# IGNF/StrataNet2-Vegetation-Coverage-Maps

Hardware: AMD Instinct MI355X
Metric: plots/s fwd+bwd, 32k-pt synthetic plots, batch 16/GPU (higher is better)
Workload: dtype f32; 1 GPU; C2 ref-arch: 16 plots/GPU x 32768 pts, SA npoint 1024/256 + global, r 1/2 m, train step fwd+P2+loss+bwd+Adam, inputs resident in HBM; plots_per_gpu=16, points_per_plot=32768, batches_per_geometry_pass=8, exchange=none (single GPU), parallelism=single GPU, ranks_seen=1, exchange_in_graph=False

## Files before the change

### include/strata_hip.h

```cpp
#ifndef STRATA_HIP_H
#define STRATA_HIP_H

#include <stddef.h>

#ifdef __cplusplus
extern "C" {
#endif

#define SN2_VERSION 102
#define SN2_EINVAL (-1)
#define SN2_ELIMIT (-2)

#define SN2_MAX_NEIGHBORS 2000
#define SN2_STAT_SLOTS 1024

int sn2_version(void);
int sn2_debug_mfma_chain(const float *a, const float *b, float *d, int mode, void *stream);
int sn2_debug_spin(int blocks, long long clocks, int *out, void *stream);

int sn2_debug_fp1_backward_parts(int mask);
int sn2_debug_fp_rows_form(int form);
int sn2_debug_fp_table_form(int form);
#define SN2_PROBE_SINK_WORDS 4096
int sn2_debug_stream_probe(const float *src, float *dst, size_t n_floats, int mode, float *sink, void *stream);
int sn2_debug_mfma_probe(int mode, int iters, float *sink, double *flops, void *stream);

typedef struct sn2_block {
    int cin, cout;
    const float *W, *b;
    const float *gamma, *beta;
    float *running_mean, *running_var;
    float *a, *c;
    float *mean, *invstd;
    float *stat_slots;
    float *dW, *db, *dgamma, *dbeta;
    int grad_replicas, grad_replica_stride;
    int mma_bf16;
    long long *num_batches_tracked;
    int frozen_stats;
} sn2_block;
#define SN2_BN_FROZEN_KEEP 2
int sn2_grad_reduce(float *flat, int n, int replicas, int stride, void *stream);


int sn2_pack_rows(const float *cloud, const float *xyz, int B, int C, int N, float *rows0, void *stream);

#define SN2_FPS_WS_WORDS(B, N) (6L * (B) * (N) + (4104L + 4096L) * (B) + 32L)
int sn2_fps(const float *pos_soa, int B, int N, int M, const int *start, int *idx, float *cpos_soa,
            float *cpos_aos, int *order_ws, void *stream);
int sn2_fps_waves(const float *pos_soa, int B, int N, int M, const int *start, int *idx, float *cpos_soa,
                  float *cpos_aos, int *order_ws, int waves, void *stream);
int sn2_fps_status(const float *pos_soa, int B, int N, int M, const int *start, int *idx, float *cpos_soa,
                   float *cpos_aos, int *order_ws, int waves, unsigned *status, void *stream);
int sn2_debug_fps_spin_limit(unsigned sweeps);

int sn2_ball_query(const float *src_soa, int B, int N, const float *cpos_soa, int M, float r2, int cap,
                   int *nbr, int *cnt, unsigned long long *total, const int *fps_ws, void *stream);

int sn2_count_sum(const int *cnt, int n, unsigned long long *total, void *stream);
int sn2_count_sum_group(const int *cnt, int G, int n, unsigned long long *total, size_t total_stride, void *stream);

#define SN2_THREE_NN_WS_WORDS(B, S) ((size_t)(B) * (4 * (size_t)(S) + 1032))
int sn2_three_nn(const float *src_soa, int B, int S, const float *dst_soa, int T, int k, int *idx, float *w,
                 void *ws, const int *dst_fps_ws, void *stream);
#define SN2_THREE_NN_XY_WS_WORDS(B, S, T) ((size_t)(B) * (4 * (size_t)(S) + 5 * (size_t)(T) + 1032))
int sn2_three_nn_xy(const float *src_soa, int B, int S, const float *dst_soa, int T, int k, int *idx, float *w,
                    void *ws, void *stream);

int sn2_prepare_plots(const float *raw, long T, const int *offsets, const float *centers, const float *fake_xy, int n_fake,
                      const int *idx, int B, int N, int train, const double *rot, const int *flips, const float *noise,
                      const long *noise_offsets, long noise_T, float z_max, float *cloud, float *xyz, void *stream);

#define SN2_SUBSAMPLE_LDS 1
#define SN2_SUBSAMPLE_GLOBAL 2
#define SN2_SUBSAMPLE_COARSE 4
#define SN2_SUBSAMPLE_LDS_MAX 16384
int sn2_subsample_form(int n_max, int N);
size_t sn2_subsample_ws_words(int B, int n_max, int N, int form);
int sn2_subsample(const int *offsets, int extra, int n_max, int B, int N, unsigned long long seed, const long long *plot_keys,
                  int form, int *ws, size_t ws_words, int *idx, void *stream);

#define SN2_ZNORM_WS_WORDS(n, cells) ((size_t)5 * (n) + 3 * (size_t)(cells) + 8)
int sn2_znorm(const float *x, const float *y, const float *z, int n, float radius, float x_min, float y_min, float x_max,
              float y_max, int *ws, float *zmin, float *z_out, void *stream);

size_t sn2_parcel_count_ws_words(int P, int rows);
size_t sn2_parcel_znorm_ws_words(long T, float radius, float x_min, float y_min, float x_max, float y_max);
int sn2_parcel_count(const float *cloud, long T, int L, int rows, const float *centers, int P, const int *cell_start,
                     const int *cell_items, int GX, int GY, double gx0, double gy0, double cell_inv, float radius, int *ws,
                     size_t ws_words, int *prefix, long long *total, void *stream);
int sn2_parcel_fill(const float *cloud, long T, int L, int rows, const float *centers, int P, const int *cell_start,
                    const int *cell_items, int GX, int GY, double gx0, double gy0, double cell_inv, float radius, int *prefix,
                    const int *plot_base, long sum_n, float *raw, int *point_index, void *stream);
int sn2_parcel_znorm(const float *cloud, long T, float x_min, float y_min, float x_max, float y_max, float radius,
                     float disc_radius, const int *offsets, const float *centers, int P, const int *point_index, long sum_n,
                     int *ws, size_t ws_words, float *raw, void *stream);

typedef struct sn2_sa {
    int B, Nsrc, M, cap;
    int cf;
    int nl;
    const float *feat; int feat_stride;
    const float *spos; int spos_stride;
    const float *cpos;
    const int *nbr, *cnt;
    const unsigned long long *total;
    const int *order;
    sn2_block blk[2];
    float *ext; int *arg;
    float *out;
    const float *dout;
    float *dfeat;
    float *bwd_ws;
} sn2_sa;
#define SN2_SA_BWD_WS_REPLICAS 32
#define SN2_SA_BWD_WS_WORDS (SN2_SA_BWD_WS_REPLICAS * 2 * 16 * 12)
#define SN2_SA_SOLO_MIN 64
#define SN2_SA_QUAD_MIN 8
#define SN2_SA_OCT_MIN 4
#define SN2_SA_SOLO_FLAG 0x40000000
#define SN2_SA_OCT_FLAG 0x20000000
#define SN2_SA_PACKED_ITEMS(M) ((M) / 8 + 2)
#define SN2_SA_ORDER_WORDS(B, M) ((size_t)4 * (B) * (M) + (size_t)16 * (B) * SN2_SA_PACKED_ITEMS(M) + 8)
int sn2_sa_order(const int *cnt, int B, int M, int *order, void *stream);
int sn2_sa_order_group(const int *cnt, int G, int B, int M, int *order, size_t stride_words, void *stream);
int sn2_sa_forward(const sn2_sa *p, int training, void *stream);
int sn2_sa_backward(const sn2_sa *p, void *stream);

typedef struct sn2_fp {
    int B, R_per_plot, S_per_plot;
    int ca, cb;
    const float *src; int src_stride; const float *src_a, *src_c;
    const int *knn_idx; const float *knn_w;
    const float *skip; int skip_stride;
    sn2_block blk;
    float *h; int h_stride;
    const float *dy;
    float *dsrc; int dsrc_stride;
    float *dskip; int dskip_stride;
    float *du_scratch;
    float *scatter_ws;
    int scatter_ready;
    const int *bn_sums_done;
    float *src_ws;
    int act_bf16;
    const int *row_perm;
} sn2_fp;
#define SN2_INTERP_CHUNKS(R, S) ((3 * (size_t)(R) + 62) / 63 + (size_t)(S))
#define SN2_FP_SRC_WS_WORDS(B, R, S, cout) ((size_t)(B) * SN2_INTERP_CHUNKS(R, S) * ((((cout) + 3) / 4) * 4))
#define SN2_INTERP_WS_WORDS(B, R, S) \
    ((size_t)(B) * (S) * (((R) + 2047) / 2048 + 6) + 6 * (size_t)(B) * (R) + 64 + 4 * (size_t)(B) * SN2_INTERP_CHUNKS(R, S))
int sn2_interp_index(const int *knn_idx, const float *knn_w, const float *src_pos, int B, int R_per_plot,
                     int S_per_plot, float *ws, void *stream);
int sn2_interp_index_perm(const int *knn_idx, const float *knn_w, const float *src_pos, const int *row_perm, int B,
                          int R_per_plot, int S_per_plot, float *ws, void *stream);
int sn2_interp_index_group(const int *knn_idx, const float *knn_w, const float *src_pos, const int *row_perm, int G, int B,
                           int R_per_plot, int S_per_plot, float *ws, size_t ws_stride_words, void *stream);
int sn2_fp_forward(const sn2_fp *p, int training, void *stream);
int sn2_fp_backward(const sn2_fp *p, void *stream);

int sn2_plot_max_forward(const float *h, const float *a, const float *c, int B, int R_per_plot, int C, float *out,
                         int *arg, void *stream);
int sn2_plot_max_backward(const float *dout, const int *arg, int B, int R_per_plot, int C, float *dy, void *stream);

int sn2_global_pool_backward(const float *du, int du_stride, const int *arg, const float *h, const float *mean,
                             const float *invstd, int B, int R_per_plot, int C, float *dx, float *dy, float *dgamma,
                             float *dbeta, void *stream);

#define SN2_GLOBAL_XCHG_WORDS(B) ((size_t)2 * (size_t)(B) * 4 * 128)
#define SN2_GLOBAL_CTL_WORDS 8
int sn2_global_level_forward(const sn2_fp *sa3, const sn2_fp *fp3, float *x3, int *arg3, unsigned long long *xchg,
                             unsigned *ctl, void *stream);
int sn2_debug_global_spin_limit(unsigned sweeps);

typedef struct sn2_head {
    int R, cin, f_stride;
    const float *f, *fa, *fc;
    const float *W1, *b1, *W2, *b2;
    float *coverages, *proba;
    const float *dcoverages, *dproba;
    float *dy;
    float *dW1, *db1, *dW2, *db2;
    int grad_replicas, grad_replica_stride;
    const int *drop_mask;
    float drop_scale;
    int act_bf16;
    float *zero_fill; long zero_fill_words;
} sn2_head;
int sn2_head_forward(const sn2_head *p, void *stream);
int sn2_fp_head_eval(const sn2_fp *p, const sn2_head *hd, void *stream);
int sn2_head_backward(const sn2_head *p, void *stream);
int sn2_head_bn_sums(const sn2_head *p, const float *gamma, const float *beta, const float *mean, const float *invstd,
                     float *dgamma, float *dbeta, int *ok, void *stream);
int sn2_fp_bn_sums(const sn2_fp *p, const float *gamma, const float *beta, const float *mean, const float *invstd,
                   float *dgamma, float *dbeta, int *ok, void *stream);


int sn2_plot_project_forward(const float *pred_pointwise, const float *cloud_xy, long plot_stride, int B, int N,
                             int D, unsigned long long *keys, int *pix, int *arg, int *nocc, float *pred,
                             void *stream);
#define SN2_P2_KEY_PARTS(N) (((N) + 4095) / 4096 < 1 ? 1 : (((N) + 4095) / 4096 > 64 ? 64 : ((N) + 4095) / 4096))
int sn2_plot_pixels(const float *cloud_xy, long plot_stride, int B, int N, int D, float *mm, int *pix, void *stream);
int sn2_plot_project_forward_pix(const float *pred_pointwise, const int *pix, int B, int N, int D,
                                 unsigned long long *keys, int *arg, int *nocc, float *pred, void *stream);
int sn2_plot_project_backward(const float *dpred, const int *arg, const int *nocc, const int *pix, int B, int N,
                              int D, float *dpointwise, void *stream);

int sn2_raster_project(const float *coverages, const float *cloud_xy, long plot_stride, int B, int N, int D,
                       int diam_meters, unsigned long long *keys, int *pix, float *rasters, void *stream);

int sn2_mosaic_merge(const float *rasters, const float *weights, const int *offsets, int B, int D, int H, int W,
                     float *mean, float *wsum, int win_y0, int win_x0, int win_h, int win_w, void *stream);

#define SN2_MOSAIC_HIST_WORDS 10004
int sn2_mosaic_finalize(const float *mean, const float *wsum, int H, int W, int *hist_ws, double *sum_ws, float *thr_out,
                        float *out, void *stream);

int sn2_kde_lookup(const float *cloud, int B, int C, int N, int z_channel, float z_max, const double *X, const double *Y,
                   int K, double *pdf, void *stream);
#define SN2_KDE_FIT_MAX_K 65536
#define SN2_KDE_FIT_ABS_SLOTS 256
#define SN2_KDE_FIT_SLICES 8
#define SN2_KDE_FIT_WS_WORDS(K) \
    (2 * ((4 + 3 * SN2_KDE_FIT_SLICES) * (size_t)(K) + 3 * (((size_t)(K) + 255) / 256)) + SN2_KDE_FIT_ABS_SLOTS)
int sn2_kde_fit(const float *z, long n, double bw, int K, void *ws, double *X, double *Y, void *stream);
#define SN2_LOSS_BLOCKS 1024
int sn2_loss_forward(const float *pred, const double *gt, int B, const float *proba, const double *pdf, int R, double m,
                     double e, double *partials, double *out, void *stream);
int sn2_loss_backward(const float *pred, const double *gt, int B, const float *proba, const double *pdf, int R, double m,
                      double e, const double *grad_total, float *dpred, float *dproba, void *stream);

#define SN2_PROJECTED_LOSS_WS (2 * 512 + 2)
int sn2_projected_loss_forward(const float *coverages, const int *pix, const float *proba, const double *pdf, const double *gt,
                               int B, int N, int D, double m, double e, unsigned long long *keys, int *arg, int *nocc,
                               float *pred, double *partials, double *out, void *stream);
int sn2_projected_loss_backward(const float *pred, const double *gt, int B, const float *proba, const double *pdf, int N, int D,
                                double m, double e, const double *grad_total, const int *arg, const int *nocc, const int *pix,
                                float *dcoverages, float *dproba, void *stream);

#define SN2_PLOT_LOSSES_SLICE_ROWS 2048
#define SN2_PLOT_LOSSES_SLICES(N) \
    (((N) + SN2_PLOT_LOSSES_SLICE_ROWS - 1) / SN2_PLOT_LOSSES_SLICE_ROWS < 1 ? 1 : \
     (((N) + SN2_PLOT_LOSSES_SLICE_ROWS - 1) / SN2_PLOT_LOSSES_SLICE_ROWS > 64 ? 64 : ((N) + SN2_PLOT_LOSSES_SLICE_ROWS - 1) / SN2_PLOT_LOSSES_SLICE_ROWS))
size_t sn2_plot_losses_ws_words(int B, int N, int D);
int sn2_plot_losses(const float *coverages, const int *pix, const float *proba, const double *pdf, const double *gt, int B, int N,
                    int D, double m, double e, void *ws, float *pred, double *out, void *stream);

int sn2_adam_step(float *param, const float *grad, float *exp_avg, float *exp_avg_sq, int n, float lr, float beta1,
                  float beta2, float eps, float weight_decay, int *step_dev ,
                  float grad_scale, void *stream);


typedef struct sn2_net_layer {
    int cin, cout;
    const float *W, *b, *gamma, *beta;
    float *running_mean, *running_var;
    long long *num_batches_tracked;
    int gW, gb, ggamma, gbeta;
    int mma_bf16;
} sn2_net_layer;

typedef struct sn2_net_model {
    sn2_net_layer sa1[2], sa2, sa3, fp3, fp2, fp1;
    const float *lin1_W, *lin1_b, *lin2_W, *lin2_b;
    int g_lin1_W, g_lin1_b, g_lin2_W, g_lin2_b;
    int n_flat;
    float r1_sq, r2_sq;
    int max_neighbors;
    float drop_p;
    int fuse_global_level;
    int fuse_eval_head;
    int source_side;
    int fps_waves_shared, fps_waves_many;
} sn2_net_model;

typedef struct sn2_net_dims {
    int B, N, M1, M2;
    int cap1, cap2;
    int act_bf16;
    int p2_diam_pix;
} sn2_net_dims;

typedef struct sn2_net_geo {
    const float *xyz;
    int *idx1; float *pos1_soa, *pos1_aos; int *ws1;
    int *nbr1, *cnt1; unsigned long long *tot1; int *ord1;
    int *idx2; float *pos2_soa, *pos2_aos; int *ws2;
    int *nbr2, *cnt2; unsigned long long *tot2; int *ord2;
    const float *pos3;
    int *knn3_idx; float *knn3_w;
    int *knn2_idx; float *knn2_w;
    int *knn1_idx; float *knn1_w;
    float *inv3, *inv2, *inv1;
    int *nn_ws2, *nn_ws1;
    const int *rank1;
    float *rows0;
    int *p2_pix; float *p2_mm;
} sn2_net_geo;

typedef struct sn2_net_act {
    float *aux;
    float *stats;
    float *ext1; int *arg1; float *x1;
    float *ext2; int *arg2; float *x2;
    float *h_sa3, *h3;
    float *x3; int *arg3;
    float *h2;
    void *h1;
    float *src_ws1, *src_ws2;
    float *cov, *proba;
    const int *drop_mask;
    float *bwd_arena; long bwd_arena_words;
} sn2_net_act;

typedef struct sn2_net_bwd {
    const float *dcov, *dproba;
    float *arena; long arena_words;
    int images, image_stride;
    float *dy2, *dy3, *dx1, *dx2, *dx3, *dy_sa3;
    float *sa1_ws;
    void *dy1, *du1;
    float *du2, *du3;
    int *bn_ok;
    float *src_ws1, *src_ws2;
    int defer_grad_reduce;
    int arena_is_zero;
    int frozen_stats;
} sn2_net_bwd;

#define SN2_NET_FORK 1
#define SN2_NET_SHARED 2
#define SN2_NET_INVERTED 4
#define SN2_NET_DEFER_JOIN 8
#define SN2_NET_INPUT_ONLY 16
#define SN2_NET_HAS_ROWS0 32
#define SN2_NET_JOIN_PENDING 64
#define SN2_NET_WITH_GEOMETRY 128
#define SN2_NET_HAS_INVERTED 256

typedef struct sn2_net_io {
    const float *cloud;
    const int *fps_start;
    unsigned *fps_status;
    unsigned long long *gl_xchg; unsigned *gl_ctl;
    void *stream_b, *stream_c, *stream_pack;
    void *ctx;
    int flags;
    int training;
} sn2_net_io;

int sn2_net_ctx_create(void **ctx);
int sn2_net_ctx_destroy(void *ctx);
int sn2_net_geo_carve(const sn2_net_model *m, const sn2_net_dims *d, void *base, sn2_net_geo *out, size_t *bytes);
int sn2_net_act_carve(const sn2_net_model *m, const sn2_net_dims *d, int training, void *base, sn2_net_act *out, size_t *bytes);
int sn2_net_bwd_carve(const sn2_net_model *m, const sn2_net_dims *d, void *arena_base, void *scratch_base, sn2_net_bwd *out,
                      size_t *arena_bytes, size_t *scratch_bytes);
int sn2_net_geometry(const sn2_net_model *m, const sn2_net_dims *d, const sn2_net_geo *g, const sn2_net_io *io, void *stream);
int sn2_net_forward(const sn2_net_model *m, const sn2_net_dims *d, const sn2_net_geo *g, const sn2_net_act *a,
                    const sn2_net_io *io, void *stream);
int sn2_net_backward(const sn2_net_model *m, const sn2_net_dims *d, const sn2_net_geo *g, const sn2_net_act *a,
                     const sn2_net_bwd *b, void *stream);

int sn2_adam_step_images(float *param, float *grad_images, int replicas, int stride, float *exp_avg, float *exp_avg_sq, int n,
                         float lr, float beta1, float beta2, float eps, float weight_decay, int *step_dev, float grad_scale,
                         void *stream);

#ifdef __cplusplus
}
#endif
#endif
```

### stratanet2_vegetation_coverage_maps_amd/_build.py

```python
import os
import subprocess
import sys
from concurrent.futures import ThreadPoolExecutor

HERE = os.path.dirname(os.path.abspath(__file__))
CSRC = os.path.join(HERE, "csrc")
LIB = os.path.join(CSRC, "libstrata_hip.so")
VARIANT_DIR = os.path.join(os.path.dirname(HERE), "build", "variants")
SOURCES = ["geometry.hip", "sa.hip", "sa_mfma.hip", "fp.hip", "interp_index.hip", "global_level.hip", "head.hip", "project.hip",
           "loss.hip", "misc.hip", "net.hip", "parcel.hip", "sample.hip", "kde.hip"]
HEADERS = ["common.h", "mlp.h", "fp_rows.h", os.path.join("..", "..", "include", "strata_hip.h")]
FLAGS = ["--offload-arch=gfx950", "-O3", "-fPIC", "-std=c++17", "-Wno-unused-result"] + os.environ.get("SN2_EXTRA_HIPCC_FLAGS", "").split()


def _stale(target, deps):
    if not os.path.exists(target):
        return True
    t = os.path.getmtime(target)
    return any(os.path.getmtime(d) > t for d in deps)


def _compile(lib, objdir, flags, force, verbose):
    hipcc = os.environ.get("HIPCC", "/opt/rocm/bin/hipcc")
    if not os.path.exists(hipcc):
        hipcc = "hipcc"
    hdrs = [os.path.join(CSRC, h) for h in HEADERS]
    objs, jobs = [], []
    for s in SOURCES:
        src = os.path.join(CSRC, s)
        obj = os.path.join(objdir, s.replace(".hip", ".o"))
        objs.append(obj)
        if force or _stale(obj, [src] + hdrs):
            jobs.append([hipcc] + flags + ["-c", src, "-o", obj])

    def run(cmd):
        if verbose:
            print(" ".join(cmd), flush=True)
        r = subprocess.run(cmd, stdout=subprocess.PIPE, stderr=subprocess.STDOUT, text=True)
        if r.returncode != 0:
            raise RuntimeError(f"hipcc failed ({r.returncode}):\n{r.stdout}")
        return r.stdout

    with ThreadPoolExecutor(max_workers=min(4, max(1, len(jobs)))) as ex:
        list(ex.map(run, jobs))
    if force or jobs or _stale(lib, objs):
        run([hipcc, "--offload-arch=gfx950", "-shared", "-fPIC"] + objs + ["-o", lib])
    return lib


def build(force: bool = False, verbose: bool = True) -> str:
    return _compile(LIB, CSRC, FLAGS, force, verbose)


def build_variant(name: str, extra_flags=(), verbose: bool = False) -> str:
    out = os.path.abspath(os.path.join(VARIANT_DIR, name))
    if os.path.commonpath([out, CSRC]) == CSRC:
        raise ValueError(f"{out}: a variant build must not go into {CSRC}")
    objdir = out + ".objs"
    os.makedirs(objdir, exist_ok=True)
    return _compile(out, objdir, FLAGS + list(extra_flags), True, verbose)


if __name__ == "__main__":
    print(build(force="--force" in sys.argv))
```

### stratanet2_vegetation_coverage_maps_amd/_lib.py

```python
import ctypes
import os
from ctypes import POINTER, Structure, c_double, c_float, c_int, c_long, c_longlong, c_void_p

HERE = os.path.dirname(os.path.abspath(__file__))
LIB_PATH = os.path.join(HERE, "csrc", "libstrata_hip.so")

SN2_VERSION = 102
MAX_NEIGHBORS = 2000
STAT_SLOTS = 1024


class Block(Structure):
    _fields_ = [("cin", c_int), ("cout", c_int), ("W", c_void_p), ("b", c_void_p), ("gamma", c_void_p),
                ("beta", c_void_p), ("running_mean", c_void_p), ("running_var", c_void_p), ("a", c_void_p),
                ("c", c_void_p), ("mean", c_void_p), ("invstd", c_void_p), ("stat_slots", c_void_p),
                ("dW", c_void_p), ("db", c_void_p), ("dgamma", c_void_p), ("dbeta", c_void_p),
                ("grad_replicas", c_int), ("grad_replica_stride", c_int), ("mma_bf16", c_int),
                ("num_batches_tracked", c_void_p), ("frozen_stats", c_int)]


BN_FROZEN_KEEP = 2


class SA(Structure):
    _fields_ = [("B", c_int), ("Nsrc", c_int), ("M", c_int), ("cap", c_int), ("cf", c_int), ("nl", c_int),
                ("feat", c_void_p), ("feat_stride", c_int), ("spos", c_void_p), ("spos_stride", c_int),
                ("cpos", c_void_p), ("nbr", c_void_p), ("cnt", c_void_p), ("total", c_void_p), ("order", c_void_p),
                ("blk", Block * 2),
                ("ext", c_void_p), ("arg", c_void_p), ("out", c_void_p), ("dout", c_void_p), ("dfeat", c_void_p),
                ("bwd_ws", c_void_p)]


class FP(Structure):
    _fields_ = [("B", c_int), ("R_per_plot", c_int), ("S_per_plot", c_int), ("ca", c_int), ("cb", c_int),
                ("src", c_void_p), ("src_stride", c_int), ("src_a", c_void_p), ("src_c", c_void_p),
                ("knn_idx", c_void_p), ("knn_w", c_void_p), ("skip", c_void_p), ("skip_stride", c_int),
                ("blk", Block), ("h", c_void_p), ("h_stride", c_int), ("dy", c_void_p), ("dsrc", c_void_p),
                ("dsrc_stride", c_int), ("dskip", c_void_p), ("dskip_stride", c_int), ("du_scratch", c_void_p),
                ("scatter_ws", c_void_p), ("scatter_ready", c_int), ("bn_sums_done", c_void_p), ("src_ws", c_void_p),
                ("act_bf16", c_int), ("row_perm", c_void_p)]


class Head(Structure):
    _fields_ = [("R", c_int), ("cin", c_int), ("f_stride", c_int), ("f", c_void_p), ("fa", c_void_p),
                ("fc", c_void_p), ("W1", c_void_p), ("b1", c_void_p), ("W2", c_void_p), ("b2", c_void_p),
                ("coverages", c_void_p), ("proba", c_void_p), ("dcoverages", c_void_p), ("dproba", c_void_p),
                ("dy", c_void_p), ("dW1", c_void_p), ("db1", c_void_p), ("dW2", c_void_p), ("db2", c_void_p),
                ("grad_replicas", c_int), ("grad_replica_stride", c_int), ("drop_mask", c_void_p), ("drop_scale", c_float),
                ("act_bf16", c_int), ("zero_fill", c_void_p), ("zero_fill_words", c_long)]


class NetLayer(Structure):
    _fields_ = [("cin", c_int), ("cout", c_int), ("W", c_void_p), ("b", c_void_p), ("gamma", c_void_p), ("beta", c_void_p),
                ("running_mean", c_void_p), ("running_var", c_void_p), ("num_batches_tracked", c_void_p),
                ("gW", c_int), ("gb", c_int), ("ggamma", c_int), ("gbeta", c_int), ("mma_bf16", c_int)]


class NetModel(Structure):
    _fields_ = [("sa1", NetLayer * 2), ("sa2", NetLayer), ("sa3", NetLayer), ("fp3", NetLayer), ("fp2", NetLayer), ("fp1", NetLayer),
                ("lin1_W", c_void_p), ("lin1_b", c_void_p), ("lin2_W", c_void_p), ("lin2_b", c_void_p),
                ("g_lin1_W", c_int), ("g_lin1_b", c_int), ("g_lin2_W", c_int), ("g_lin2_b", c_int), ("n_flat", c_int),
                ("r1_sq", c_float), ("r2_sq", c_float), ("max_neighbors", c_int), ("drop_p", c_float),
                ("fuse_global_level", c_int), ("fuse_eval_head", c_int), ("source_side", c_int),
                ("fps_waves_shared", c_int), ("fps_waves_many", c_int)]


class NetDims(Structure):
    _fields_ = [("B", c_int), ("N", c_int), ("M1", c_int), ("M2", c_int), ("cap1", c_int), ("cap2", c_int), ("act_bf16", c_int),
                ("p2_diam_pix", c_int)]


class NetGeo(Structure):
    _fields_ = [(n, c_void_p) for n in (
        "xyz", "idx1", "pos1_soa", "pos1_aos", "ws1", "nbr1", "cnt1", "tot1", "ord1",
        "idx2", "pos2_soa", "pos2_aos", "ws2", "nbr2", "cnt2", "tot2", "ord2", "pos3",
        "knn3_idx", "knn3_w", "knn2_idx", "knn2_w", "knn1_idx", "knn1_w", "inv3", "inv2", "inv1", "nn_ws2", "nn_ws1",
        "rank1", "rows0", "p2_pix", "p2_mm")]


class NetAct(Structure):
    _fields_ = [(n, c_void_p) for n in (
        "aux", "stats", "ext1", "arg1", "x1", "ext2", "arg2", "x2", "h_sa3", "h3", "x3", "arg3", "h2", "h1", "src_ws1", "src_ws2",
        "cov", "proba", "drop_mask", "bwd_arena")] + [("bwd_arena_words", c_long)]


class NetBwd(Structure):
    _fields_ = [("dcov", c_void_p), ("dproba", c_void_p), ("arena", c_void_p), ("arena_words", c_long), ("images", c_int),
                ("image_stride", c_int)] + [(n, c_void_p) for n in (
                    "dy2", "dy3", "dx1", "dx2", "dx3", "dy_sa3", "sa1_ws", "dy1", "du1", "du2", "du3", "bn_ok", "src_ws1", "src_ws2")] + [
                        ("defer_grad_reduce", c_int), ("arena_is_zero", c_int), ("frozen_stats", c_int)]


class NetIO(Structure):
    _fields_ = [("cloud", c_void_p), ("fps_start", c_void_p), ("fps_status", c_void_p), ("gl_xchg", c_void_p), ("gl_ctl", c_void_p),
                ("stream_b", c_void_p), ("stream_c", c_void_p), ("stream_pack", c_void_p), ("ctx", c_void_p), ("flags", c_int),
                ("training", c_int)]


NET_FORK, NET_SHARED, NET_INVERTED, NET_DEFER_JOIN, NET_INPUT_ONLY = 1, 2, 4, 8, 16
NET_HAS_ROWS0, NET_JOIN_PENDING, NET_WITH_GEOMETRY, NET_HAS_INVERTED = 32, 64, 128, 256


SIGNATURES = {
    "sn2_version": [],
    "sn2_debug_mfma_chain": [c_void_p, c_void_p, c_void_p, c_int, c_void_p],
    "sn2_debug_spin": [c_int, c_longlong, c_void_p, c_void_p],
    "sn2_debug_fp1_backward_parts": [c_int],
    "sn2_debug_fp_rows_form": [c_int],
    "sn2_debug_fp_table_form": [c_int],
    "sn2_debug_stream_probe": [c_void_p, c_void_p, ctypes.c_size_t, c_int, c_void_p, c_void_p],
    "sn2_debug_mfma_probe": [c_int, c_int, c_void_p, POINTER(c_double), c_void_p],
    "sn2_pack_rows": [c_void_p, c_void_p, c_int, c_int, c_int, c_void_p, c_void_p],
    "sn2_fps": [c_void_p, c_int, c_int, c_int, c_void_p, c_void_p, c_void_p, c_void_p, c_void_p, c_void_p],
    "sn2_fps_waves": [c_void_p, c_int, c_int, c_int, c_void_p, c_void_p, c_void_p, c_void_p, c_void_p, c_int, c_void_p],
    "sn2_fps_status": [c_void_p, c_int, c_int, c_int, c_void_p, c_void_p, c_void_p, c_void_p, c_void_p, c_int, c_void_p, c_void_p],
    "sn2_debug_fps_spin_limit": [ctypes.c_uint],
    "sn2_ball_query": [c_void_p, c_int, c_int, c_void_p, c_int, c_float, c_int, c_void_p, c_void_p, c_void_p, c_void_p,
                       c_void_p],
    "sn2_three_nn": [c_void_p, c_int, c_int, c_void_p, c_int, c_int, c_void_p, c_void_p, c_void_p, c_void_p, c_void_p],
    "sn2_count_sum": [c_void_p, c_int, c_void_p, c_void_p],
    "sn2_count_sum_group": [c_void_p, c_int, c_int, c_void_p, ctypes.c_size_t, c_void_p],
    "sn2_three_nn_xy": [c_void_p, c_int, c_int, c_void_p, c_int, c_int, c_void_p, c_void_p, c_void_p, c_void_p],
    "sn2_prepare_plots": [c_void_p, c_long, c_void_p, c_void_p, c_void_p, c_int, c_void_p, c_int, c_int, c_int, c_void_p,
                          c_void_p, c_void_p, c_void_p, c_long, c_float, c_void_p, c_void_p, c_void_p],
    "sn2_znorm": [c_void_p, c_void_p, c_void_p, c_int, c_float, c_float, c_float, c_float, c_float, c_void_p, c_void_p,
                  c_void_p, c_void_p],
    "sn2_parcel_count": [c_void_p, c_long, c_int, c_int, c_void_p, c_int, c_void_p, c_void_p, c_int, c_int, c_double, c_double,
                         c_double, c_float, c_void_p, ctypes.c_size_t, c_void_p, c_void_p, c_void_p],
    "sn2_parcel_fill": [c_void_p, c_long, c_int, c_int, c_void_p, c_int, c_void_p, c_void_p, c_int, c_int, c_double, c_double,
                        c_double, c_float, c_void_p, c_void_p, c_long, c_void_p, c_void_p, c_void_p],
    "sn2_parcel_znorm": [c_void_p, c_long, c_float, c_float, c_float, c_float, c_float, c_float, c_void_p, c_void_p, c_int,
                         c_void_p, c_long, c_void_p, ctypes.c_size_t, c_void_p, c_void_p],
    "sn2_subsample_form": [c_int, c_int],
    "sn2_subsample": [c_void_p, c_int, c_int, c_int, c_int, ctypes.c_ulonglong, c_void_p, c_int, c_void_p, ctypes.c_size_t,
                      c_void_p, c_void_p],
    "sn2_sa_order": [c_void_p, c_int, c_int, c_void_p, c_void_p],
    "sn2_sa_order_group": [c_void_p, c_int, c_int, c_int, c_void_p, ctypes.c_size_t, c_void_p],
    "sn2_sa_forward": [POINTER(SA), c_int, c_void_p],
    "sn2_sa_backward": [POINTER(SA), c_void_p],
    "sn2_grad_reduce": [c_void_p, c_int, c_int, c_int, c_void_p],
    "sn2_interp_index": [c_void_p, c_void_p, c_void_p, c_int, c_int, c_int, c_void_p, c_void_p],
    "sn2_interp_index_perm": [c_void_p, c_void_p, c_void_p, c_void_p, c_int, c_int, c_int, c_void_p, c_void_p],
    "sn2_interp_index_group": [c_void_p, c_void_p, c_void_p, c_void_p, c_int, c_int, c_int, c_int, c_void_p, ctypes.c_size_t, c_void_p],
    "sn2_fp_forward": [POINTER(FP), c_int, c_void_p],
    "sn2_fp_backward": [POINTER(FP), c_void_p],
    "sn2_plot_max_forward": [c_void_p, c_void_p, c_void_p, c_int, c_int, c_int, c_void_p, c_void_p, c_void_p],
    "sn2_plot_max_backward": [c_void_p, c_void_p, c_int, c_int, c_int, c_void_p, c_void_p],
    "sn2_global_pool_backward": [c_void_p, c_int, c_void_p, c_void_p, c_void_p, c_void_p, c_int, c_int, c_int, c_void_p, c_void_p,
                                 c_void_p, c_void_p, c_void_p],
    "sn2_global_level_forward": [POINTER(FP), POINTER(FP), c_void_p, c_void_p, c_void_p, c_void_p, c_void_p],
    "sn2_debug_global_spin_limit": [ctypes.c_uint],
    "sn2_head_forward": [POINTER(Head), c_void_p],
    "sn2_fp_head_eval": [POINTER(FP), POINTER(Head), c_void_p],
    "sn2_fp_bn_sums": [POINTER(FP), c_void_p, c_void_p, c_void_p, c_void_p, c_void_p, c_void_p, c_void_p, c_void_p],
    "sn2_head_bn_sums": [POINTER(Head), c_void_p, c_void_p, c_void_p, c_void_p, c_void_p, c_void_p, c_void_p, c_void_p],
    "sn2_head_backward": [POINTER(Head), c_void_p],
    "sn2_plot_project_forward": [c_void_p, c_void_p, c_long, c_int, c_int, c_int, c_void_p, c_void_p, c_void_p,
                                 c_void_p, c_void_p, c_void_p],
    "sn2_plot_pixels": [c_void_p, c_long, c_int, c_int, c_int, c_void_p, c_void_p, c_void_p],
    "sn2_plot_project_forward_pix": [c_void_p, c_void_p, c_int, c_int, c_int, c_void_p, c_void_p, c_void_p, c_void_p, c_void_p],
    "sn2_plot_project_backward": [c_void_p, c_void_p, c_void_p, c_void_p, c_int, c_int, c_int, c_void_p, c_void_p],
    "sn2_raster_project": [c_void_p, c_void_p, c_long, c_int, c_int, c_int, c_int, c_void_p, c_void_p, c_void_p,
                           c_void_p],
    "sn2_mosaic_merge": [c_void_p, c_void_p, c_void_p, c_int, c_int, c_int, c_int, c_void_p, c_void_p,
                         c_int, c_int, c_int, c_int, c_void_p],
    "sn2_mosaic_finalize": [c_void_p, c_void_p, c_int, c_int, c_void_p, c_void_p, c_void_p, c_void_p, c_void_p],
    "sn2_kde_lookup": [c_void_p, c_int, c_int, c_int, c_int, c_float, c_void_p, c_void_p, c_int, c_void_p, c_void_p],
    "sn2_kde_fit": [c_void_p, c_long, c_double, c_int, c_void_p, c_void_p, c_void_p, c_void_p],
    "sn2_loss_forward": [c_void_p, c_void_p, c_int, c_void_p, c_void_p, c_int, c_double, c_double, c_void_p, c_void_p,
                         c_void_p],
    "sn2_loss_backward": [c_void_p, c_void_p, c_int, c_void_p, c_void_p, c_int, c_double, c_double, c_void_p, c_void_p,
                          c_void_p, c_void_p],
    "sn2_adam_step": [c_void_p, c_void_p, c_void_p, c_void_p, c_int, c_float, c_float, c_float, c_float, c_float,
                      c_void_p, c_float, c_void_p],
    "sn2_projected_loss_forward": [c_void_p, c_void_p, c_void_p, c_void_p, c_void_p, c_int, c_int, c_int, c_double, c_double, c_void_p,
                                   c_void_p, c_void_p, c_void_p, c_void_p, c_void_p, c_void_p],
    "sn2_projected_loss_backward": [c_void_p, c_void_p, c_int, c_void_p, c_void_p, c_int, c_int, c_double, c_double, c_void_p, c_void_p,
                                    c_void_p, c_void_p, c_void_p, c_void_p, c_void_p],
    "sn2_plot_losses": [c_void_p, c_void_p, c_void_p, c_void_p, c_void_p, c_int, c_int, c_int, c_double, c_double, c_void_p, c_void_p,
                        c_void_p, c_void_p],
    "sn2_adam_step_images": [c_void_p, c_void_p, c_int, c_int, c_void_p, c_void_p, c_int, c_float, c_float, c_float, c_float, c_float,
                             c_void_p, c_float, c_void_p],
    "sn2_net_ctx_create": [POINTER(c_void_p)],
    "sn2_net_ctx_destroy": [c_void_p],
    "sn2_net_geo_carve": [POINTER(NetModel), POINTER(NetDims), c_void_p, POINTER(NetGeo), POINTER(ctypes.c_size_t)],
    "sn2_net_act_carve": [POINTER(NetModel), POINTER(NetDims), c_int, c_void_p, POINTER(NetAct), POINTER(ctypes.c_size_t)],
    "sn2_net_bwd_carve": [POINTER(NetModel), POINTER(NetDims), c_void_p, c_void_p, POINTER(NetBwd), POINTER(ctypes.c_size_t),
                          POINTER(ctypes.c_size_t)],
    "sn2_net_geometry": [POINTER(NetModel), POINTER(NetDims), POINTER(NetGeo), POINTER(NetIO), c_void_p],
    "sn2_net_forward": [POINTER(NetModel), POINTER(NetDims), POINTER(NetGeo), POINTER(NetAct), POINTER(NetIO), c_void_p],
    "sn2_net_backward": [POINTER(NetModel), POINTER(NetDims), POINTER(NetGeo), POINTER(NetAct), POINTER(NetBwd), c_void_p],
}

SIZE_HELPERS = {
    "sn2_parcel_count_ws_words": [c_int, c_int],
    "sn2_parcel_znorm_ws_words": [c_long, c_float, c_float, c_float, c_float, c_float],
    "sn2_subsample_ws_words": [c_int, c_int, c_int, c_int],
    "sn2_plot_losses_ws_words": [c_int, c_int, c_int],
}

_lib = None


class StrataHipError(RuntimeError):
    pass


def load():
    global _lib
    if _lib is not None:
        return _lib
    if not os.path.exists(LIB_PATH):
        raise StrataHipError(
            f"{LIB_PATH} not found: build it with `python -m stratanet2_vegetation_coverage_maps_amd._build` "
            "(or __graft_entry__.build()); the HIP library is mandatory, there is no fallback path")
    lib = ctypes.CDLL(LIB_PATH)
    for name, argtypes in SIGNATURES.items():
        fn = getattr(lib, name)
        fn.argtypes = argtypes
        fn.restype = c_int
    for name, argtypes in SIZE_HELPERS.items():
        fn = getattr(lib, name)
        fn.argtypes = argtypes
        fn.restype = ctypes.c_size_t
    if lib.sn2_version() != SN2_VERSION:
        raise StrataHipError(f"libstrata_hip.so version {lib.sn2_version()} != binding {SN2_VERSION}: rebuild")
    _lib = lib
    return lib


def check(rc: int, what: str):
    if rc != 0:
        kind = "hipError_t" if rc > 0 else {-1: "SN2_EINVAL", -2: "SN2_ELIMIT"}.get(rc, "error")
        raise StrataHipError(f"{what} failed: {kind} {rc}")
```

### stratanet2_vegetation_coverage_maps_amd/csrc/common.h

```cpp
#pragma once
#include <hip/hip_runtime.h>
#include <stdint.h>

#include "../../include/strata_hip.h"

#define SN2_WAVE 64

#define SN2_RETURN_LAUNCH()                                   \
    do {                                                      \
        hipError_t e__ = hipGetLastError();                   \
        return e__ == hipSuccess ? 0 : (int)e__;              \
    } while (0)

#define SN2_TRY(expr)                \
    do {                             \
        int r__ = (expr);            \
        if (r__ != 0) return r__;    \
    } while (0)

#ifdef SN2_NO_FLUSH
#define SN2_FLUSH_ADD(ptr, v) do { if ((v) == 12345.678f) atomicAdd((ptr), (v)); } while (0)
#else
#define SN2_FLUSH_ADD(ptr, v) atomicAdd((ptr), (v))
#endif

#ifdef __HIPCC__
__device__ __forceinline__ int sn2_grad_image(int replicas, int stride) {
    return replicas > 1 ? (int)(blockIdx.x % (unsigned)replicas) * stride : 0;
}
#endif

static inline int sn2_cdiv(long a, long b) { return (int)((a + b - 1) / b); }

constexpr int GL_MAX_PLOTS = 28;

#ifdef __HIPCC__
static __global__ __launch_bounds__(256) void sn2_fill_words_kernel(uint32_t* __restrict__ p, uint32_t v, size_t n) {
    for (size_t i = (size_t)blockIdx.x * 256 + threadIdx.x; i < n; i += (size_t)gridDim.x * 256) p[i] = v;
}
static inline void sn2_fill_words(void* p, uint32_t v, size_t nwords, hipStream_t st) {
    if (nwords == 0) return;
    int grid = sn2_cdiv((long)nwords, 256 * 4);
    grid = grid < 1 ? 1 : (grid > 2048 ? 2048 : grid);
    hipLaunchKernelGGL(sn2_fill_words_kernel, dim3(grid), dim3(256), 0, st, (uint32_t*)p, v, nwords);
}
#endif

static inline bool sn2_small_sort_wg(int B) { return B > 32; }

static inline int sn2_cu_count() {
    static int n = 0;
    if (n == 0) {
        int dev = 0, v = 0;
        if (hipGetDevice(&dev) == hipSuccess &&
            hipDeviceGetAttribute(&v, hipDeviceAttributeMultiprocessorCount, dev) == hipSuccess && v > 0)
            n = v;
        else
            n = 256;
    }
    return n;
}

typedef const float __attribute__((address_space(4)))* cfp;
__device__ __forceinline__ cfp as_const(const float* p) { return (cfp)(uintptr_t)p; }
__device__ __forceinline__ cfp opaque(cfp p) {
    uint64_t v = (uint64_t)p;
    asm volatile("" : "+s"(v));
    return (cfp)v;
}

__device__ __forceinline__ float sn2_d2(float ax, float ay, float az, float bx, float by, float bz) {
#pragma clang fp contract(off)
    float dx = ax - bx;
    float dy = ay - by;
    float dz = az - bz;
    float xx = dx * dx;
    float yy = dy * dy;
    float zz = dz * dz;
    float s = xx + yy;
    return s + zz;
}

__device__ __forceinline__ unsigned long long wave_max_u64(unsigned long long v) {
#pragma unroll
    for (int o = 32; o > 0; o >>= 1) {
        unsigned long long t = __shfl_xor(v, o);
        v = t > v ? t : v;
    }
    return v;
}

#define SN2_DPP(x, ctrl, rmask) __builtin_amdgcn_update_dpp((x), (x), (ctrl), (rmask), 0xF, false)
__device__ __forceinline__ float wave_max_dpp(float v) {
    v = fmaxf(v, __int_as_float(SN2_DPP(__float_as_int(v), 0xB1, 0xF)));
    v = fmaxf(v, __int_as_float(SN2_DPP(__float_as_int(v), 0x4E, 0xF)));
    v = fmaxf(v, __int_as_float(SN2_DPP(__float_as_int(v), 0x141, 0xF)));
    v = fmaxf(v, __int_as_float(SN2_DPP(__float_as_int(v), 0x140, 0xF)));
    v = fmaxf(v, __int_as_float(SN2_DPP(__float_as_int(v), 0x142, 0xA)));
    v = fmaxf(v, __int_as_float(SN2_DPP(__float_as_int(v), 0x143, 0xC)));
    return __int_as_float(__builtin_amdgcn_readlane(__float_as_int(v), 63));
}
__device__ __forceinline__ float wave_min_dpp(float v) { return -wave_max_dpp(-v); }
__device__ __forceinline__ float wave_sum_dpp(float v) {
    v += __int_as_float(SN2_DPP(__float_as_int(v), 0xB1, 0xF));
    v += __int_as_float(SN2_DPP(__float_as_int(v), 0x4E, 0xF));
    v += __int_as_float(SN2_DPP(__float_as_int(v), 0x141, 0xF));
    v += __int_as_float(SN2_DPP(__float_as_int(v), 0x140, 0xF));
    v += __int_as_float(SN2_DPP(__float_as_int(v), 0x142, 0xA));
    v += __int_as_float(SN2_DPP(__float_as_int(v), 0x143, 0xC));
    return __int_as_float(__builtin_amdgcn_readlane(__float_as_int(v), 63));
}
__device__ __forceinline__ float wave_sum(float v) { return wave_sum_dpp(v); }
__device__ __forceinline__ float wave_max(float v) { return wave_max_dpp(v); }
__device__ __forceinline__ float wave_min(float v) { return wave_min_dpp(v); }
__device__ __forceinline__ unsigned wave_min_u32_dpp(unsigned v) {
    v = min(v, (unsigned)SN2_DPP((int)v, 0xB1, 0xF));
    v = min(v, (unsigned)SN2_DPP((int)v, 0x4E, 0xF));
    v = min(v, (unsigned)SN2_DPP((int)v, 0x141, 0xF));
    v = min(v, (unsigned)SN2_DPP((int)v, 0x140, 0xF));
    v = min(v, (unsigned)SN2_DPP((int)v, 0x142, 0xA));
    v = min(v, (unsigned)SN2_DPP((int)v, 0x143, 0xC));
    return (unsigned)__builtin_amdgcn_readlane((int)v, 63);
}

__device__ __forceinline__ int lane_id() { return threadIdx.x & 63; }

__device__ __forceinline__ uint32_t f2ord(float f) {
    uint32_t u = __float_as_uint(f);
    return (u & 0x80000000u) ? ~u : (u | 0x80000000u);
}
__device__ __forceinline__ float ord2f(uint32_t o) {
    uint32_t u = (o & 0x80000000u) ? (o & 0x7FFFFFFFu) : ~o;
    return __uint_as_float(u);
}
```

### stratanet2_vegetation_coverage_maps_amd/csrc/global_level.hip

```cpp
#include "fp_rows.h"

namespace {

#ifdef SN2_GL_STAMPS
__device__ unsigned long long g_gl_dbg[16];
extern "C" int sn2_debug_gl_stamps(unsigned long long* out) {
    return (int)hipMemcpyFromSymbol(out, HIP_SYMBOL(g_gl_dbg), sizeof(g_gl_dbg));
}
#define GSTAMP(i)                                                                                   \
    if (blockIdx.x == 0 && threadIdx.x == 0) {                                                      \
        unsigned long long t_;                                                                      \
        asm volatile("s_memtime %0\n\ts_waitcnt lgkmcnt(0)" : "=s"(t_)::"memory");                   \
        g_gl_dbg[i] = t_;                                                                           \
    }
#else
#define GSTAMP(i)
#endif
typedef unsigned long long gl_u64;
constexpr int GL_GROUPS = 4, GL_QS = OuterAcc<16, 36>::QS;
constexpr int GL_W3 = 64 * 35 + 64, GL_WF = 64 * 96 + 64;
constexpr int GL_FIXED_FLOATS = GL_GROUPS * 64 * GL_QS + GL_GROUPS * 128 + 128 + 64 + 2 * 1024 + 2 * 8 * 128 + GL_W3 + GL_WF;
static_assert((GL_FIXED_FLOATS + GL_MAX_PLOTS * GL_GROUPS * 128) * 4 <= 160 * 1024, "LDS");

template <int KB>
__device__ __forceinline__ void gl_block_tiles(const float* s_q, int QS, int lane, int g, long row0, long R_lim,
                                               const float (&Wb)[KB], float init, float* __restrict__ h, int h_stride,
                                               float& ssum, float& ssq, f32x4 (&V)[4]) {
    const int qq = lane >> 4, cc = lane & 15, o = 16 * g + cc;
#pragma unroll
    for (int t = 0; t < 4; ++t) V[t] = f32x4{init, init, init, init};
#pragma unroll
    for (int kb = 0; kb < KB; ++kb) {
#pragma unroll
        for (int t = 0; t < 4; ++t)
            V[t] = __builtin_amdgcn_mfma_f32_16x16x4f32(s_q[(16 * t + cc) * QS + 4 * kb + qq], Wb[kb], V[t], 0, 0, 0);
    }
#pragma unroll
    for (int t = 0; t < 4; ++t)
#pragma unroll
        for (int j = 0; j < 4; ++j) {
            const long row = row0 + 16 * t + 4 * qq + j;
            const float v = row < R_lim ? fmaxf(V[t][j], 0.f) : 0.f;
            V[t][j] = v;
            ssum += v;
            ssq = fmaf(v, v, ssq);
            if (row < R_lim) h[(size_t)row * h_stride + o] = v;
        }
}

struct GlLayer {
    const float *W, *bias, *gamma, *beta;
    float *running_mean, *running_var, *a, *c, *mean, *invstd;
    long long* nbt;
    float* h;
};
struct GlArgs {
    int B, M2;
    const float* x2;
    const float* pos2;
    const int* knn_idx;
    const float* knn_w;
    float* x3;
    int* arg3;
    GlLayer sa3, fp3;
    gl_u64* xchg;
    unsigned* ctl;
    unsigned spin_limit;
};

constexpr unsigned GL_POISON = 0x80000000u;
__device__ __forceinline__ bool gl_collect(const gl_u64* gx, int n, unsigned tag, float* s_x, unsigned spin_limit) {
    bool ok = true;
    for (int i0 = threadIdx.x; i0 < n; i0 += 8 * 1024) {
        gl_u64 v[8];
        unsigned spins = 0;
        bool all, poisoned;
        do {
#pragma unroll
            for (int u = 0; u < 8; ++u) {
                const int i = i0 + u * 1024;
                v[u] = __hip_atomic_load(gx + (i < n ? i : i0), __ATOMIC_RELAXED, __HIP_MEMORY_SCOPE_AGENT);
            }
            all = true, poisoned = false;
#pragma unroll
            for (int u = 0; u < 8; ++u) {
                all = all && (unsigned)(v[u] >> 32) == tag;
                poisoned = poisoned || (unsigned)(v[u] >> 32) == (tag ^ GL_POISON);
            }
            if (!all && !poisoned) __builtin_amdgcn_s_sleep(2);
        } while (!all && !poisoned && ++spins < spin_limit);
        if (!all) ok = false;
#pragma unroll
        for (int u = 0; u < 8; ++u)
            if (i0 + u * 1024 < n) s_x[i0 + u * 1024] = __uint_as_float((unsigned)v[u]);
    }
    return ok;
}

template <bool REPAIR>
__device__ __forceinline__ void gl_level_body(const GlArgs& A, float* gl_smem) {
    const int tid = threadIdx.x, lane = tid & 63;
    const int grp = __builtin_amdgcn_readfirstlane(tid >> 8), g = __builtin_amdgcn_readfirstlane((tid >> 6) & 3);
    float* s_q = gl_smem + grp * 64 * GL_QS;

    float* s_red = gl_smem + GL_GROUPS * 64 * GL_QS;
    float* s_ac = s_red + GL_GROUPS * 128;
    float* s_x3 = s_ac + 128;
    float* s_mv = s_x3 + 64;
    int* s_mi = reinterpret_cast<int*>(s_mv + 1024);
    double* s_d = reinterpret_cast<double*>(s_mi + 1024);
    float* s_w3 = reinterpret_cast<float*>(s_d + 8 * 128);
    float* s_wf = s_w3 + GL_W3;
    float* s_x = s_wf + GL_WF;
    __shared__ unsigned s_epoch;
    __shared__ int s_fail;
    const int B = A.B, M2 = A.M2;
    const int b_lo = REPAIR ? 0 : (int)blockIdx.x, b_hi = REPAIR ? B : b_lo + 1;
    const bool lead = REPAIR || blockIdx.x == 0;
    float w3r[3], b3r, bfr;
    f32x4 wfr[2];
#pragma unroll
    for (int j = 0; j < 3; ++j) w3r[j] = A.sa3.W[min(tid + 1024 * j, 64 * 35 - 1)];
#pragma unroll
    for (int j = 0; j < 2; ++j) wfr[j] = reinterpret_cast<const f32x4*>(A.fp3.W)[min(tid + 1024 * j, 64 * 96 / 4 - 1)];
    b3r = A.sa3.bias[tid & 63], bfr = A.fp3.bias[tid & 63];
    unsigned epoch_now = 0;
    if (tid == 0) epoch_now = __hip_atomic_load(&A.ctl[0], __ATOMIC_RELAXED, __HIP_MEMORY_SCOPE_AGENT);
#pragma unroll
    for (int j = 0; j < 3; ++j)
        if (tid + 1024 * j < 64 * 35) s_w3[tid + 1024 * j] = w3r[j];
#pragma unroll
    for (int j = 0; j < 2; ++j)
        if (tid + 1024 * j < 64 * 96 / 4) reinterpret_cast<f32x4*>(s_wf)[tid + 1024 * j] = wfr[j];
    if (tid < 64) s_w3[64 * 35 + tid] = b3r, s_wf[64 * 96 + tid] = bfr;
    if (tid == 0) {
        s_epoch = epoch_now + 1u;
        s_fail = 0;
    }
    const int nblk = (M2 + 63) >> 6, trips = (nblk + GL_GROUPS - 1) / GL_GROUPS;
    const int qq = lane >> 4, cc = lane & 15, o = 16 * g + cc;
    const int n_gran = B * GL_GROUPS * 128;
    const double n_rows = (double)B * (double)M2;
    __syncthreads();
    const unsigned epoch = s_epoch;
    unsigned applied = 0;
    if constexpr (REPAIR) applied = __hip_atomic_load(&A.ctl[3], __ATOMIC_RELAXED, __HIP_MEMORY_SCOPE_AGENT);
    f32x4 V3[4];
#pragma unroll
    for (int t = 0; t < 4; ++t) V3[t] = f32x4{0.f, 0.f, 0.f, 0.f};
    GSTAMP(0)
    for (int b = b_lo; b < b_hi; ++b) {
        constexpr int CA = 32, CB = 3, CI = CA + CB, CK = CI + 1, KB = (CK + 3) / 4, QS = OuterAcc<16, CK>::QS;
        const long row_lo = (long)b * M2, R_lim = row_lo + M2;
        float Wb[KB];
        float ssum = 0.f, ssq = 0.f;
        for (int it = 0; it < trips; ++it) {
            const int blk = it * GL_GROUPS + grp;
            const long r0 = row_lo + (long)blk * 64;
            if (blk < nblk) {
                stage_inputs<CA, CB, false>(s_q, QS, g, lane, r0, (int)R_lim, M2, M2, A.x2, 32, nullptr, nullptr, nullptr, nullptr,
                                            A.pos2, 4);
                if (g == 2) {
#pragma unroll
                    for (int k = CK; k < 4 * KB; ++k) s_q[lane * QS + k] = 0.f;
                }
            }
            __syncthreads();
            if (it == 0) {
#pragma unroll
                for (int kb = 0; kb < KB; ++kb) {
                    const int k = 4 * kb + qq;
                    Wb[kb] = k < CI ? s_w3[o * CI + k] : (k == CI ? s_w3[64 * CI + o] : 0.f);
                }
            }
            if (blk < nblk) gl_block_tiles<KB>(s_q, QS, lane, g, r0, R_lim, Wb, 0.f, A.sa3.h, 64, ssum, ssq, V3);
            __syncthreads();
        }
        ssum += __shfl_xor(ssum, 16);
        ssq += __shfl_xor(ssq, 16);
        ssum += __shfl_xor(ssum, 32);
        ssq += __shfl_xor(ssq, 32);
        if (qq == 0) {
            s_red[grp * 128 + o] = ssum;
            s_red[grp * 128 + 64 + o] = ssq;
        }
        __syncthreads();
        if (b == b_lo) { GSTAMP(1) }
        if (tid < GL_GROUPS * 128)
            __hip_atomic_store(A.xchg + (size_t)b * GL_GROUPS * 128 + tid,
                               ((gl_u64)(epoch * 2u + 0u) << 32) | (gl_u64)__float_as_uint(s_red[tid]), __ATOMIC_RELAXED,
                               __HIP_MEMORY_SCOPE_AGENT);
        if constexpr (REPAIR) __syncthreads();
    }
    {
        const unsigned tag = epoch * 2u + 0u;
        if (!gl_collect(A.xchg, n_gran, tag, s_x, A.spin_limit)) s_fail = 1;
        __syncthreads();
        GSTAMP(2)
        if (s_fail) {
            if constexpr (!REPAIR) {
                if (tid < GL_GROUPS * 128)
                    __hip_atomic_store(A.xchg + n_gran + (size_t)b_lo * GL_GROUPS * 128 + tid, (gl_u64)((epoch * 2u + 1u) ^ GL_POISON) << 32,
                                       __ATOMIC_RELAXED, __HIP_MEMORY_SCOPE_AGENT);
                if (tid == 0) {
                    atomicAdd(&A.ctl[1], 1u);
                    if (lead) {
                        __hip_atomic_store(&A.ctl[3], 0u, __ATOMIC_RELAXED, __HIP_MEMORY_SCOPE_AGENT);
                        __hip_atomic_store(&A.ctl[0], epoch, __ATOMIC_RELAXED, __HIP_MEMORY_SCOPE_AGENT);
                    }
                }
                return;
            }
        }
        {
            const int col = tid & 127, part = tid >> 7;
            double acc = 0.0;
            for (int w = part; w < B * GL_GROUPS; w += 8) acc += (double)s_x[w * 128 + col];
            s_d[part * 128 + col] = acc;
        }
        __syncthreads();
        if (tid < 64) {
            double s1 = 0.0, s2 = 0.0;
#pragma unroll
            for (int part = 0; part < 8; ++part) s1 += s_d[part * 128 + tid], s2 += s_d[part * 128 + 64 + tid];
            float aa, cc2, mean, invstd;
            const bool upd = lead && !(applied & 1u);
            sn2_bn_from_sums(s1, s2, n_rows, A.sa3.gamma[tid], A.sa3.beta[tid], upd ? &A.sa3.running_mean[tid] : nullptr,
                             upd ? &A.sa3.running_var[tid] : nullptr, aa, cc2, mean, invstd);
            s_ac[tid] = aa;
            s_ac[64 + tid] = cc2;
            if (lead) {
                A.sa3.a[tid] = aa, A.sa3.c[tid] = cc2, A.sa3.mean[tid] = mean, A.sa3.invstd[tid] = invstd;
                if (tid == 0 && upd && A.sa3.nbt) *A.sa3.nbt += 1;
            }
        }
        __syncthreads();
    }
    GSTAMP(3)
    for (int b = b_lo; b < b_hi; ++b) {
    const long row_lo = (long)b * M2, R_lim = row_lo + M2;
    if (!REPAIR && trips == 1) {
        const float aa = s_ac[o], cc2 = s_ac[64 + o];
        float best = -INFINITY;
        int bi = 0x7FFFFFFF;
#pragma unroll
        for (int t = 0; t < 4; ++t)
#pragma unroll
            for (int j = 0; j < 4; ++j) {
                const int r = grp * 64 + 16 * t + 4 * qq + j;
                const float y = fmaf(aa, V3[t][j], cc2);
                if (r < M2 && y > best) best = y, bi = r;
            }
#pragma unroll
        for (int m = 16; m <= 32; m <<= 1) {
            const float v = __shfl_xor(best, m);
            const int i = __shfl_xor(bi, m);
            if (v > best || (v == best && i < bi)) best = v, bi = i;
        }
        if (qq == 0) s_mv[grp * 64 + o] = best, s_mi[grp * 64 + o] = bi;
        __syncthreads();
        if (tid < 64) {
            best = s_mv[tid], bi = s_mi[tid];
            for (int k2 = 1; k2 < GL_GROUPS; ++k2) {
                const float v = s_mv[k2 * 64 + tid];
                const int i = s_mi[k2 * 64 + tid];
                if (v > best || (v == best && i < bi)) best = v, bi = i;
            }
            A.x3[(size_t)b * 64 + tid] = best;
            A.arg3[(size_t)b * 64 + tid] = bi;
            s_x3[tid] = best;
        }
        __syncthreads();
    } else {
        const int ch = tid & 63, rg = tid >> 6;
        const float aa = s_ac[ch], cc2 = s_ac[64 + ch];
        float best = -INFINITY;
        int bi = 0x7FFFFFFF;
        const float* hb = A.sa3.h + (size_t)row_lo * 64 + ch;
        int r = rg;
        for (; r + 7 * 16 < M2; r += 8 * 16) {
            float v[8];
#pragma unroll
            for (int u = 0; u < 8; ++u) v[u] = hb[(size_t)(r + u * 16) * 64];
#pragma unroll
            for (int u = 0; u < 8; ++u) {
                const float y = fmaf(aa, v[u], cc2);
                if (y > best) best = y, bi = r + u * 16;
            }
        }
        for (; r < M2; r += 16) {
            const float y = fmaf(aa, hb[(size_t)r * 64], cc2);
            if (y > best) best = y, bi = r;
        }
        s_mv[tid] = best;
        s_mi[tid] = bi;
        __syncthreads();
        if (tid < 64) {
            for (int k2 = 1; k2 < 16; ++k2) {
                const float v = s_mv[k2 * 64 + ch];
                const int i = s_mi[k2 * 64 + ch];
                if (v > best || (v == best && i < bi)) best = v, bi = i;
            }
            A.x3[(size_t)b * 64 + ch] = best;
            A.arg3[(size_t)b * 64 + ch] = bi;
            s_x3[ch] = best;
        }
        __syncthreads();
    }
    if (b == b_lo) { GSTAMP(4) }
    {
        constexpr int CA = 64, CB = 32, CI = CA + CB, KB = CB / 4, QS = OuterAcc<16, 36>::QS;
        float* s_pv = s_mv;
        {
            const int oo = tid >> 4, part = tid & 15;
            const float4 w4 = *reinterpret_cast<const float4*>(s_wf + oo * CI + 4 * part);
            const float4 u4 = *reinterpret_cast<const float4*>(s_x3 + 4 * part);
            float acc = ((w4.x * u4.x + w4.y * u4.y) + w4.z * u4.z) + w4.w * u4.w;
#pragma unroll
            for (int m = 8; m > 0; m >>= 1) acc += __shfl_xor(acc, m);
            if (part == 0) s_pv[oo] = acc + s_wf[64 * CI + oo];
        }
        float Wb[KB];
#pragma unroll
        for (int kb = 0; kb < KB; ++kb) Wb[kb] = s_wf[o * CI + CA + 4 * kb + qq];
        float ssum = 0.f, ssq = 0.f;
        f32x4 Vf[4];
        for (int it = 0; it < trips; ++it) {
            const int blk = it * GL_GROUPS + grp;
            const long r0 = row_lo + (long)blk * 64;
            if (blk < nblk && (REPAIR || trips > 1)) {
                const int t256 = tid & 255;
#pragma unroll
                for (int pass = 0; pass < 2; ++pass) {
                    const int row = pass * 32 + (t256 >> 3), q8 = t256 & 7;
                    const long r = r0 + row;
                    const size_t rr = r < R_lim ? (size_t)r : (size_t)(R_lim - 1);
                    *reinterpret_cast<float4*>(&s_q[row * QS + 4 * q8]) = reinterpret_cast<const float4*>(A.x2 + rr * 32)[q8];
                }
            }
            __syncthreads();
            if (blk < nblk) gl_block_tiles<KB>(s_q, QS, lane, g, r0, R_lim, Wb, s_pv[o], A.fp3.h, 64, ssum, ssq, Vf);
            __syncthreads();
        }
        ssum += __shfl_xor(ssum, 16);
        ssq += __shfl_xor(ssq, 16);
        ssum += __shfl_xor(ssum, 32);
        ssq += __shfl_xor(ssq, 32);
        if (qq == 0) {
            s_red[grp * 128 + o] = ssum;
            s_red[grp * 128 + 64 + o] = ssq;
        }
    }
    __syncthreads();
    if (b == b_lo) { GSTAMP(5) }
    if (tid < GL_GROUPS * 128)
        __hip_atomic_store(A.xchg + n_gran + (size_t)b * GL_GROUPS * 128 + tid,
                           ((gl_u64)(epoch * 2u + 1u) << 32) | (gl_u64)__float_as_uint(s_red[tid]), __ATOMIC_RELAXED,
                           __HIP_MEMORY_SCOPE_AGENT);
    if constexpr (REPAIR) __syncthreads();
    }
    {
        gl_u64* gx = A.xchg + n_gran;
        const unsigned tag = epoch * 2u + 1u;
        if (!lead) return;
        if (!gl_collect(gx, n_gran, tag, s_x, A.spin_limit)) s_fail = 1;
        __syncthreads();
        GSTAMP(6)
        if (s_fail) {
            if (tid == 0) {
                atomicAdd(&A.ctl[1], 1u);
                __hip_atomic_store(&A.ctl[3], 1u, __ATOMIC_RELAXED, __HIP_MEMORY_SCOPE_AGENT);
                __hip_atomic_store(&A.ctl[0], epoch, __ATOMIC_RELAXED, __HIP_MEMORY_SCOPE_AGENT);
            }
            return;
        }
        {
            const int col = tid & 127, part = tid >> 7;
            double acc = 0.0;
            for (int w = part; w < B * GL_GROUPS; w += 8) acc += (double)s_x[w * 128 + col];
            s_d[part * 128 + col] = acc;
        }
        __syncthreads();
        if (tid < 64) {
            double s1 = 0.0, s2 = 0.0;
#pragma unroll
            for (int part = 0; part < 8; ++part) s1 += s_d[part * 128 + tid], s2 += s_d[part * 128 + 64 + tid];
            float aa, cc2, mean, invstd;
            const bool upd = !(applied & 2u);
            sn2_bn_from_sums(s1, s2, n_rows, A.fp3.gamma[tid], A.fp3.beta[tid], upd ? &A.fp3.running_mean[tid] : nullptr,
                             upd ? &A.fp3.running_var[tid] : nullptr, aa, cc2, mean, invstd);
            A.fp3.a[tid] = aa, A.fp3.c[tid] = cc2, A.fp3.mean[tid] = mean, A.fp3.invstd[tid] = invstd;
            if (tid == 0 && upd && A.fp3.nbt) *A.fp3.nbt += 1;
        }
        __syncthreads();
        GSTAMP(7)
        if (tid == 0) {
            if constexpr (REPAIR) {
                __hip_atomic_store(&A.ctl[2], __hip_atomic_load(&A.ctl[1], __ATOMIC_RELAXED, __HIP_MEMORY_SCOPE_AGENT), __ATOMIC_RELAXED,
                                   __HIP_MEMORY_SCOPE_AGENT);
                __hip_atomic_store(&A.ctl[0], epoch + 2u, __ATOMIC_RELAXED, __HIP_MEMORY_SCOPE_AGENT);
            } else {
                __hip_atomic_store(&A.ctl[3], 3u, __ATOMIC_RELAXED, __HIP_MEMORY_SCOPE_AGENT);
                __hip_atomic_store(&A.ctl[0], epoch, __ATOMIC_RELAXED, __HIP_MEMORY_SCOPE_AGENT);
            }
        }
    }
}

__global__ __launch_bounds__(1024) void global_level_fwd_kernel(GlArgs A) {
    extern __shared__ __attribute__((aligned(16))) float gl_smem[];
    __shared__ int s_repair;
    gl_level_body<false>(A, gl_smem);
    __syncthreads();
    if (threadIdx.x == 0) {
        const unsigned t = atomicAdd(&A.ctl[4], 1u);
        int repair = 0;
        if (t == gridDim.x - 1) {
            __hip_atomic_store(&A.ctl[4], 0u, __ATOMIC_RELAXED, __HIP_MEMORY_SCOPE_AGENT);
            repair = __hip_atomic_load(&A.ctl[1], __ATOMIC_RELAXED, __HIP_MEMORY_SCOPE_AGENT) !=
                     __hip_atomic_load(&A.ctl[2], __ATOMIC_RELAXED, __HIP_MEMORY_SCOPE_AGENT);
        }
        s_repair = repair;
    }
    __syncthreads();
    if (!s_repair) return;
    gl_level_body<true>(A, gl_smem);
}

}

static unsigned g_gl_spin_limit = 1u << 18;
extern "C" int sn2_debug_global_spin_limit(unsigned sweeps) {
    g_gl_spin_limit = sweeps ? sweeps : (1u << 18);
    return 0;
}

extern "C" int sn2_global_level_forward(const sn2_fp* sa3, const sn2_fp* fp3, float* x3, int* arg3, unsigned long long* xchg,
                                        unsigned* ctl, void* stream) {
    if (!sa3 || !fp3 || !x3 || !arg3 || !xchg || !ctl) return SN2_EINVAL;
    const int B = sa3->B, M2 = sa3->R_per_plot;
    if (!(B > 0 && M2 > 0 && fp3->B == B && fp3->R_per_plot == M2 && sa3->S_per_plot == M2 && fp3->S_per_plot == 1)) return SN2_EINVAL;
    if (!(sa3->ca == 32 && sa3->cb == 3 && sa3->blk.cin == 35 && sa3->blk.cout == 64 && fp3->ca == 64 && fp3->cb == 32 &&
          fp3->blk.cin == 96 && fp3->blk.cout == 64))
        return SN2_ELIMIT;
    if (sa3->blk.mma_bf16 || fp3->blk.mma_bf16 || sa3->act_bf16 || fp3->act_bf16) return SN2_ELIMIT;
    if (sa3->knn_idx || sa3->src_a || !fp3->knn_idx || !fp3->knn_w || fp3->src_a) return SN2_EINVAL;
    if (!sa3->src || sa3->src_stride != 32 || !sa3->skip || sa3->skip_stride != 4 || !sa3->h || sa3->h_stride != 64) return SN2_EINVAL;
    if (fp3->src != x3 || fp3->src_stride != 64 || fp3->skip != sa3->src || fp3->skip_stride != 32 || !fp3->h || fp3->h_stride != 64)
        return SN2_EINVAL;
    if (B > GL_MAX_PLOTS || (long)B * M2 >= (1L << 31) / 64) return SN2_ELIMIT;
    for (const sn2_block* k : {&sa3->blk, &fp3->blk})
        if (!k->W || !k->b || !k->gamma || !k->beta || !k->running_mean || !k->running_var || !k->a || !k->c || !k->mean || !k->invstd)
            return SN2_EINVAL;
    GlArgs A;
    A.B = B, A.M2 = M2;
    A.x2 = sa3->src, A.pos2 = sa3->skip, A.knn_idx = fp3->knn_idx, A.knn_w = fp3->knn_w, A.x3 = x3, A.arg3 = arg3;
    auto layer = [](const sn2_fp* p) {
        GlLayer l;
        l.W = p->blk.W, l.bias = p->blk.b, l.gamma = p->blk.gamma, l.beta = p->blk.beta;
        l.running_mean = p->blk.running_mean, l.running_var = p->blk.running_var;
        l.a = p->blk.a, l.c = p->blk.c, l.mean = p->blk.mean, l.invstd = p->blk.invstd;
        l.nbt = p->blk.num_batches_tracked, l.h = p->h;
        return l;
    };
    A.sa3 = layer(sa3), A.fp3 = layer(fp3);
    A.xchg = xchg, A.ctl = ctl;
    A.spin_limit = g_gl_spin_limit;
    const size_t lds = ((size_t)GL_FIXED_FLOATS + (size_t)B * GL_GROUPS * 128) * 4;
    (void)hipFuncSetAttribute(reinterpret_cast<const void*>(&global_level_fwd_kernel), hipFuncAttributeMaxDynamicSharedMemorySize, (int)lds);
    hipLaunchKernelGGL(global_level_fwd_kernel, dim3(B), dim3(1024), lds, (hipStream_t)stream, A);
    SN2_RETURN_LAUNCH();
}
```

### stratanet2_vegetation_coverage_maps_amd/csrc/net.hip

```cpp
#include "common.h"

#include <cstring>
#include <new>

namespace {

constexpr int WIDTHS[7] = {16, 16, 32, 64, 64, 34, 34};
constexpr int WIDTH_SUM = 260;
constexpr int GRAD_IMAGES = 32;

struct NetCtx {
    hipEvent_t fork, b_tables, b_nn, b_done, c_nn, c_done, pack_fork, packed;
};

inline long rows_stat_limit() { return 64L * SN2_STAT_SLOTS; }

inline bool fps_fills_ws(int B, int N, int m) {
    const bool many_small = N <= 4096 && B > 32;
    return N > 2048 && !many_small && m > 16 && ((long)B * N) % 4 == 0 && N <= 131072;
}
inline bool three_nn_uses_grid(int S, int T) { return S >= 128 && S <= 8192 && T > 2048; }
inline bool fp_src_ws_wanted(const sn2_net_model* m, long R, int cb, bool force) {
    return m->source_side && cb > 0 && cb <= 16 && cb % 4 == 0 && (R > rows_stat_limit() || force);
}
// ... 227 lines not shown
    if (fork) {
        sb = (hipStream_t)io->stream_b, sc = (hipStream_t)io->stream_c;
        NET_HIP(hipEventRecord(ctx->fork, cur));
        NET_HIP(hipStreamWaitEvent(sb, ctx->fork, 0));
        NET_HIP(hipStreamWaitEvent(sc, ctx->fork, 0));
    }
    SN2_TRY(sn2_fps_status(g->pos1_soa, B, M1, M2, start1, g->idx2, g->pos2_soa, g->pos2_aos, ws2, 0, io->fps_status, sb));
    SN2_TRY(sn2_ball_query(g->pos1_soa, B, M1, g->pos2_soa, M2, m->r2_sq, d->cap2, g->nbr2, g->cnt2, inverted ? g->tot2 : nullptr, ws2, sb));
    SN2_TRY(sn2_sa_order(g->cnt2, B, M2, g->ord2, sb));
    if (fork) NET_HIP(hipEventRecord(ctx->b_tables, sb));
    SN2_TRY(sn2_three_nn(g->pos3, B, 1, g->pos2_soa, M2, 1, g->knn3_idx, g->knn3_w, nullptr, nullptr, sb));
    SN2_TRY(three_nn_any(g->pos2_soa, B, M2, g->pos1_soa, M1, 3, g->knn2_idx, g->knn2_w, g->nn_ws2, sb));
    if (fork) NET_HIP(hipEventRecord(ctx->b_nn, sb));
    if (inverted) SN2_TRY(inverted_tables(d, g, 1, sb));
    SN2_TRY(three_nn_any(g->pos1_soa, B, M1, g->xyz, N, 3, g->knn1_idx, g->knn1_w, g->nn_ws1, sc));
    if (fork) NET_HIP(hipEventRecord(ctx->c_nn, sc));
    if (inverted) SN2_TRY(inverted_tables(d, g, 2, sc));
    if (flags & SN2_NET_INPUT_ONLY) {
        if (!io->cloud) return SN2_EINVAL;
        SN2_TRY(sn2_pack_rows(io->cloud, g->xyz, B, 10, N, g->rows0, cur));
        if (d->p2_diam_pix > 0 && g->p2_pix && g->p2_mm)
            SN2_TRY(sn2_plot_pixels(io->cloud, 10L * N, B, N, d->p2_diam_pix, g->p2_mm, g->p2_pix, cur));
    }
    SN2_TRY(sn2_ball_query(g->xyz, B, N, g->pos1_soa, M1, m->r1_sq, d->cap1, g->nbr1, g->cnt1, inverted ? g->tot1 : nullptr, ws1, cur));
    SN2_TRY(sn2_sa_order(g->cnt1, B, M1, g->ord1, cur));
    if (fork) {
        NET_HIP(hipEventRecord(ctx->b_done, sb));
        NET_HIP(hipEventRecord(ctx->c_done, sc));
        if (!(flags & SN2_NET_DEFER_JOIN)) {
            NET_HIP(hipStreamWaitEvent(cur, ctx->b_done, 0));
            NET_HIP(hipStreamWaitEvent(cur, ctx->c_done, 0));
        }
    }
    return 0;
}

}

extern "C" int sn2_net_ctx_create(void** out) {
    if (!out) return SN2_EINVAL;
    NetCtx* c = new (std::nothrow) NetCtx();
    if (!c) return SN2_EINVAL;
    hipEvent_t* ev[8] = {&c->fork, &c->b_tables, &c->b_nn, &c->b_done, &c->c_nn, &c->c_done, &c->pack_fork, &c->packed};
    for (int i = 0; i < 8; ++i) {
        hipError_t e = hipEventCreateWithFlags(ev[i], hipEventDisableTiming);
        if (e != hipSuccess) {
            for (int j = 0; j < i; ++j) (void)hipEventDestroy(*ev[j]);
            delete c;
            return (int)e;
        }
    }
    *out = c;
    return 0;
}

extern "C" int sn2_net_ctx_destroy(void* ctx) {
    if (!ctx) return SN2_EINVAL;
    NetCtx* c = static_cast<NetCtx*>(ctx);
    (void)hipEventDestroy(c->fork);
    (void)hipEventDestroy(c->b_tables);
    (void)hipEventDestroy(c->b_nn);
    (void)hipEventDestroy(c->b_done);
    (void)hipEventDestroy(c->c_nn);
    (void)hipEventDestroy(c->c_done);
    (void)hipEventDestroy(c->pack_fork);
    (void)hipEventDestroy(c->packed);
    delete c;
    return 0;
}

extern "C" int sn2_net_geo_carve(const sn2_net_model* m, const sn2_net_dims* d, void* base, sn2_net_geo* g, size_t* bytes) {
    SN2_TRY(check_dims(m, d));
    if (!g || !bytes) return SN2_EINVAL;
    const size_t B = d->B, N = d->N, M1 = d->M1, M2 = d->M2;
    memset(g, 0, sizeof(*g));
    Carver c(base);
    g->idx1 = c.take<int>(B * M1), g->pos1_soa = c.take<float>(B * 3 * M1), g->pos1_aos = c.take<float>(B * M1 * 4);
    g->ws1 = fps_fills_ws(d->B, d->N, d->M1) ? c.take<int>((size_t)SN2_FPS_WS_WORDS(B, N)) : nullptr;
    g->nbr1 = c.take<int>(B * M1 * (size_t)d->cap1), g->cnt1 = c.take<int>(B * M1);
    g->tot1 = c.take<unsigned long long>(1), g->ord1 = c.take<int>(SN2_SA_ORDER_WORDS(B, M1));
    g->idx2 = c.take<int>(B * M2), g->pos2_soa = c.take<float>(B * 3 * M2), g->pos2_aos = c.take<float>(B * M2 * 4);
    g->ws2 = fps_fills_ws(d->B, d->M1, d->M2) ? c.take<int>((size_t)SN2_FPS_WS_WORDS(B, M1)) : nullptr;
    g->nbr2 = c.take<int>(B * M2 * (size_t)d->cap2), g->cnt2 = c.take<int>(B * M2);
    g->tot2 = c.take<unsigned long long>(1), g->ord2 = c.take<int>(SN2_SA_ORDER_WORDS(B, M2));
    g->knn3_idx = c.take<int>(B * M2 * 3), g->knn3_w = c.take<float>(B * M2 * 3);
    g->knn2_idx = c.take<int>(B * M1 * 3), g->knn2_w = c.take<float>(B * M1 * 3);
    g->knn1_idx = c.take<int>(B * N * 3), g->knn1_w = c.take<float>(B * N * 3);
    g->inv3 = c.take<float>(SN2_INTERP_WS_WORDS(B, M2, 1));
    g->inv2 = c.take<float>(SN2_INTERP_WS_WORDS(B, M1, M2));
    g->inv1 = c.take<float>(SN2_INTERP_WS_WORDS(B, N, M1));
    g->nn_ws2 = three_nn_uses_grid(d->M2, d->M1) ? c.take<int>(SN2_THREE_NN_XY_WS_WORDS(B, M2, M1)) : nullptr;
    g->nn_ws1 = three_nn_uses_grid(d->M1, d->N) ? c.take<int>(SN2_THREE_NN_XY_WS_WORDS(B, M1, N)) : nullptr;
    g->rows0 = c.take<float>(B * N * 12);
    if (d->p2_diam_pix > 0) g->p2_pix = c.take<int>(B * N), g->p2_mm = c.take<float>(B * 4);
    *bytes = c.bytes();
    return 0;
}

extern "C" int sn2_net_act_carve(const sn2_net_model* m, const sn2_net_dims* d, int training, void* base, sn2_net_act* a,
                                 size_t* bytes) {
    SN2_TRY(check_dims(m, d));
    if (!a || !bytes) return SN2_EINVAL;
    const size_t B = d->B, N = d->N, M1 = d->M1, M2 = d->M2;
    memset(a, 0, sizeof(*a));
    Carver c(base);
    a->aux = c.take<float>(4 * WIDTH_SUM), a->stats = c.take<float>((size_t)SN2_STAT_SLOTS * 2 * WIDTH_SUM);
    a->ext1 = c.take<float>(B * M1 * 16), a->arg1 = c.take<int>(B * M1 * 16), a->x1 = c.take<float>(B * M1 * 16);
    a->ext2 = c.take<float>(B * M2 * 32), a->arg2 = c.take<int>(B * M2 * 32), a->x2 = c.take<float>(B * M2 * 32);
    a->h_sa3 = c.take<float>(B * M2 * 64), a->h3 = c.take<float>(B * M2 * 64);
    a->x3 = c.take<float>(B * 64), a->arg3 = c.take<int>(B * 64);
    a->h2 = c.take<float>(B * M1 * 36);
    const bool fused_eval = !training && m->fuse_eval_head && !d->act_bf16 && m->source_side;
    if (!fused_eval) a->h1 = d->act_bf16 ? (void*)c.take<unsigned short>(B * N * 36) : (void*)c.take<float>(B * N * 36);
    if (fp_src_ws_wanted(m, (long)B * N, 8, fused_eval)) a->src_ws1 = c.take<float>(SN2_FP_SRC_WS_WORDS(B, N, M1, 34));
    if (fp_src_ws_wanted(m, (long)B * M1, 16, false)) a->src_ws2 = c.take<float>(SN2_FP_SRC_WS_WORDS(B, M1, M2, 34));
    *bytes = c.bytes();
    return 0;
}

extern "C" int sn2_net_bwd_carve(const sn2_net_model* m, const sn2_net_dims* d, void* arena_base, void* scratch_base,
                                 sn2_net_bwd* b, size_t* arena_bytes, size_t* scratch_bytes) {
    SN2_TRY(check_dims(m, d));
    if (!b || !arena_bytes || !scratch_bytes || m->n_flat <= 0) return SN2_EINVAL;
    const size_t B = d->B, N = d->N, M1 = d->M1, M2 = d->M2;
    memset(b, 0, sizeof(*b));
    const size_t stride = ((size_t)m->n_flat + 63) / 64 * 64;
    float* ar = static_cast<float*>(arena_base);
    size_t o = GRAD_IMAGES * stride;
    auto take = [&](size_t n) {
        float* p = ar + o;
        o += (n + 3) / 4 * 4;
        return p;
    };
    b->arena = ar, b->images = GRAD_IMAGES, b->image_stride = (int)stride;
    b->dy2 = take(B * M1 * 36), b->dy3 = take(B * M2 * 64), b->dx1 = take(B * M1 * 16), b->dx2 = take(B * M2 * 32);
    b->dx3 = take(B * 64), b->dy_sa3 = take(B * M2 * 64);
    b->sa1_ws = take(SN2_SA_BWD_WS_WORDS);
    b->arena_words = (long)o;
    *arena_bytes = o * sizeof(float);
    Carver c(scratch_base);
    if (d->act_bf16) {
        b->dy1 = c.take<unsigned short>(B * N * 36), b->du1 = c.take<unsigned short>(B * N * 36);
    } else {
        b->dy1 = c.take<float>(B * N * 36), b->du1 = c.take<float>(B * N * 36);
    }
    b->du2 = c.take<float>(B * M1 * 64), b->du3 = c.take<float>(B * M2 * 64);
    b->bn_ok = c.take<int>(4);
    if (fp_src_ws_wanted(m, (long)B * N, 8, false)) b->src_ws1 = c.take<float>(SN2_FP_SRC_WS_WORDS(B, N, M1, 34));
    if (fp_src_ws_wanted(m, (long)B * M1, 16, false)) b->src_ws2 = c.take<float>(SN2_FP_SRC_WS_WORDS(B, M1, M2, 34));
    *scratch_bytes = c.bytes();
    return 0;
}

extern "C" int sn2_net_geometry(const sn2_net_model* m, const sn2_net_dims* d, const sn2_net_geo* g, const sn2_net_io* io,
                                void* stream) {
    SN2_TRY(check_dims(m, d));
    if (!io) return SN2_EINVAL;
    SN2_TRY(check_geo(d, g));
    SN2_TRY(check_geo_workspaces(d, g));
    if ((io->flags & SN2_NET_INVERTED) && (!g->inv1 || !g->inv2 || !g->inv3)) return SN2_EINVAL;
    return geometry_impl(m, d, g, io, io->flags, (hipStream_t)stream);
}

extern "C" int sn2_net_forward(const sn2_net_model* m, const sn2_net_dims* d, const sn2_net_geo* g, const sn2_net_act* a,
                               const sn2_net_io* io, void* stream) {
    SN2_TRY(check_dims(m, d));
    SN2_TRY(check_model_ptrs(m));
    if (!io || !a) return SN2_EINVAL;
    SN2_TRY(check_geo(d, g));
    if (!a->aux || !a->stats || !a->ext1 || !a->arg1 || !a->x1 || !a->ext2 || !a->arg2 || !a->x2 || !a->h_sa3 || !a->h3 || !a->x3 ||
        !a->arg3 || !a->h2 || !a->cov || !a->proba)
        return SN2_EINVAL;
    if (io->training < 0 || io->training > SN2_BN_FROZEN_KEEP) return SN2_EINVAL;
    const int mode = io->training, training = mode != 0 ? 1 : 0, batch_stats = mode == 1 ? 1 : 0, flags = io->flags;
    const int B = d->B, N = d->N, M2 = d->M2;
    hipStream_t cur = (hipStream_t)stream;
    NetCtx* ctx = static_cast<NetCtx*>(io->ctx);
    const bool fused_eval = !training && m->fuse_eval_head && !d->act_bf16 && m->source_side;
    if (!fused_eval && !a->h1) return SN2_EINVAL;
    if (training && !(g->inv1 && g->inv2 && g->inv3)) return SN2_EINVAL;
    const GradDst nograd{nullptr, 0, 0};
    bool join_b = false, join_c = false, wait_pack = false;
    bool have_rows0 = flags & SN2_NET_HAS_ROWS0;
    if (flags & SN2_NET_WITH_GEOMETRY) {
        if (!io->cloud) return SN2_EINVAL;
        SN2_TRY(check_geo_workspaces(d, g));
        int gflags = (flags & (SN2_NET_FORK | SN2_NET_SHARED)) | (training ? SN2_NET_INVERTED : 0);
        const bool fork = (flags & SN2_NET_FORK) && ctx && io->stream_b && io->stream_c;
        if (fork) {
            gflags |= SN2_NET_DEFER_JOIN;
            if (io->stream_pack && !have_rows0) {
                hipStream_t sp = (hipStream_t)io->stream_pack;
                NET_HIP(hipEventRecord(ctx->pack_fork, cur));
                NET_HIP(hipStreamWaitEvent(sp, ctx->pack_fork, 0));
                SN2_TRY(sn2_pack_rows(io->cloud, g->xyz, B, 10, N, g->rows0, sp));
                NET_HIP(hipEventRecord(ctx->packed, sp));
                wait_pack = have_rows0 = true;
            }
        } else {
            gflags &= ~SN2_NET_FORK;
        }
        SN2_TRY(geometry_impl(m, d, g, io, gflags, cur));
        join_b = join_c = fork;
    } else {
        if (flags & SN2_NET_JOIN_PENDING) {
            if (!ctx) return SN2_EINVAL;
            join_b = join_c = true;
        }
        if (training && !(flags & SN2_NET_HAS_INVERTED)) {
            if (join_b) NET_HIP(hipStreamWaitEvent(cur, ctx->b_done, 0));
            if (join_c) NET_HIP(hipStreamWaitEvent(cur, ctx->c_done, 0));
            join_b = join_c = false;
            SN2_TRY(inverted_tables(d, g, 3, cur));
        }
    }
    if (wait_pack) NET_HIP(hipStreamWaitEvent(cur, ctx->packed, 0));
    if (!have_rows0) {
        if (!io->cloud) return SN2_EINVAL;
        SN2_TRY(sn2_pack_rows(io->cloud, g->xyz, B, 10, N, g->rows0, cur));
    }
    sn2_sa sa;
    sa1_desc(&sa, m, d, g, a, nograd, nullptr);
    SN2_TRY(sn2_sa_forward(&sa, mode, cur));
    if (join_b) NET_HIP(hipStreamWaitEvent(cur, ctx->b_tables, 0));
    sa2_desc(&sa, m, d, g, a, nograd, nullptr, nullptr);
    SN2_TRY(sn2_sa_forward(&sa, mode, cur));
    if (join_b) NET_HIP(hipStreamWaitEvent(cur, ctx->b_nn, 0));
    sn2_fp p3, pf3;
    fp_desc(&p3, d, a, sa3_in(m, d, g, a), nograd);
    fp_desc(&pf3, d, a, fp3_in(m, d, g, a), nograd);
    if (batch_stats && m->fuse_global_level && io->gl_xchg && io->gl_ctl && B <= GL_MAX_PLOTS && !m->sa3.mma_bf16 &&
        !m->fp3.mma_bf16) {
        SN2_TRY(sn2_global_level_forward(&p3, &pf3, a->x3, a->arg3, io->gl_xchg, io->gl_ctl, cur));
    } else {
        SN2_TRY(sn2_fp_forward(&p3, mode, cur));
        SN2_TRY(sn2_plot_max_forward(a->h_sa3, p3.blk.a, p3.blk.c, B, M2, 64, a->x3, a->arg3, cur));
        SN2_TRY(sn2_fp_forward(&pf3, mode, cur));
    }
    sn2_fp p2;
    fp_desc(&p2, d, a, fp2_in(m, d, g, a, a->src_ws2), nograd);
    SN2_TRY(sn2_fp_forward(&p2, mode, cur));
    if (join_c) NET_HIP(hipStreamWaitEvent(cur, ctx->c_nn, 0));
    sn2_fp p1;
    sn2_head hd;
    if (fused_eval) {
        if (!a->src_ws1) return SN2_EINVAL;
        sn2_net_act a2 = *a;
        a2.h1 = nullptr;
        fp_desc(&p1, d, &a2, fp1_in(m, d, g, &a2, a->src_ws1), nograd);
        head_desc(&hd, m, d, &a2, 0);
        SN2_TRY(sn2_fp_head_eval(&p1, &hd, cur));
    } else {
        fp_desc(&p1, d, a, fp1_in(m, d, g, a, a->src_ws1), nograd);
        SN2_TRY(sn2_fp_forward(&p1, mode, cur));
        head_desc(&hd, m, d, a, batch_stats);
        if (training && a->bwd_arena && a->bwd_arena_words > 0) hd.zero_fill = a->bwd_arena, hd.zero_fill_words = a->bwd_arena_words;
        SN2_TRY(sn2_head_forward(&hd, cur));
    }
    if (join_b) NET_HIP(hipStreamWaitEvent(cur, ctx->b_done, 0));
    if (join_c) NET_HIP(hipStreamWaitEvent(cur, ctx->c_done, 0));
    return 0;
}

extern "C" int sn2_net_backward(const sn2_net_model* m, const sn2_net_dims* d, const sn2_net_geo* g, const sn2_net_act* a,
                                const sn2_net_bwd* b, void* stream) {
    SN2_TRY(check_dims(m, d));
    SN2_TRY(check_model_ptrs(m));
    if (!a || !b) return SN2_EINVAL;
    SN2_TRY(check_geo(d, g));
    if (!g->inv1 || !g->inv2 || !g->inv3) return SN2_EINVAL;
    if (!a->aux || !a->stats || !a->h1 || !a->h2 || !a->h3 || !a->h_sa3 || !a->x3 || !a->arg3) return SN2_EINVAL;
    if (!b->arena || b->images != GRAD_IMAGES || b->image_stride < m->n_flat || !b->dy1 || !b->du1 || !b->du2 || !b->du3 || !b->bn_ok ||
        !b->dy2 || !b->dy3 || !b->dx1 || !b->dx2 || !b->dx3 || !b->dy_sa3 || b->arena_words <= 0)
        return SN2_EINVAL;
    const int B = d->B, M2 = d->M2;
    hipStream_t cur = (hipStream_t)stream;
    if (!b->arena_is_zero) {
        sn2_fill_words(b->arena, 0u, (size_t)b->arena_words, cur);
        NET_HIP(hipGetLastError());
    }
    const GradDst gd{b->arena, b->image_stride, b->frozen_stats ? 1 : 0};
    sn2_head hd;
    head_desc(&hd, m, d, a, b->frozen_stats ? 0 : 1);
    hd.coverages = hd.proba = nullptr;
    hd.dcoverages = b->dcov, hd.dproba = b->dproba, hd.dy = static_cast<float*>(b->dy1);
    hd.dW1 = b->arena + m->g_lin1_W, hd.db1 = b->arena + m->g_lin1_b, hd.dW2 = b->arena + m->g_lin2_W, hd.db2 = b->arena + m->g_lin2_b;
    hd.grad_replicas = GRAD_IMAGES, hd.grad_replica_stride = b->image_stride;
    SN2_TRY(sn2_head_backward(&hd, cur));
    SN2_TRY(sn2_head_bn_sums(&hd, m->fp1.gamma, m->fp1.beta, aux_row(a, 6, 2), aux_row(a, 6, 3), b->arena + m->fp1.ggamma,
                             b->arena + m->fp1.gbeta, b->bn_ok + 0, cur));
    sn2_fp p1;
    fp_desc(&p1, d, a, fp1_in(m, d, g, a, b->src_ws1), gd);
    p1.dy = static_cast<const float*>(b->dy1), p1.dsrc = b->dy2, p1.dsrc_stride = 36, p1.dskip = nullptr, p1.dskip_stride = 0;
    p1.du_scratch = static_cast<float*>(b->du1), p1.scatter_ws = g->inv1, p1.scatter_ready = 1, p1.bn_sums_done = b->bn_ok + 0;
    p1.row_perm = (g->rank1 && p1.src_ws) ? g->rank1 : nullptr;
    SN2_TRY(sn2_fp_backward(&p1, cur));
    SN2_TRY(sn2_fp_bn_sums(&p1, m->fp2.gamma, m->fp2.beta, aux_row(a, 5, 2), aux_row(a, 5, 3), b->arena + m->fp2.ggamma,
                           b->arena + m->fp2.gbeta, b->bn_ok + 1, cur));
    sn2_fp p2;
    fp_desc(&p2, d, a, fp2_in(m, d, g, a, b->src_ws2), gd);
    p2.dy = b->dy2, p2.dsrc = b->dy3, p2.dsrc_stride = 64, p2.dskip = b->dx1, p2.dskip_stride = 16;
    p2.du_scratch = b->du2, p2.scatter_ws = g->inv2, p2.scatter_ready = 1, p2.bn_sums_done = b->bn_ok + 1;
    SN2_TRY(sn2_fp_backward(&p2, cur));
    SN2_TRY(sn2_fp_bn_sums(&p2, m->fp3.gamma, m->fp3.beta, aux_row(a, 4, 2), aux_row(a, 4, 3), b->arena + m->fp3.ggamma,
                           b->arena + m->fp3.gbeta, b->bn_ok + 2, cur));
    sn2_fp pf3;
    fp_desc(&pf3, d, a, fp3_in(m, d, g, a), gd);
    pf3.dy = b->dy3, pf3.dsrc = b->dx3, pf3.dsrc_stride = 64, pf3.dskip = b->dx2, pf3.dskip_stride = 32;
    pf3.du_scratch = b->du3, pf3.scatter_ws = g->inv3, pf3.scatter_ready = -1, pf3.bn_sums_done = b->bn_ok + 2;
    SN2_TRY(sn2_fp_backward(&pf3, cur));
    SN2_TRY(sn2_global_pool_backward(b->du3, 64, a->arg3, a->h_sa3, aux_row(a, 3, 2), aux_row(a, 3, 3), B, M2, 64, b->dx3, b->dy_sa3,
                                     b->arena + m->sa3.ggamma, b->arena + m->sa3.gbeta, cur));
    sn2_fp p3;
    fp_desc(&p3, d, a, sa3_in(m, d, g, a), gd);
    p3.dy = b->dy_sa3, p3.dsrc = b->dx2, p3.dsrc_stride = 32, p3.bn_sums_done = b->bn_ok + 3;
    SN2_TRY(sn2_fp_backward(&p3, cur));
    sn2_sa sa;
    sa2_desc(&sa, m, d, g, a, gd, b->dx2, b->dx1);
    SN2_TRY(sn2_sa_backward(&sa, cur));
    sa1_desc(&sa, m, d, g, a, gd, b->dx1, b->sa1_ws);
    SN2_TRY(sn2_sa_backward(&sa, cur));
    if (b->defer_grad_reduce) return 0;
    return sn2_grad_reduce(b->arena, m->n_flat, GRAD_IMAGES, b->image_stride, cur);
}
```

### stratanet2_vegetation_coverage_maps_amd/executor.py

```python
import ctypes
import weakref
from ctypes import byref

import torch

from . import _lib
from . import hip_ops as ops
from ._lib import NetAct, NetBwd, NetDims, NetGeo, NetIO, NetModel, StrataHipError

F32, I32, I64, BF16, U8 = torch.float32, torch.int32, torch.int64, torch.bfloat16, torch.uint8
_FAKE_BASE = 1 << 40
_ITEM = {F32: 4, I32: 4, I64: 8, BF16: 2, U8: 1}


def _geo_shapes(B, N, M1, M2, cap1, cap2):
    return {
        "idx1": (I32, (B, M1)), "pos1_soa": (F32, (B, 3, M1)), "pos1_aos": (F32, (B * M1, 4)), "ws1": (I32, (ops.fps_ws_words(B, N),)),
        "nbr1": (I32, (B * M1, cap1)), "cnt1": (I32, (B * M1,)), "tot1": (I64, (1,)), "ord1": (I32, (ops.sa_order_len(B, M1),)),
        "idx2": (I32, (B, M2)), "pos2_soa": (F32, (B, 3, M2)), "pos2_aos": (F32, (B * M2, 4)), "ws2": (I32, (ops.fps_ws_words(B, M1),)),
        "nbr2": (I32, (B * M2, cap2)), "cnt2": (I32, (B * M2,)), "tot2": (I64, (1,)), "ord2": (I32, (ops.sa_order_len(B, M2),)),
        "knn3_idx": (I32, (B * M2, 3)), "knn3_w": (F32, (B * M2, 3)), "knn2_idx": (I32, (B * M1, 3)), "knn2_w": (F32, (B * M1, 3)),
        "knn1_idx": (I32, (B * N, 3)), "knn1_w": (F32, (B * N, 3)),
        "inv3": (F32, (ops.interp_ws_words(B, M2, 1),)), "inv2": (F32, (ops.interp_ws_words(B, M1, M2),)),
        "inv1": (F32, (ops.interp_ws_words(B, N, M1),)),
# ... 94 lines not shown

    _PAIRS = {"knn3": ("knn3_idx", "knn3_w"), "knn2": ("knn2_idx", "knn2_w"), "knn1": ("knn1_idx", "knn1_w")}

    def __getattr__(self, name):
        d = self.__dict__
        plan = d.get("plan")
        if plan is None:
            raise AttributeError(name)
        spec = plan.geo_offsets.get(name)
        if spec is not None:
            v = _view(d["arena"], *spec)
        elif name in self._PAIRS:
            v = tuple(getattr(self, n) for n in self._PAIRS[name])
        elif name == "nn_ws":
            v = tuple(getattr(self, n) if n in plan.geo_offsets else None for n in ("nn_ws2", "nn_ws1"))
        elif name == "rank1":
            v = ops.fps_ws_rank(self.ws1, self.B, self.N) if d.get("_want_rank1") else None
        elif name in ("ws1", "ws2", "nn_ws1", "nn_ws2", "p2_pix", "p2_mm"):
            v = None
        else:
            raise AttributeError(name)
        d[name] = v
        return v


def geo_struct(g):
    cg = getattr(g, "cgeo", None)
    if cg is not None:
        return cg
    cg = NetGeo()
    p = lambda t: None if t is None else t.data_ptr()
    for n in ("idx1", "pos1_soa", "pos1_aos", "nbr1", "cnt1", "tot1", "ord1", "idx2", "pos2_soa", "pos2_aos", "nbr2", "cnt2", "tot2",
              "ord2", "inv3", "inv2", "inv1", "rows0"):
        setattr(cg, n, p(getattr(g, n)))
    for n in ("ws1", "ws2", "rank1", "p2_pix", "p2_mm"):
        setattr(cg, n, p(getattr(g, n, None)))
    nn_ws = getattr(g, "nn_ws", None) or (None, None)
    cg.nn_ws2, cg.nn_ws1 = p(nn_ws[0]), p(nn_ws[1])
    for k in ("knn3", "knn2", "knn1"):
        idx, w = getattr(g, k)
        setattr(cg, k + "_idx", idx.data_ptr())
        setattr(cg, k + "_w", w.data_ptr())
    pos3 = getattr(g, "pos3", None)
    if pos3 is None:
        pos3 = g.pos3 = _pos3(g.idx1.device, g.B)
    cg.pos3 = pos3.data_ptr()
    g.cgeo = cg
    return cg


def _check_handle(g, plan, what):
    d = plan.dims
    ok = (g.B, g.N, g.M1, g.M2) == (d.B, d.N, d.M1, d.M2)
    if ok:
        gp = getattr(g, "plan", None)
        if gp is not None:
            ok = gp is plan or (gp.dims.cap1, gp.dims.cap2, gp.geo_bytes) == (d.cap1, d.cap2, plan.geo_bytes) or \
                (gp.dims.cap1, gp.dims.cap2) == (d.cap1, d.cap2) and gp.dims.p2_diam_pix >= d.p2_diam_pix
        else:
            ok = g.nbr1.shape[1] == d.cap1 and g.nbr2.shape[1] == d.cap2
    if not ok:
        raise ValueError(f"{what} do not match this batch")


class NetSaved:

    def __init__(self, plan, geo, arena, cact, training):
        self.plan, self.geo, self.arena, self.cact, self.training = plan, geo, arena, cact, training
        self.B, self.N, self.M1, self.M2 = plan.B, plan.N, plan.M1, plan.M2

    def __getattr__(self, name):
        d = self.__dict__
        plan = d.get("plan")
        if plan is None:
            raise AttributeError(name)
        spec = plan.act_offsets[1 if d["training"] else 0].get(name)
        if spec is not None:
            v = d[name] = _view(d["arena"], *spec)
            return v
        return getattr(d["geo"], name)


_BLOCKS = ("sa1_module.conv.local_nn.0", "sa1_module.conv.local_nn.1", "sa2_module.conv.local_nn.0", "sa3_module.nn.0",
           "fp3_module.nn.0", "fp2_module.nn.0", "fp1_module.nn.0")


class ModelStruct:

    def __init__(self, model, params, max_neighbors):
        offs, n_flat = ops.flat_layout(params)
        off_of = {id(p): o for p, o in zip(params, offs)}
        self.param_offsets, self.n_flat = offs, n_flat
        self.param_shapes = [tuple(p.shape) for p in params]
        self.param_numels = [p.numel() for p in params]
        m = NetModel()
        mods = dict(model.named_modules())
        layers = [m.sa1[0], m.sa1[1], m.sa2, m.sa3, m.fp3, m.fp2, m.fp1]
        self.tensors = []
        for L, name in zip(layers, _BLOCKS):
            blk = mods[name]
            lin, bn = blk[0], blk[2]
            prefix = name.rsplit(".", 1)[0]
            for t in (lin.weight, lin.bias, bn.weight, bn.bias, bn.running_mean, bn.running_var):
                ops._chk(t, F32, None, name)
            L.cin, L.cout = lin.in_features, lin.out_features
            L.W, L.b, L.gamma, L.beta = lin.weight.data_ptr(), lin.bias.data_ptr(), bn.weight.data_ptr(), bn.bias.data_ptr()
            L.running_mean, L.running_var = bn.running_mean.data_ptr(), bn.running_var.data_ptr()
            nbt = bn.num_batches_tracked
            if nbt is not None:
                ops._chk(nbt, I64, None, "num_batches_tracked")
            L.num_batches_tracked = None if nbt is None else nbt.data_ptr()
            L.gW, L.gb, L.ggamma, L.gbeta = (off_of[id(t)] for t in (lin.weight, lin.bias, bn.weight, bn.bias))
            L.mma_bf16 = int(model.mma_dtype == "bf16" and prefix in model.BF16_BLOCKS)
            self.tensors += [lin.weight, lin.bias, bn.weight, bn.bias, bn.running_mean, bn.running_var] + ([nbt] if nbt is not None else [])
        for t, shape in ((model.lin1.weight, (16, 34)), (model.lin1.bias, (16,)), (model.lin2.weight, (5, 16)), (model.lin2.bias, (5,))):
            ops._chk(t, F32, shape, "head parameter")
        m.lin1_W, m.lin1_b, m.lin2_W, m.lin2_b = (t.data_ptr() for t in (model.lin1.weight, model.lin1.bias, model.lin2.weight, model.lin2.bias))
        m.g_lin1_W, m.g_lin1_b, m.g_lin2_W, m.g_lin2_b = (off_of[id(t)] for t in (model.lin1.weight, model.lin1.bias, model.lin2.weight,
                                                                                model.lin2.bias))
        self.tensors += [model.lin1.weight, model.lin1.bias, model.lin2.weight, model.lin2.bias]
        m.n_flat = n_flat
        m.r1_sq, m.r2_sq = ops.r2_threshold(model.sa1_module.r), ops.r2_threshold(model.sa2_module.r)
        m.max_neighbors = int(max_neighbors)
        m.drop_p = float(model.drop)
        m.fuse_global_level, m.fuse_eval_head, m.source_side = int(bool(model.fuse_global_level)), int(bool(model.fuse_eval_head)), int(bool(ops.SOURCE_SIDE))
        m.fps_waves_shared, m.fps_waves_many = int(model.fps_waves_shared), int(model.fps_waves_many)
        self.c = m
        self.settings = settings_of(model, max_neighbors)
        self.key = tuple(t.data_ptr() for t in self.tensors)
        self.plans = {}
        dev = model.lin1.weight.device
        if any(t.device != dev for t in self.tensors):
            raise StrataHipError("PointNet2: parameters and buffers must live on one HIP device")

    def current(self, model, max_neighbors):
        return self.settings == settings_of(model, max_neighbors) and self.key == tuple(t.data_ptr() for t in self.tensors)

    def plan(self, model, B, N):
        k = (B, N)
        p = self.plans.get(k)
        if p is None:
            if len(self.plans) > 32:
                self.plans.clear()
            p = self.plans[k] = Plan(model, self.c, B, N, self.c.max_neighbors)
        return p


def settings_of(model, max_neighbors):
    return (model.mma_dtype, float(model.drop), bool(model.fuse_global_level), bool(model.fuse_eval_head), bool(ops.SOURCE_SIDE),
            int(model.fps_waves_shared), int(model.fps_waves_many), float(model.sa1_module.r), float(model.sa2_module.r),
            float(model.sa1_module.ratio), float(model.sa2_module.ratio), int(max_neighbors), model.p2_diam_pix,
            bool(model.fp1_morton_rows))


class NetCtx:

    def __init__(self):
        h = ctypes.c_void_p()
        _lib.check(_lib.load().sn2_net_ctx_create(byref(h)), "sn2_net_ctx_create")
        self.handle = h.value
        self._fin = weakref.finalize(self, _destroy_ctx, self.handle)


def _destroy_ctx(handle):
    try:
        _lib.load().sn2_net_ctx_destroy(handle)
    except Exception:
        pass


def _io(model, dev, training, flags, cloud=None, fps_start=None, fork=False):
    io = NetIO()
    io.cloud = None if cloud is None else cloud.data_ptr()
    io.fps_start = None if fps_start is None else fps_start.data_ptr()
    io.fps_status = ops.fps_status_word(dev).data_ptr()
    io.training = int(training) if training in (0, 1, 2) else int(bool(training))
    if fork:
        io.stream_b = ops.shared_stream(dev, "fork_b").cuda_stream
        io.stream_c = ops.shared_stream(dev, "fork_c").cuda_stream
        io.stream_pack = ops.shared_stream(dev, "pack").cuda_stream
        io.ctx = model._net_ctx().handle
    io.flags = flags
    return io


def geometry(model, ms, xyz, fps_start, out=None, fork=None, shared=False, defer_join=False, inverted=True, cloud=None):
    dev = xyz.device
    B, _, N = xyz.shape
    ops._chk(xyz, F32, (B, 3, N), "xyz")
    ops._chk(fps_start, I32, (2, B), "fps_start")
    plan = ms.plan(model, B, N)
    g = out if out is not None else ArenaGeometry(plan, dev, model)
    _check_handle(g, plan, "geometry buffers")
    cg = geo_struct(g)
    g.xyz = xyz
    cg.xyz = xyz.data_ptr()
    fork = model.geometry_fork if fork is None else fork
    flags = (_lib.NET_FORK if fork else 0) | (_lib.NET_SHARED if shared else 0) | (_lib.NET_INVERTED if inverted else 0)
    if fork and defer_join:
        flags |= _lib.NET_DEFER_JOIN
    if cloud is not None:
        ops._chk(cloud, F32, (B, 10, N), "cloud")
        flags |= _lib.NET_INPUT_ONLY
    io = _io(model, dev, model.training, flags, cloud=cloud, fps_start=fps_start, fork=fork)
    _lib.check(_lib.load().sn2_net_geometry(byref(ms.c), byref(plan.dims), byref(cg), byref(io), ops._stream()), "sn2_net_geometry")
    g.has_inverted = bool(inverted)
    g.has_rows0 = cloud is not None
    if cloud is not None and plan.dims.p2_diam_pix > 0 and getattr(g, "p2_pix", None) is not None:
        g.p2_diam_pix = int(plan.dims.p2_diam_pix)
    g._join = "ctx" if (fork and defer_join) else None
    return g


def forward(model, ms, xyz, cloud, fps_start, training, geo=None, drop_keep=None, need_grad=True):
    dev = xyz.device
    B, _, N = xyz.shape
    ops._chk(xyz, F32, (B, 3, N), "xyz")
    ops._chk(cloud, F32, (B, 10, N), "cloud")
    plan = ms.plan(model, B, N)
    lib = _lib.load()
    fork = False
    frozen = (not training) and bool(need_grad)
    keep = bool(training) or frozen
    mode = 1 if training else (_lib.BN_FROZEN_KEEP if frozen else 0)
    if geo is None:
        ops._chk(fps_start, I32, (2, B), "fps_start")
        geo = ArenaGeometry(plan, dev, model)
        fork = bool(model.geometry_fork)
        flags = _lib.NET_WITH_GEOMETRY | (_lib.NET_FORK if fork else 0)
        geo.has_inverted = keep
        fs = fps_start
    else:
        _check_handle(geo, plan, "prefetched geometry tables")
        flags, fs = 0, None
        if getattr(geo, "has_rows0", False):
            flags |= _lib.NET_HAS_ROWS0
        if getattr(geo, "_join", None) is not None:
            flags |= _lib.NET_JOIN_PENDING
            geo._join = None
            fork = True
        if getattr(geo, "has_inverted", True):
            flags |= _lib.NET_HAS_INVERTED
    cg = geo_struct(geo)
    geo.xyz = xyz
    cg.xyz = xyz.data_ptr()
    t = 1 if keep else 0
    arena = torch.empty(plan.act_bytes[t], dtype=U8, device=dev)
    ca = NetAct()
    base = arena.data_ptr()
    for name, (off, _, _) in plan.act_offsets[t].items():
        setattr(ca, name, base + off)
    cov = torch.empty(B * N, 4, dtype=F32, device=dev)
    proba = torch.empty(B * N, 4, dtype=F32, device=dev)
    ca.cov, ca.proba = cov.data_ptr(), proba.data_ptr()
    if drop_keep is not None:
        ops._chk(drop_keep, I32, (B * N,), "drop_mask")
        ca.drop_mask = drop_keep.data_ptr()
    bwd_arena = None
    if keep and need_grad:
        bwd_arena = torch.empty(plan.bwd_arena_words, dtype=F32, device=dev)
        ca.bwd_arena, ca.bwd_arena_words = bwd_arena.data_ptr(), plan.bwd_arena_words
    io = _io(model, dev, mode, flags, cloud=cloud, fps_start=fs, fork=fork)
    if training and model.fuse_global_level:
        ws = ops.global_level_ws(dev, owner=model)
        io.gl_xchg, io.gl_ctl = ws[0].data_ptr(), ws[1].data_ptr()
    _lib.check(lib.sn2_net_forward(byref(ms.c), byref(plan.dims), byref(cg), byref(ca), byref(io), ops._stream()), "sn2_net_forward")
    geo.has_rows0 = True
    if keep:
        geo.has_inverted = True
    s = NetSaved(plan, geo, arena, ca, keep)
    s.frozen = frozen
    s.drop_keep = drop_keep
    s.xyz = xyz
    s.ms = ms
    s.bwd_arena = bwd_arena
    return cov, proba, s


def backward(model, s, dcov, dproba):
    plan, ms = s.plan, s.ms
    dev = s.xyz.device
    R = plan.B * plan.N
    arena = s.__dict__.get("bwd_arena")
    s.bwd_arena = None
    pre_zeroed = arena is not None
    if arena is None:
        arena = torch.empty(plan.bwd_arena_words, dtype=F32, device=dev)
    scratch = torch.empty(plan.bwd_scratch_bytes, dtype=U8, device=dev)
    cb = NetBwd()
    sz, sz2 = ctypes.c_size_t(), ctypes.c_size_t()
    lib = _lib.load()
    _lib.check(lib.sn2_net_bwd_carve(byref(ms.c), byref(plan.dims), arena.data_ptr(), scratch.data_ptr(), byref(cb), byref(sz), byref(sz2)),
               "sn2_net_bwd_carve")
    if dcov is not None:
        dcov = ops._chk(dcov.contiguous(), F32, (R, 4), "dcoverages")
        cb.dcov = dcov.data_ptr()
    if dproba is not None:
        dproba = ops._chk(dproba.contiguous(), F32, (R, 4), "dproba")
        cb.dproba = dproba.data_ptr()
    defer = bool(getattr(model, "defer_grad_reduce", False))
    cb.defer_grad_reduce = int(defer)
    cb.arena_is_zero = int(pre_zeroed)
    cb.frozen_stats = int(bool(s.__dict__.get("frozen", False)))
    _lib.check(lib.sn2_net_backward(byref(ms.c), byref(plan.dims), byref(geo_struct(s.geo)), byref(s.cact), byref(cb), ops._stream()),
               "sn2_net_backward")
    flat = arena[:ms.n_flat]
    s.flat_grad = flat
    model._last_flat_grad = flat
    model._grad_images_pending = (arena, cb.images, cb.image_stride) if defer else None
    return [p if len(shape) == 1 else p.view(shape) for p, shape in zip(flat.split(ms.param_numels), ms.param_shapes)]
```

### stratanet2_vegetation_coverage_maps_amd/hip_ops.py

```python
import math
from typing import Optional

import numpy as np
import torch

from . import _lib
from ._lib import FP, SA, Block, Head, StrataHipError, check

I32, F32, F64, I64, BF16 = torch.int32, torch.float32, torch.float64, torch.int64, torch.bfloat16


_timing = None


class timing:

    def __init__(self, names=None):
        self.names = None if names is None else set(names)
        self.events = []

    def __enter__(self):
        global _timing
        self._prev, _timing = _timing, self
        return self
# ... 512 lines not shown
    return int(_lib.load().sn2_parcel_count_ws_words(int(P), int(rows)))


def parcel_znorm_ws_words(T: int, radius: float, x_min: float, y_min: float, x_max: float, y_max: float) -> int:
    return int(_lib.load().sn2_parcel_znorm_ws_words(int(T), float(radius), float(x_min), float(y_min), float(x_max),
                                                     float(y_max)))


def _chk_center_grid(grid, P: int):
    start, items, GX, GY, gx0, gy0, inv = grid
    _chk(start, I32, (GX * GY + 1,), "cell_start")
    _chk(items, I32, None, "cell_items")
    if items.dim() != 1 or items.numel() < 1 or items.numel() > P:
        raise ValueError("cell_items: expected 1..P centre ids")
    return start, items, int(GX), int(GY), float(gx0), float(gy0), float(inv)


def parcel_count(cloud: torch.Tensor, centers: torch.Tensor, grid, radius: float, L: int, rows: int):
    _, T = cloud.shape
    _chk(cloud, F32, (10, T), "cloud")
    P = centers.shape[0]
    _chk(centers, F32, (P, 2), "centers")
    start, items, GX, GY, gx0, gy0, inv = _chk_center_grid(grid, P)
    dev = cloud.device
    nw = parcel_count_ws_words(P, rows)
    ws = torch.empty(nw + 4, dtype=I32, device=dev)
    prefix = torch.empty(P * rows + 1, dtype=I32, device=dev)
    total = torch.empty(1, dtype=I64, device=dev)
    _call("sn2_parcel_count", _ptr(cloud), T, int(L), int(rows), _ptr(centers), P, _ptr(start), _ptr(items), GX, GY, gx0, gy0,
          inv, float(radius), _ptr(ws), nw, _ptr(prefix), _ptr(total), _stream())
    return prefix, total


def parcel_fill(cloud: torch.Tensor, centers: torch.Tensor, grid, radius: float, L: int, rows: int, prefix: torch.Tensor,
                plot_base: torch.Tensor, sum_n: int):
    _, T = cloud.shape
    _chk(cloud, F32, (10, T), "cloud")
    P = centers.shape[0]
    _chk(centers, F32, (P, 2), "centers")
    start, items, GX, GY, gx0, gy0, inv = _chk_center_grid(grid, P)
    _chk(prefix, I32, (P * rows + 1,), "prefix")
    _chk(plot_base, I32, (P,), "plot_base")
    dev = cloud.device
    raw = torch.empty(10, sum_n, dtype=F32, device=dev)
    pidx = torch.empty(sum_n, dtype=I32, device=dev)
    _call("sn2_parcel_fill", _ptr(cloud), T, int(L), int(rows), _ptr(centers), P, _ptr(start), _ptr(items), GX, GY, gx0, gy0,
          inv, float(radius), _ptr(prefix), _ptr(plot_base), int(sum_n), _ptr(raw), _ptr(pidx), _stream())
    return raw, pidx


def parcel_znorm(cloud: torch.Tensor, bbox, radius: float, disc_radius: float, offsets: torch.Tensor, centers: torch.Tensor,
                 point_index: torch.Tensor, raw: torch.Tensor):
    _, T = cloud.shape
    _chk(cloud, F32, (10, T), "cloud")
    P = centers.shape[0]
    _chk(centers, F32, (P, 2), "centers")
    _chk(offsets, I32, (P + 1,), "offsets")
    sum_n = point_index.shape[0]
    _chk(point_index, I32, (sum_n,), "point_index")
    _chk(raw, F32, (10, sum_n), "raw")
    nw = parcel_znorm_ws_words(T, radius, *bbox)
    if nw == 0:
        raise ValueError("parcel_znorm: the parcel's extent needs more than 2^26 cells of the z-norm radius")
    ws = torch.empty(nw + 4, dtype=I32, device=cloud.device)
    _call("sn2_parcel_znorm", _ptr(cloud), T, *[float(v) for v in bbox], float(radius), float(disc_radius), _ptr(offsets),
          _ptr(centers), P, _ptr(point_index), sum_n, _ptr(ws), nw, _ptr(raw), _stream())
    return raw


def sa_order_len(B: int, M: int) -> int:
    return 4 * B * M + 16 * B * (M // 8 + 2) + 8


def sa_order(cnt: torch.Tensor, B: int, M: int, out: Optional[torch.Tensor] = None) -> torch.Tensor:
    _chk(cnt, I32, (B * M,), "cnt")
    n = sa_order_len(B, M)
    if out is None:
        out = torch.empty(n, dtype=I32, device=cnt.device)
    else:
        _chk(out, I32, (n,), "out order")
    _call("sn2_sa_order", _ptr(cnt), B, M, _ptr(out), _stream())
    return out


def sa_order_group(cnt: torch.Tensor, G: int, B: int, M: int, out_all: torch.Tensor, stride: int):
    _chk(cnt, I32, (G * B * M,), "cnt")
    if stride < sa_order_len(B, M):
        raise ValueError("sa_order_group: stride smaller than a table")
    _chk(out_all, I32, (G * stride,), "out order tables")
    _call("sn2_sa_order_group", _ptr(cnt), G, B, M, _ptr(out_all), stride, _stream(), key="sn2_sa_order")


SA_BWD_WS_WORDS = 32 * 2 * 16 * 12


def sa_desc(blocks, feat, cf, spos, cpos_aos, nbr, cnt, total, B, Nsrc, M, ext, arg, out, dout=None, dfeat=None,
            with_grads=False, order=None, bwd_ws=None) -> SA:
    cap = nbr.shape[1]
    cl = blocks[-1].cout
    feat_stride = _chk_rows(feat, F32, B * Nsrc, cf, "feat")
    spos_stride = _chk_rows(spos, F32, B * Nsrc, 4, "spos")
    _chk(cpos_aos, F32, (B * M, 4), "cpos_aos")
    _chk(nbr, I32, (B * M, cap), "nbr")
    _chk(cnt, I32, (B * M,), "cnt")
    _chk(total, I64, (1,), "total")
    _chk(ext, F32, (B * M, cl), "ext")
    _chk(arg, I32, (B * M, cl), "arg")
    _chk(out, F32, (B * M, cl), "out")
    d = SA()
    d.B, d.Nsrc, d.M, d.cap, d.cf, d.nl = B, Nsrc, M, cap, cf, len(blocks)
    d.feat, d.feat_stride, d.spos, d.spos_stride = _ptr(feat), feat_stride, _ptr(spos), spos_stride
    d.cpos, d.nbr, d.cnt, d.total = _ptr(cpos_aos), _ptr(nbr), _ptr(cnt), _ptr(total)
    if order is not None:
        _chk(order, I32, (sa_order_len(B, M),), "order")
    d.order = _ptr(order)
    for i, bb in enumerate(blocks):
        bb.fill(d.blk[i], with_grads)
    d.ext, d.arg, d.out = _ptr(ext), _ptr(arg), _ptr(out)
    if dout is not None:
        _chk(dout, F32, (B * M, cl), "dout")
    if dfeat is not None:
        _chk(dfeat, F32, (B * Nsrc, cf), "dfeat")
    if bwd_ws is not None:
        _chk(bwd_ws, F32, (SA_BWD_WS_WORDS,), "bwd_ws")
    d.dout, d.dfeat, d.bwd_ws = _ptr(dout), _ptr(dfeat), _ptr(bwd_ws)
    return d


def sa_forward(d: SA, training: bool):
    _call("sn2_sa_forward", d, int(training), _stream(), tag=f"cf={d.cf}")


def sa_backward(d: SA):
    _call("sn2_sa_backward", d, _stream(), tag=f"cf={d.cf}")


def interp_ws_words(B: int, R_per_plot: int, S_per_plot: int) -> int:
    return (B * S_per_plot * ((R_per_plot + 2047) // 2048 + 6) + 6 * B * R_per_plot + 64
            + 4 * B * interp_chunks(R_per_plot, S_per_plot))


def interp_chunks(R_per_plot: int, S_per_plot: int) -> int:
    return (3 * R_per_plot + 62) // 63 + S_per_plot


def interp_index(knn, B: int, R_per_plot: int, S_per_plot: int, out: Optional[torch.Tensor] = None,
                 src_pos: Optional[torch.Tensor] = None, row_perm: Optional[torch.Tensor] = None) -> torch.Tensor:
    if src_pos is not None:
        _chk(src_pos, F32, (B * S_per_plot, 4), "src_pos")
    if row_perm is not None:
        _chk(row_perm, I32, (B * R_per_plot,), "row_perm")
    R = B * R_per_plot
    _chk(knn[0], I32, (R, 3), "knn_idx")
    _chk(knn[1], F32, (R, 3), "knn_w")
    n = interp_ws_words(B, R_per_plot, S_per_plot)
    if out is None:
        out = torch.empty(n, dtype=F32, device=knn[0].device)
    else:
        _chk(out, F32, (n,), "out index")
    _call("sn2_interp_index_perm", _ptr(knn[0]), _ptr(knn[1]), _ptr(src_pos), _ptr(row_perm), B, R_per_plot, S_per_plot, _ptr(out),
          _stream(), key="sn2_interp_index")
    return out


def interp_index_group(knn, G: int, B: int, R_per_plot: int, S_per_plot: int, out_all: torch.Tensor, stride: int,
                       src_pos: Optional[torch.Tensor] = None, row_perm: Optional[torch.Tensor] = None):
    R = G * B * R_per_plot
    _chk(knn[0], I32, (R, 3), "knn_idx")
    _chk(knn[1], F32, (R, 3), "knn_w")
    if src_pos is not None:
        _chk(src_pos, F32, (G * B * S_per_plot, 4), "src_pos")
    if row_perm is not None:
        _chk(row_perm, I32, (R,), "row_perm")
    if stride % 4 or stride < interp_ws_words(B, R_per_plot, S_per_plot):
        raise ValueError("interp_index_group: stride must be a multiple of 4 words and hold one index")
    _chk(out_all, F32, (G * stride,), "out indices")
    _call("sn2_interp_index_group", _ptr(knn[0]), _ptr(knn[1]), _ptr(src_pos), _ptr(row_perm), G, B, R_per_plot, S_per_plot, _ptr(out_all),
          stride, _stream(), key="sn2_interp_index")


SOURCE_SIDE = True


def fp_desc(block: BlockBuffers, B, R_per_plot, S_per_plot, ca, cb, src, h, src_affine=None, knn=None, skip=None,
            dy=None, dsrc=None, dskip=None, du_scratch=None, with_grads=False, interp_index=None,
            bn_sums_done=None, row_perm=None, force_src_ws=False, gather=True) -> FP:
    R = B * R_per_plot
    hs = (block.cout + 3) // 4 * 4
    AT = BF16 if (h is not None and h.dtype == BF16) else F32
    n_src_rows = R if knn is None else B * S_per_plot
    src_stride = _chk_rows(src, F32, n_src_rows, ca, "src")
    if src.shape[1] < (ca + 3) // 4 * 4 and src_stride < (ca + 3) // 4 * 4:
        raise ValueError("fp: src rows must be padded to a multiple of 4 floats")
    if h is not None or not force_src_ws:
        _chk(h, AT, (R, hs), "h")
    d = FP()
    d.B, d.R_per_plot, d.S_per_plot, d.ca, d.cb = B, R_per_plot, S_per_plot, ca, cb
    d.src, d.src_stride = _ptr(src), src_stride
    if src_affine is not None:
        _chk(src_affine[0], F32, (ca,), "src_a")
        _chk(src_affine[1], F32, (ca,), "src_c")
        d.src_a, d.src_c = _ptr(src_affine[0]), _ptr(src_affine[1])
    else:
        d.src_a = d.src_c = None
    if knn is not None:
        _chk(knn[0], I32, (R, 3), "knn_idx")
        _chk(knn[1], F32, (R, 3), "knn_w")
        d.knn_idx, d.knn_w = _ptr(knn[0]), _ptr(knn[1])
    else:
        d.knn_idx = d.knn_w = None
    if cb > 0:
        d.skip_stride = _chk_rows(skip, F32, R, cb, "skip", align=4 if cb % 4 == 0 else 1)
        d.skip = _ptr(skip)
    else:
        d.skip, d.skip_stride = None, 0
    block.fill(d.blk, with_grads)
    if R > 64 * _lib.STAT_SLOTS:
        d.blk.mma_bf16 = 0
    d.h, d.h_stride = _ptr(h), hs
    if dy is not None:
        _chk(dy, AT, (R, hs), "dy")
    d.dsrc_stride = d.dskip_stride = 0
    if dsrc is not None:
        d.dsrc_stride = _chk_rows(dsrc, F32, n_src_rows, ca, "dsrc", align=1)
    if dskip is not None:
        d.dskip_stride = _chk_rows(dskip, F32, R, cb, "dskip", align=1)
    d.scatter_ws, d.scatter_ready = None, 0
    if bn_sums_done is not None:
        _chk(bn_sums_done, I32, (1,), "bn_sums_done")
    d.bn_sums_done = _ptr(bn_sums_done)
    d._src_ws = None
    if SOURCE_SIDE and knn is not None and 0 < cb <= 16 and cb % 4 == 0 and (R > 64 * _lib.STAT_SLOTS or force_src_ws):
        d._src_ws = torch.empty(B * interp_chunks(R_per_plot, S_per_plot) * hs, dtype=F32, device=src.device)
    d.src_ws = _ptr(d._src_ws)
    d.row_perm = None
    if row_perm is not None and d._src_ws is not None and du_scratch is not None:
        _chk(row_perm, I32, (R,), "row_perm")
        d.row_perm = _ptr(row_perm)
    d.act_bf16 = int(AT == BF16)
    if d.act_bf16 and d._src_ws is None:
        raise ValueError("fp: bfloat16 activation rows need the source-side form (a k-NN layer of more than 65 536 rows)")
    if du_scratch is not None:
        _chk(du_scratch, AT, (R, max(ca, hs)), "du_scratch")
        if knn is not None and dsrc is not None:
            words = interp_ws_words(B, R_per_plot, S_per_plot)
            if interp_index is not None:
                _chk(interp_index, F32, (words,), "interp_index")
                d._scatter_ws, d.scatter_ready = interp_index, 1
            else:
                d._scatter_ws = torch.empty(words, dtype=F32, device=src.device)
            d.scatter_ws = _ptr(d._scatter_ws)
            if not gather:
                d.scatter_ready = -1
    d.dy, d.dsrc, d.dskip, d.du_scratch = _ptr(dy), _ptr(dsrc), _ptr(dskip), _ptr(du_scratch)
    return d


def fp_bn_sums(d: FP, gamma, beta, mean, invstd, dgamma, dbeta, ok):
    for t, n in ((gamma, "gamma"), (beta, "beta"), (mean, "mean"), (invstd, "invstd"), (dgamma, "dgamma"), (dbeta, "dbeta")):
        _chk(t, F32, (d.ca,), n)
    _chk(ok, I32, (1,), "ok")
    _call("sn2_fp_bn_sums", d, _ptr(gamma), _ptr(beta), _ptr(mean), _ptr(invstd), _ptr(dgamma), _ptr(dbeta), _ptr(ok), _stream())


def fp_forward(d: FP, training: bool):
    _call("sn2_fp_forward", d, int(training), _stream(), tag=f"{d.ca}+{d.cb}->{d.blk.cout}")


def fp_backward(d: FP):
    _call("sn2_fp_backward", d, _stream(), tag=f"{d.ca}+{d.cb}->{d.blk.cout}")


def plot_max_forward(h, a, c, B, R_per_plot, C):
    hs = (C + 3) // 4 * 4
    _chk(h, F32, (B * R_per_plot, hs), "h")
    _chk(a, F32, (C,), "a")
    _chk(c, F32, (C,), "c")
    out = torch.empty(B, C, dtype=F32, device=h.device)
    arg = torch.empty(B, C, dtype=I32, device=h.device)
    _call("sn2_plot_max_forward", _ptr(h), _ptr(a), _ptr(c), B, R_per_plot, C, _ptr(out), _ptr(arg), _stream())
    return out, arg


GL_MAX_PLOTS = 28
_GLOBAL_WS = {}
_GLOBAL_WS_ALL = []


class _GlobalWs(list):
    __slots__ = ("__weakref__",)


def global_level_ws(dev, B: int = GL_MAX_PLOTS, owner=None):
    dev = torch.device(dev)
    if B > GL_MAX_PLOTS:
        raise ValueError(f"global_level_forward takes at most {GL_MAX_PLOTS} plots")
    key = dev.index if dev.index is not None else torch.cuda.current_device()
    store = _GLOBAL_WS if owner is None else owner.__dict__.setdefault("_gl_ws", {})
    ws = store.get(key)
    if ws is None:
        if torch.cuda.is_current_stream_capturing():
            raise StrataHipError("global_level_forward: its exchange area must exist before a stream capture starts -- run one "
                                 "eager training forward first (TrainPipeline.capture does) or call hip_ops.global_level_ws(dev, owner=model)")
        ws = _GlobalWs([torch.zeros(2 * GL_MAX_PLOTS * 4 * 128, dtype=I64, device=dev), torch.zeros(8, dtype=I32, device=dev), 0])
        store[key] = ws
        import weakref
        _GLOBAL_WS_ALL[:] = [r for r in _GLOBAL_WS_ALL if r() is not None]
        _GLOBAL_WS_ALL.append(weakref.ref(ws))
    return ws


def global_level_forward(d_sa3: FP, d_fp3: FP, x3: torch.Tensor, arg3: torch.Tensor, owner=None):
    B = d_sa3.B
    _chk(x3, F32, (B, 64), "x3")
    _chk(arg3, I32, (B, 64), "arg3")
    ws = global_level_ws(x3.device, B, owner=owner)
    _call("sn2_global_level_forward", d_sa3, d_fp3, _ptr(x3), _ptr(arg3), _ptr(ws[0]), _ptr(ws[1]), _stream())


def global_level_gave_up(dev, warn: bool = True) -> int:
    dev = torch.device(dev)
    key = dev.index if dev.index is not None else torch.cuda.current_device()
    total = 0
    for r in list(_GLOBAL_WS_ALL):
        ws = r()
        if ws is None or ws[1].device.index != key:
            continue
        n = int(ws[1][1].item())
        total += n
        if n > ws[2]:
            seen, ws[2] = ws[2], n
            if warn:
                import warnings
                warnings.warn(f"global_level_forward: {n - seen} exchange wait(s) gave up on {dev}; those launches were repeated "
                              "by the single-workgroup repair launch (results unaffected, the passes took longer); set "
                              "PointNet2.fuse_global_level = False where other kernels or processes share the device",
                              StrataHipWarning, stacklevel=2)
    return total


def plot_max_backward(dout, arg, B, R_per_plot, C, dy):
    hs = (C + 3) // 4 * 4
    _chk(dout, F32, (B, C), "dout")
    _chk(arg, I32, (B, C), "arg")
    _chk(dy, F32, (B * R_per_plot, hs), "dy")
    _call("sn2_plot_max_backward", _ptr(dout), _ptr(arg), B, R_per_plot, C, _ptr(dy), _stream())


def global_pool_backward(du, arg, h, mean, invstd, B, R_per_plot, dx, dy, dgamma, dbeta):
    _chk(du, F32, (B * R_per_plot, 64), "du")
    _chk(arg, I32, (B, 64), "arg")
    _chk(h, F32, (B * R_per_plot, 64), "h")
    for t, n in ((mean, "mean"), (invstd, "invstd"), (dgamma, "dgamma"), (dbeta, "dbeta")):
        _chk(t, F32, (64,), n)
    _chk(dx, F32, (B, 64), "dx")
    _chk(dy, F32, (B * R_per_plot, 64), "dy")
    _call("sn2_global_pool_backward", _ptr(du), 64, _ptr(arg), _ptr(h), _ptr(mean), _ptr(invstd), B, R_per_plot, 64, _ptr(dx), _ptr(dy),
          _ptr(dgamma), _ptr(dbeta), _stream())


def dropout_mask_words(keep: torch.Tensor) -> torch.Tensor:
    if keep.dim() != 2 or keep.shape[1] != 16:
        raise ValueError("dropout mask must be (rows, 16)")
    pow2 = (2 ** torch.arange(16, device=keep.device, dtype=torch.int32))
    return ((keep != 0).to(torch.int32) * pow2).sum(1, dtype=torch.int32).contiguous()


def head_desc(f, fa, fc, lin1, lin2, coverages=None, proba=None, dcov=None, dproba=None, dy=None, grads=None,
              grad_images=(1, 0), drop_mask=None, drop_p: float = 0.0, rows: Optional[int] = None) -> Head:
    if f is None:
        if rows is None or coverages is None:
            raise ValueError("head_desc: without f the row count and the outputs must be given")
        R, AT = int(rows), F32
    else:
        R = f.shape[0]
        AT = BF16 if f.dtype == BF16 else F32
        _chk(f, AT, (R, 36), "f")
    _chk(fa, F32, (34,), "fa")
    _chk(fc, F32, (34,), "fc")
    _chk(lin1.weight, F32, (16, 34), "lin1.weight")
    _chk(lin1.bias, F32, (16,), "lin1.bias")
    _chk(lin2.weight, F32, (5, 16), "lin2.weight")
    _chk(lin2.bias, F32, (5,), "lin2.bias")
    d = Head()
    d.R, d.cin, d.f_stride = R, 34, 36
    d.f, d.fa, d.fc = _ptr(f), _ptr(fa), _ptr(fc)
    d.W1, d.b1, d.W2, d.b2 = _ptr(lin1.weight), _ptr(lin1.bias), _ptr(lin2.weight), _ptr(lin2.bias)
    for t, n in ((coverages, "coverages"), (proba, "proba"), (dcov, "dcoverages"), (dproba, "dproba")):
        if t is not None:
            _chk(t, F32, (R, 4), n)
    d.coverages, d.proba, d.dcoverages, d.dproba = _ptr(coverages), _ptr(proba), _ptr(dcov), _ptr(dproba)
    if dy is not None:
        _chk(dy, AT, (R, 36), "dy")
    d.dy = _ptr(dy)
    d.act_bf16 = int(AT == BF16)
    if grads is not None:
        for t, ref in zip(grads, (lin1.weight, lin1.bias, lin2.weight, lin2.bias)):
            _chk(t, F32, ref.shape, "head grad view")
        d.dW1, d.db1, d.dW2, d.db2 = (_ptr(t) for t in grads)
        d.grad_replicas, d.grad_replica_stride = grad_images
    else:
        d.dW1 = d.db1 = d.dW2 = d.db2 = None
        d.grad_replicas, d.grad_replica_stride = 1, 0
    if drop_mask is not None:
        _chk(drop_mask, I32, (R,), "drop_mask")
        d.drop_mask, d.drop_scale = _ptr(drop_mask), (1.0 / (1.0 - drop_p) if drop_p < 1.0 else 0.0)
    else:
        d.drop_mask, d.drop_scale = None, 1.0
    return d


GRAD_IMAGES = 32


def flat_layout(params):
    offs, o = [], 0
    for p in params:
        offs.append(o)
        o += p.numel()
    return offs, o


def grad_images_alloc(n_flat: int, device, extra_words: int = 0):
    stride = (n_flat + 63) // 64 * 64
    arena = torch.zeros(GRAD_IMAGES * stride + extra_words, dtype=F32, device=device)
    return arena, arena[:n_flat], (GRAD_IMAGES, stride), arena[GRAD_IMAGES * stride:]


def grad_reduce(arena, n_flat: int, images):
    replicas, stride = images
    _chk(arena, F32, None, "arena")
    if arena.numel() < replicas * stride:
        raise ValueError("grad_reduce: arena smaller than its images")
    _call("sn2_grad_reduce", _ptr(arena), n_flat, replicas, stride, _stream())


def fp_head_eval(d: FP, hd: Head):
    _call("sn2_fp_head_eval", d, hd, _stream())


def head_forward(d: Head):
    _call("sn2_head_forward", d, _stream())


def head_backward(d: Head):
    _call("sn2_head_backward", d, _stream())


def head_bn_sums(d: Head, gamma, beta, mean, invstd, dgamma, dbeta, ok):
    for t, n in ((gamma, "gamma"), (beta, "beta"), (mean, "mean"), (invstd, "invstd"), (dgamma, "dgamma"), (dbeta, "dbeta")):
        _chk(t, F32, (d.cin,), n)
    _chk(ok, I32, (1,), "ok")
    _call("sn2_head_bn_sums", d, _ptr(gamma), _ptr(beta), _ptr(mean), _ptr(invstd), _ptr(dgamma), _ptr(dbeta), _ptr(ok), _stream())


def _xy_rows(clouds_dev: torch.Tensor):
    B, C, N = clouds_dev.shape
    _chk(clouds_dev, F32, (B, C, N), "clouds")
    if C < 2:
        raise ValueError("clouds needs at least the x and y rows")
    return clouds_dev, C * N


def plot_project_forward(pred_pointwise: torch.Tensor, clouds_dev: torch.Tensor, diam_pix: int):
    B, C, N = clouds_dev.shape
    _chk(pred_pointwise, F32, (B * N, 4), "pred_pointwise")
    t, stride = _xy_rows(clouds_dev)
    dev = pred_pointwise.device
    D = int(diam_pix)
    keys = torch.empty(B * D * D * 3, dtype=I64, device=dev)
    pix = torch.empty(B * N, dtype=I32, device=dev)
    arg = torch.empty(B * D * D * 3, dtype=I32, device=dev)
    nocc = torch.empty(B, dtype=I32, device=dev)
    pred = torch.empty(B, 4, dtype=F32, device=dev)
    _call("sn2_plot_project_forward", _ptr(pred_pointwise), _ptr(t), stride, B, N, D, _ptr(keys), _ptr(pix),
                                               _ptr(arg), _ptr(nocc), _ptr(pred), _stream())
    return pred, pix, arg, nocc


def p2_key_parts(N: int) -> int:
    return max(1, min(64, (N + 4095) // 4096))


def plot_pixels(clouds_dev: torch.Tensor, diam_pix: int, out=None):
    B, C, N = clouds_dev.shape
    t, stride = _xy_rows(clouds_dev)
    if out is None:
        mm = torch.empty(B, 4, dtype=F32, device=clouds_dev.device)
        pix = torch.empty(B * N, dtype=I32, device=clouds_dev.device)
    else:
        mm, pix = out
        _chk(mm, F32, (B, 4), "out mm")
        _chk(pix, I32, (B * N,), "out pix")
    _call("sn2_plot_pixels", _ptr(t), stride, B, N, int(diam_pix), _ptr(mm), _ptr(pix), _stream())
    return mm, pix


def plot_project_forward_pix(pred_pointwise: torch.Tensor, pix: torch.Tensor, B: int, N: int, diam_pix: int):
    _chk(pred_pointwise, F32, (B * N, 4), "pred_pointwise")
    _chk(pix, I32, (B * N,), "pix")
    dev = pred_pointwise.device
    D = int(diam_pix)
    keys = torch.empty(p2_key_parts(N) * B * D * D * 3, dtype=I64, device=dev)
    arg = torch.empty(B * D * D * 3, dtype=I32, device=dev)
    nocc = torch.empty(B, dtype=I32, device=dev)
    pred = torch.empty(B, 4, dtype=F32, device=dev)
    _call("sn2_plot_project_forward_pix", _ptr(pred_pointwise), _ptr(pix), B, N, D, _ptr(keys), _ptr(arg), _ptr(nocc), _ptr(pred),
          _stream(), key="sn2_plot_project_forward")
    return pred, pix, arg, nocc


def plot_project_backward(dpred, arg, nocc, pix, B, N, diam_pix):
    D = int(diam_pix)
    _chk(dpred, F32, (B, 4), "dpred")
    _chk(arg, I32, (B * D * D * 3,), "arg")
    _chk(nocc, I32, (B,), "nocc")
    _chk(pix, I32, (B * N,), "pix")
    dpw = torch.empty(B * N, 4, dtype=F32, device=dpred.device)
    _call("sn2_plot_project_backward", _ptr(dpred), _ptr(arg), _ptr(nocc), _ptr(pix), B, N, D, _ptr(dpw), _stream())
    return dpw


def raster_project(coverages: torch.Tensor, clouds_dev: torch.Tensor, diam_pix: int, diam_meters: int):
    B, C, N = clouds_dev.shape
    _chk(coverages, F32, (B * N, 4), "coverages")
    t, stride = _xy_rows(clouds_dev)
    dev = coverages.device
    D = int(diam_pix)
    keys = torch.empty(B * D * D * 3, dtype=I64, device=dev)
    pix = torch.empty(B * N, dtype=I32, device=dev)
    rasters = torch.empty(B, 3, D, D, dtype=F32, device=dev)
    _call("sn2_raster_project", _ptr(coverages), _ptr(t), stride, B, N, D, int(diam_meters), _ptr(keys),
                                         _ptr(pix), _ptr(rasters), _stream())
    return rasters, pix


def mosaic_merge(rasters, weights, offsets, mean, wsum, window=None):
    B, _, D, _ = rasters.shape
    _, H, W = mean.shape
    _chk(rasters, F32, (B, 3, D, D), "rasters")
    _chk(weights, F32, (D, D), "weights")
    _chk(offsets, I32, (B, 2), "offsets")
    _chk(mean, F32, (3, H, W), "mean")
    _chk(wsum, F32, (3, H, W), "wsum")
    y0, x0, wh, ww = (0, 0, H, W) if window is None else [int(v) for v in window]
    _call("sn2_mosaic_merge", _ptr(rasters), _ptr(weights), _ptr(offsets), B, D, H, W, _ptr(mean), _ptr(wsum),
          y0, x0, wh, ww, _stream())


def mosaic_finalize(mean: torch.Tensor, wsum: torch.Tensor):
    _, H, W = mean.shape
    _chk(mean, F32, (3, H, W), "mean")
    _chk(wsum, F32, (H, W), "wsum")
    dev = mean.device
    hist = torch.empty(10004, dtype=I32, device=dev)
    acc = torch.empty(1, dtype=F64, device=dev)
    thr = torch.empty(2, dtype=F32, device=dev)
    out = torch.empty(5, H, W, dtype=F32, device=dev)
    _call("sn2_mosaic_finalize", _ptr(mean), _ptr(wsum), H, W, _ptr(hist), _ptr(acc), _ptr(thr), _ptr(out), _stream())
    return out, thr


LOSS_BLOCKS = 1024


def kde_lookup(clouds_dev: torch.Tensor, z_max: float, X: torch.Tensor, Y: torch.Tensor, z_channel: int = 2) -> torch.Tensor:
    B, C, N = clouds_dev.shape
    _chk(clouds_dev, F32, (B, C, N), "clouds")
    K = X.shape[0]
    _chk(X, F64, (K,), "X")
    _chk(Y, F64, (3, K), "Y")
    if K < 2 or not (0 <= z_channel < C):
        raise ValueError("kde_lookup: need K >= 2 knots and a valid z channel")
    pdf = torch.empty(B * N, 3, dtype=F64, device=clouds_dev.device)
    _call("sn2_kde_lookup", _ptr(clouds_dev), B, C, N, int(z_channel), float(z_max), _ptr(X), _ptr(Y), K, _ptr(pdf), _stream())
    return pdf


KDE_FIT_MAX_K = 65536


def kde_fit_ws_words(K: int) -> int:
    K = max(int(K), 2)
    return 2 * ((4 + 3 * 8) * K + 3 * ((K + 255) // 256)) + 256


def kde_fit(z_dev: torch.Tensor, bw: float = 0.1, grid_points: int = 5000):
    _chk(z_dev, F32, None, "z")
    if z_dev.dim() != 1:
        raise ValueError(f"z: expected a 1-D tensor of heights, got {tuple(z_dev.shape)}")
    K = int(grid_points)
    dev = z_dev.device
    ws = torch.empty(kde_fit_ws_words(K) // 2 + 1, dtype=F64, device=dev)
    X = torch.empty(max(K, 2), dtype=F64, device=dev)
    Y = torch.empty(3, max(K, 2), dtype=F64, device=dev)
    _call("sn2_kde_fit", _ptr(z_dev) or None, z_dev.numel(), float(bw), K, _ptr(ws), _ptr(X), _ptr(Y), _stream())
    return X, Y


def loss_forward(pred, gt, proba, pdf, m: float, e: float):
    B, R = pred.shape[0], proba.shape[0]
    _chk(pred, F32, (B, 4), "pred")
    _chk(gt, F64, (B, 4), "gt")
    _chk(proba, F32, (R, 4), "proba")
    _chk(pdf, F64, (R, 3), "pdf")
    partials = torch.empty(2 * LOSS_BLOCKS, dtype=F64, device=pred.device)
    out = torch.empty(4, dtype=F64, device=pred.device)
    _call("sn2_loss_forward", _ptr(pred), _ptr(gt), B, _ptr(proba), _ptr(pdf), R, float(m), float(e), _ptr(partials),
          _ptr(out), _stream())
    return out


def loss_backward(pred, gt, proba, pdf, m: float, e: float, grad_total):
    B, R = pred.shape[0], proba.shape[0]
    _chk(grad_total, F64, None, "grad_total")
    dpred = torch.empty(B, 4, dtype=F32, device=pred.device)
    dproba = torch.empty(R, 4, dtype=F32, device=pred.device)
    _call("sn2_loss_backward", _ptr(pred), _ptr(gt), B, _ptr(proba), _ptr(pdf), R, float(m), float(e), _ptr(grad_total),
          _ptr(dpred), _ptr(dproba), _stream())
    return dpred, dproba


PROJECTED_LOSS_WS = 2 * 512 + 2


def projected_loss_forward(cov, pix, proba, pdf, gt, B: int, N: int, diam_pix: int, m: float, e: float):
    R, D = B * N, int(diam_pix)
    _chk(cov, F32, (R, 4), "coverages")
    _chk(pix, I32, (R,), "pix")
    _chk(proba, F32, (R, 4), "proba")
    _chk(pdf, F64, (R, 3), "pdf")
    _chk(gt, F64, (B, 4), "gt")
    dev = cov.device
    keys = torch.empty(p2_key_parts(N) * B * D * D * 3, dtype=I64, device=dev)
    arg = torch.empty(B * D * D * 3, dtype=I32, device=dev)
    nocc = torch.empty(B, dtype=I32, device=dev)
    pred = torch.empty(B, 4, dtype=F32, device=dev)
    partials = torch.empty(PROJECTED_LOSS_WS, dtype=F64, device=dev)
# ... 103 lines not shown
```

### stratanet2_vegetation_coverage_maps_amd/point_net2.py

```python
import os
from collections import OrderedDict

import torch
import torch.nn as nn
from torch.nn import BatchNorm1d as BN
from torch.nn import Linear as Lin
from torch.nn import ReLU
from torch.nn import Sequential as Seq

from . import executor as X
from . import hip_ops as ops
from ._lib import BN_FROZEN_KEEP, MAX_NEIGHBORS as _MAXN, STAT_SLOTS, StrataHipError

MAX_NEIGHBORS = _MAXN

F32, I32, I64, F64 = torch.float32, torch.int32, torch.int64, torch.float64


def MLP(channels):
    return Seq(*[Seq(Lin(channels[i - 1], channels[i]), ReLU(), BN(channels[i])) for i in range(1, len(channels))])


class PointConv(nn.Module):

# ... 320 lines not shown
            if inverted:
                ops.interp_index(g.knn3, B, M2, 1, out=g.inv3)
                ops.interp_index(g.knn2, B, M1, M2, out=g.inv2)
        with torch.cuda.stream(sc):
            ops.three_nn(g.pos1_soa, xyz, 3, out=g.knn1, ws=g.nn_ws[1])
            if inverted:
                ops.interp_index(g.knn1, B, N, M1, out=g.inv1, src_pos=g.pos1_aos, row_perm=g.rank1)
        g.has_inverted = bool(inverted)
        g.has_rows0 = False
        if cloud is not None:
            self._input_only(g, cloud, xyz)
        ops.ball_query(xyz, g.pos1_soa, self.sa1_module.r, MAX_NEIGHBORS, g.tot1 if inverted else False, fps_ws=g.ws1, out=(g.nbr1, g.cnt1))
        ops.sa_order(g.cnt1, B, M1, out=g.ord1)
        g._join = None
        if fork and defer_join:
            g._join = (sb, sc)
        elif fork:
            cur.wait_stream(sb)
            cur.wait_stream(sc)
        return g

    def alloc_geometry_pair(self, B, N, device=None, group=2):
        dev = torch.device(device if device is not None else self.lin1.weight.device)
        M1, M2 = self._sizes(N)
        gp = self.alloc_geometry(group * B, N, dev)
        e = lambda *shape, dt=F32: torch.empty(*shape, dtype=dt, device=dev)
        up4 = lambda n: (n + 3) // 4 * 4
        so1, so2 = ops.sa_order_len(B, M1), ops.sa_order_len(B, M2)
        si = [up4(ops.interp_ws_words(B, R, S)) for R, S in ((M2, 1), (M1, M2), (N, M1))]
        grp = _Saved()
        grp.G, grp.so1, grp.so2, grp.si = group, so1, so2, si
        grp.ord1, grp.ord2 = e(group * so1, dt=I32), e(group * so2, dt=I32)
        grp.inv = [e(group * w) for w in si]
        grp.totals = torch.zeros(group, 2, dtype=I64, device=dev)
        gp._grp = grp
        halves = []
        for h in range(group):
            g = _Saved()
            g.B, g.N, g.M1, g.M2 = B, N, M1, M2
            pl, r1, r2, rn = slice(h * B, (h + 1) * B), slice(h * B * M1, (h + 1) * B * M1), \
                slice(h * B * M2, (h + 1) * B * M2), slice(h * B * N, (h + 1) * B * N)
            g.idx1, g.pos1_soa, g.pos1_aos, g.nbr1, g.cnt1 = gp.idx1[pl], gp.pos1_soa[pl], gp.pos1_aos[r1], gp.nbr1[r1], gp.cnt1[r1]
            g.idx2, g.pos2_soa, g.pos2_aos, g.nbr2, g.cnt2 = gp.idx2[pl], gp.pos2_soa[pl], gp.pos2_aos[r2], gp.nbr2[r2], gp.cnt2[r2]
            g.knn3 = (gp.knn3[0][r2], gp.knn3[1][r2])
            g.knn2 = (gp.knn2[0][r1], gp.knn2[1][r1])
            g.knn1 = (gp.knn1[0][rn], gp.knn1[1][rn])
            g.totals = grp.totals[h]
            g.tot1, g.tot2 = grp.totals[h, 0:1], grp.totals[h, 1:2]
            g.ord1, g.ord2 = grp.ord1[h * so1:(h + 1) * so1], grp.ord2[h * so2:(h + 1) * so2]
            g.inv3, g.inv2, g.inv1 = (grp.inv[k][h * si[k]:h * si[k] + ops.interp_ws_words(B, R, S)]
                                      for k, (R, S) in enumerate(((M2, 1), (M1, M2), (N, M1))))
            g.ws1 = g.ws2 = g.nn_ws = None
            g.rank1 = gp.rank1[rn] if (gp.rank1 is not None and self._fp1_source_side(B * N)) else None
            g.rows0, g.has_rows0 = gp.rows0[rn], False
            g.p2_pix = gp.p2_pix[rn] if gp.p2_pix is not None else None
            g.p2_mm = gp.p2_mm[pl] if gp.p2_mm is not None else None
            g.p2_diam_pix = None
            g.ready = None
            halves.append(g)
        return gp, tuple(halves)

    def _geometry_pair(self, xyz2, fps_start2, gp, halves, clouds=None, cloud2=None):
        B2, _, N = xyz2.shape
        B = B2 // len(halves)
        M1, M2 = self._sizes(N)
        if (gp.B, gp.N) != (B2, N):
            raise ValueError("geometry buffers do not match this batch pair")
        ops.fps(xyz2, M1, fps_start2[0], out=(gp.idx1, gp.pos1_soa, gp.pos1_aos, gp.ws1), waves=self.fps_waves_shared)
        ops.ball_query(xyz2, gp.pos1_soa, self.sa1_module.r, MAX_NEIGHBORS, False, fps_ws=gp.ws1, out=(gp.nbr1, gp.cnt1))
        ops.fps(gp.pos1_soa, M2, fps_start2[1], out=(gp.idx2, gp.pos2_soa, gp.pos2_aos, gp.ws2))
        ops.ball_query(gp.pos1_soa, gp.pos2_soa, self.sa2_module.r, MAX_NEIGHBORS, False, fps_ws=gp.ws2,
                       out=(gp.nbr2, gp.cnt2))
        ops.three_nn(gp.pos3, gp.pos2_soa, 1, out=gp.knn3)
        ops.three_nn(gp.pos2_soa, gp.pos1_soa, 3, out=gp.knn2, ws=gp.nn_ws[0])
        ops.three_nn(gp.pos1_soa, xyz2, 3, out=gp.knn1, ws=gp.nn_ws[1])
        grp, G = gp._grp, len(halves)
        tot_flat = grp.totals.view(-1)
        ops.count_sum_group(gp.cnt1, G, B * M1, tot_flat, 2)
        ops.count_sum_group(gp.cnt2, G, B * M2, tot_flat[1:], 2)
        ops.sa_order_group(gp.cnt1, G, B, M1, grp.ord1, grp.so1)
        ops.sa_order_group(gp.cnt2, G, B, M2, grp.ord2, grp.so2)
        ops.interp_index_group(gp.knn3, G, B, M2, 1, grp.inv[0], grp.si[0])
        ops.interp_index_group(gp.knn2, G, B, M1, M2, grp.inv[1], grp.si[1])
        rank = gp.rank1 if halves[0].rank1 is not None else None
        ops.interp_index_group(gp.knn1, G, B, N, M1, grp.inv[2], grp.si[2], src_pos=gp.pos1_aos, row_perm=rank)
        if cloud2 is not None:
            self._input_only(gp, cloud2, xyz2)
        for h, g in enumerate(halves):
            g.xyz = xyz2[h * B:(h + 1) * B]
            g.has_rows0 = cloud2 is not None
            g.p2_diam_pix = gp.p2_diam_pix if cloud2 is not None else None
            g.has_inverted = True
            if clouds is not None and cloud2 is None:
                self._input_only(g, clouds[h], g.xyz)
        return halves

    def prefetch_geometry(self, cloud_data, lane: int = 0):
        dev = self.lin1.weight.device
        if dev.type != "cuda":
            raise StrataHipError("prefetch_geometry needs a HIP device")
        with torch.cuda.device(dev):
            xyz_d, fs = self._stage_positions(cloud_data, dev)
            side = ops.shared_stream(dev, f"side{lane}")
            side.wait_stream(torch.cuda.current_stream())
            xyz_d.record_stream(side)
            fs.record_stream(side)
            with torch.cuda.stream(side):
                cl = cloud_data.get("cloud", None) if isinstance(cloud_data, dict) else None
                cl = cl if (isinstance(cl, torch.Tensor) and cl.is_cuda and cl.dtype == F32 and cl.is_contiguous()) else None
                g = self._geometry(xyz_d, fs, shared=True, fork=False, inverted=self.training, cloud=cl)
                g.fps_start = fs
                g.ready = torch.cuda.Event()
                g.ready.record(side)
            g.stream = side
        return g

    def _stage_positions(self, cloud_data, dev, ring=None):
        xyz = cloud_data["xyz"]
        if ring is not None and not xyz.is_cuda:
            xyz_d = ring.upload(xyz, dtype=F32)
        else:
            xyz_d = xyz.to(device=dev, dtype=F32, non_blocking=True).contiguous()
        B, _, N = xyz_d.shape
        fs = cloud_data.get("fps_start", None) if isinstance(cloud_data, dict) else None
        if fs is None:
            m1 = ops.fps_num_samples(N, self.sa1_module.ratio)
            fs = torch.stack([torch.randint(0, N, (B,)), torch.randint(0, m1, (B,))])
        fs = torch.as_tensor(fs).to(device=dev, dtype=I32, non_blocking=True).contiguous()
        if fs.shape != (2, B):
            raise ValueError(f"fps_start must have shape (2,{B})")
        return xyz_d, fs

    def _forward_impl(self, xyz, cloud, fps_start, training, geo=None, drop_keep=None, need_grad=True):
        if self._use_executor():
            cov, proba, s = X.forward(self, self._net_model(), xyz, cloud, fps_start, training, geo, drop_keep, need_grad=need_grad)
            if self.log_embeddings:
                self.last_G_tensor = s.x3
            return cov, proba, s
        dev = xyz.device
        B, _, N = xyz.shape
        M1, M2 = self._sizes(N)
        cur_stream = torch.cuda.current_stream(dev)
        frozen = (not training) and bool(need_grad)
        keep = bool(training) or frozen
        mode = 1 if training else (BN_FROZEN_KEEP if frozen else 0)
        rows0, packed = None, None
        if geo is not None and getattr(geo, "has_rows0", False) and geo.rows0.shape[0] == B * N:
            rows0 = geo.rows0
        if geo is None:
            if self.geometry_fork:
                rows0 = torch.empty(B * N, 12, dtype=F32, device=dev)
                pack_stream = ops.shared_stream(dev, "pack")
                pack_stream.wait_stream(cur_stream)
                with torch.cuda.stream(pack_stream):
                    ops.pack_rows(cloud, xyz, out=rows0)
                    packed = torch.cuda.Event()
                    packed.record(pack_stream)
            geo = self._geometry(xyz, fps_start, defer_join=True, inverted=keep)
        elif (geo.B, geo.N, geo.M1, geo.M2) != (B, N, M1, M2):
            raise ValueError("prefetched geometry does not match this batch")
        join = getattr(geo, "_join", None)
        geo._join = None
        if join == "ctx":
            raise StrataHipError("a geometry pass launched by the executor with a deferred join must be consumed by the executor")
        if keep and not getattr(geo, "has_inverted", True):
            if join is not None:
                cur_stream.wait_stream(join[0])
                cur_stream.wait_stream(join[1])
                join = None
            ops.count_sum(geo.cnt1, geo.tot1)
            ops.count_sum(geo.cnt2, geo.tot2)
            ops.interp_index(geo.knn3, B, M2, 1, out=geo.inv3)
            ops.interp_index(geo.knn2, B, M1, M2, out=geo.inv2)
            ops.interp_index(geo.knn1, B, N, M1, out=geo.inv1, src_pos=geo.pos1_aos, row_perm=getattr(geo, "rank1", None))
            geo.has_inverted = True
        s = _Saved()
        s.__dict__.update({k: v for k, v in geo.__dict__.items()
                           if k not in ("ready", "stream", "ws1", "ws2", "totals", "nn_ws", "fps_start", "_join", "has_rows0")})
        s.xyz = xyz
        widths = [16, 16, 32, 64, 64, 34, 34]
        aux = torch.empty(4 * sum(widths), dtype=F32, device=dev)
        stats = torch.empty(STAT_SLOTS * 2 * sum(widths), dtype=F32, device=dev)
        cur = [0, 0]
        bf = lambda prefix: self.mma_dtype == "bf16" and prefix in self.BF16_BLOCKS
        s.b_sa1 = _blocks_of(self.sa1_module.conv.local_nn, aux, stats, cur, bf("sa1_module.conv.local_nn"))
        s.b_sa2 = _blocks_of(self.sa2_module.conv.local_nn, aux, stats, cur, bf("sa2_module.conv.local_nn"))
        s.b_sa3 = _blocks_of(self.sa3_module.nn, aux, stats, cur, bf("sa3_module.nn"))[0]
        s.b_fp3 = _blocks_of(self.fp3_module.nn, aux, stats, cur, bf("fp3_module.nn"))[0]
        s.b_fp2 = _blocks_of(self.fp2_module.nn, aux, stats, cur, bf("fp2_module.nn"))[0]
        s.b_fp1 = _blocks_of(self.fp1_module.nn, aux, stats, cur)[0]
        s.aux, s.stats = aux, stats
        for bb in s.b_sa1 + s.b_sa2 + [s.b_sa3, s.b_fp3, s.b_fp2, s.b_fp1]:
            bb.frozen = frozen

        if packed is not None:
            cur_stream.wait_event(packed)
            s.rows0 = rows0
        elif rows0 is not None:
            s.rows0 = rows0
        else:
            s.rows0 = ops.pack_rows(cloud, xyz)
        s.ext1 = torch.empty(B * M1, 16, dtype=F32, device=dev)
        s.arg1 = torch.empty(B * M1, 16, dtype=I32, device=dev)
        s.x1 = torch.empty(B * M1, 16, dtype=F32, device=dev)
        ops.sa_forward(self._sa1_desc(s), mode)
        if join is not None:
            cur_stream.wait_stream(join[0])
        s.ext2 = torch.empty(B * M2, 32, dtype=F32, device=dev)
        s.arg2 = torch.empty(B * M2, 32, dtype=I32, device=dev)
        s.x2 = torch.empty(B * M2, 32, dtype=F32, device=dev)
        ops.sa_forward(self._sa2_desc(s), mode)
        s.h_sa3 = torch.empty(B * M2, 64, dtype=F32, device=dev)
        s.h3 = torch.empty(B * M2, 64, dtype=F32, device=dev)
        if training and self.fuse_global_level and B <= 28 and not (s.b_sa3.mma_bf16 or s.b_fp3.mma_bf16):
            s.x3 = torch.empty(B, 64, dtype=F32, device=dev)
            s.arg3 = torch.empty(B, 64, dtype=I32, device=dev)
            ops.global_level_forward(self._sa3_desc(s), self._fp3_desc(s), s.x3, s.arg3, owner=self)
        else:
            ops.fp_forward(self._sa3_desc(s), mode)
            s.x3, s.arg3 = ops.plot_max_forward(s.h_sa3, s.b_sa3.a, s.b_sa3.c, B, M2, 64)
            ops.fp_forward(self._fp3_desc(s), mode)
        if self.log_embeddings:
            self.last_G_tensor = s.x3
        s.h2 = torch.empty(B * M1, 36, dtype=F32, device=dev)
        ops.fp_forward(self._fp2_desc(s), mode)
        if join is not None:
            cur_stream.wait_stream(join[1])
        cov = torch.empty(B * N, 4, dtype=F32, device=dev)
        proba = torch.empty(B * N, 4, dtype=F32, device=dev)
        s.drop_keep = drop_keep
        if not keep and self.fuse_eval_head and self._act_dtype(B * N) == F32 and ops.SOURCE_SIDE:
            s.h1 = None
            d1 = ops.fp_desc(s.b_fp1, B, N, M1, 34, 8, s.h2, None, src_affine=(s.b_fp2.a, s.b_fp2.c), knn=s.knn1,
                             skip=s.rows0[:, 0:8], force_src_ws=True)
            ops.fp_head_eval(d1, ops.head_desc(None, s.b_fp1.a, s.b_fp1.c, self.lin1, self.lin2, cov, proba, rows=B * N))
            return cov, proba, s
        s.h1 = torch.empty(B * N, 36, dtype=self._act_dtype(B * N), device=dev)
        ops.fp_forward(self._fp1_desc(s), mode)
        ops.head_forward(ops.head_desc(s.h1, s.b_fp1.a, s.b_fp1.c, self.lin1, self.lin2, cov, proba, drop_mask=drop_keep,
                                       drop_p=self.drop))
        return cov, proba, s

    def _sa1_desc(self, s, dout=None, g=False, bwd_ws=None):
        return ops.sa_desc(s.b_sa1, s.rows0[:, 0:8], 8, s.rows0[:, 8:12], s.pos1_aos, s.nbr1, s.cnt1, s.tot1, s.B, s.N,
                           s.M1, s.ext1, s.arg1, s.x1, dout=dout, dfeat=None, with_grads=g, order=getattr(s, "ord1", None),
                           bwd_ws=bwd_ws)

    def _sa2_desc(self, s, dout=None, dfeat=None, g=False):
        return ops.sa_desc(s.b_sa2, s.x1, 16, s.pos1_aos, s.pos2_aos, s.nbr2, s.cnt2, s.tot2, s.B, s.M1, s.M2, s.ext2,
                           s.arg2, s.x2, dout=dout, dfeat=dfeat, with_grads=g, order=getattr(s, "ord2", None))

    def _sa3_desc(self, s, **kw):
        return ops.fp_desc(s.b_sa3, s.B, s.M2, s.M2, 32, 3, s.x2, s.h_sa3, skip=s.pos2_aos, **kw)

    def _fp3_desc(self, s, **kw):
        return ops.fp_desc(s.b_fp3, s.B, s.M2, 1, 64, 32, s.x3, s.h3, knn=s.knn3, skip=s.x2, **kw)

    def _fp2_desc(self, s, **kw):
        return ops.fp_desc(s.b_fp2, s.B, s.M1, s.M2, 64, 16, s.h3, s.h2, src_affine=(s.b_fp3.a, s.b_fp3.c), knn=s.knn2,
                           skip=s.x1, **kw)

    def _fp1_desc(self, s, **kw):
        return ops.fp_desc(s.b_fp1, s.B, s.N, s.M1, 34, 8, s.h2, s.h1, src_affine=(s.b_fp2.a, s.b_fp2.c), knn=s.knn1,
                           skip=s.rows0[:, 0:8], row_perm=getattr(s, "rank1", None), **kw)

    def _backward_impl(self, s, dcov, dproba):
        if isinstance(s, X.NetSaved):
            return X.backward(self, s, dcov, dproba)
        dev = s.xyz.device
        B, N, M1, M2 = s.B, s.N, s.M1, s.M2
        params = self._params()
        sizes = OrderedDict(dy2=B * M1 * 36, dy3=B * M2 * 64, dx1=B * M1 * 16, dx2=B * M2 * 32, dx3=B * 64,
                            dy_sa3=B * M2 * 64, sa1_ws=ops.SA_BWD_WS_WORDS)
        flat, buf, views, images, arena = self._grad_arena(params, sizes, dev)

        def attach(bb):
            bb.grads = (views[id(bb.lin.weight)], views[id(bb.lin.bias)], views[id(bb.bn.weight)], views[id(bb.bn.bias)])
            bb.grad_images = images

        for bb in s.b_sa1 + s.b_sa2 + [s.b_sa3, s.b_fp3, s.b_fp2, s.b_fp1]:
            attach(bb)
        dcov = None if dcov is None else dcov.contiguous()
        dproba = None if dproba is None else dproba.contiguous()
        dy1 = torch.empty(B * N, 36, dtype=s.h1.dtype, device=dev)
        hg = (views[id(self.lin1.weight)], views[id(self.lin1.bias)], views[id(self.lin2.weight)], views[id(self.lin2.bias)])
        hd = ops.head_desc(s.h1, s.b_fp1.a, s.b_fp1.c, self.lin1, self.lin2, dcov=dcov, dproba=dproba, dy=dy1, grads=hg,
                           grad_images=images, drop_mask=getattr(s, "drop_keep", None), drop_p=self.drop)
        ops.head_backward(hd)
        bn1 = self.fp1_module.nn[0][2]
        bn_ok = torch.empty(4, dtype=I32, device=dev)
        ops.head_bn_sums(hd, bn1.weight.detach(), bn1.bias.detach(), s.b_fp1.aux[2], s.b_fp1.aux[3], views[id(bn1.weight)],
                         views[id(bn1.bias)], bn_ok[0:1])
        dy2 = buf["dy2"].view(B * M1, 36)
        d1 = self._fp1_desc(s, dy=dy1, dsrc=dy2, du_scratch=torch.empty(B * N, 36, dtype=s.h1.dtype, device=dev), with_grads=True,
                            interp_index=s.inv1, bn_sums_done=bn_ok[0:1])
        ops.fp_backward(d1)
        bn2 = self.fp2_module.nn[0][2]
        ops.fp_bn_sums(d1, bn2.weight.detach(), bn2.bias.detach(), s.b_fp2.aux[2], s.b_fp2.aux[3], views[id(bn2.weight)],
                       views[id(bn2.bias)], bn_ok[1:2])
        dy3, dx1 = buf["dy3"].view(B * M2, 64), buf["dx1"].view(B * M1, 16)
        d2 = self._fp2_desc(s, dy=dy2, dsrc=dy3, dskip=dx1, du_scratch=torch.empty(B * M1, 64, dtype=F32, device=dev),
                            with_grads=True, interp_index=s.inv2, bn_sums_done=bn_ok[1:2])
        ops.fp_backward(d2)
        bn3 = self.fp3_module.nn[0][2]
        ops.fp_bn_sums(d2, bn3.weight.detach(), bn3.bias.detach(), s.b_fp3.aux[2], s.b_fp3.aux[3], views[id(bn3.weight)],
                       views[id(bn3.bias)], bn_ok[2:3])
        dx3, dx2 = buf["dx3"].view(B, 64), buf["dx2"].view(B * M2, 32)
        du3 = torch.empty(B * M2, 64, dtype=F32, device=dev)
        ops.fp_backward(self._fp3_desc(s, dy=dy3, dsrc=dx3, dskip=dx2, du_scratch=du3, with_grads=True,
                                       interp_index=s.inv3, bn_sums_done=bn_ok[2:3], gather=False))
        dy_sa3 = buf["dy_sa3"].view(B * M2, 64)
        bn_sa3 = self.sa3_module.nn[0][2]
        ops.global_pool_backward(du3, s.arg3, s.h_sa3, s.b_sa3.aux[2], s.b_sa3.aux[3], B, M2, dx3, dy_sa3,
                                 views[id(bn_sa3.weight)], views[id(bn_sa3.bias)])
        ops.fp_backward(self._sa3_desc(s, dy=dy_sa3, dsrc=dx2, with_grads=True, bn_sums_done=bn_ok[3:4]))
        ops.sa_backward(self._sa2_desc(s, dout=dx2, dfeat=dx1, g=True))
        ops.sa_backward(self._sa1_desc(s, dout=dx1, g=True, bwd_ws=buf["sa1_ws"]))
        if getattr(self, "defer_grad_reduce", False):
            self._grad_images_pending = (arena,) + tuple(images)
        else:
            ops.grad_reduce(arena, flat.numel(), images)
            self._grad_images_pending = None
        s.flat_grad = flat
        self._last_flat_grad = flat
        return [views[id(p)] for p in params]

    @staticmethod
    def _grad_arena(params, sizes, dev):
        poffs, n_flat = ops.flat_layout(params)
        offs, tot = {}, 0
        for k, n in sizes.items():
            offs[k] = tot
            tot += (n + 3) // 4 * 4
        arena, flat, images, extra = ops.grad_images_alloc(n_flat, dev, tot)
        buf = {k: extra[offs[k]:offs[k] + n] for k, n in sizes.items()}
        views = {id(p): flat[o:o + p.numel()].view(p.shape) for p, o in zip(params, poffs)}
        return flat, buf, views, images, arena

    @staticmethod
    def get_long_form(data):
        B, f, N = data.shape
        return data.permute(1, 0, 2).reshape(f, B * N).transpose(1, 0)

    def get_batch_format(self, data):
        n = self.subsample_size
        return data.view(-1, n, data.shape[1]).transpose(1, 2)

    def set_patience_attributes(self, args):
        self.stopped_early = False
        self.best_metric_value = 10 ** 6
        self.best_metric_epoch = 1
        self.patience_in_epochs = args.patience_in_epochs

    def stop_early(self, val_metric, epoch, args):
        if val_metric < self.best_metric_value:
            self.best_metric_value, self.best_metric_epoch = val_metric, epoch
            self.save_state(args)
            return False
        if epoch < args.epoch_to_start_early_stop:
            return False
        if epoch >= self.best_metric_epoch + self.patience_in_epochs:
            self.stopped_early = True
            return True
        return False

    @staticmethod
    def _checkpoint_path(args):
        tag = f"fold_n={args.current_fold_id}" if args.current_fold_id > 0 else "full"
        return os.path.join(args.stats_path, f"PCC_model_{tag}.pt")

    def save_state(self, args):
        torch.save({"best_metric_epoch": self.best_metric_epoch, "state_dict": self.state_dict(),
                    "best_metric_value": self.best_metric_value}, self._checkpoint_path(args))

    def load_state(self, save_path):
        checkpoint = torch.load(save_path, map_location=None if self.cuda_device is not None else torch.device("cpu"))
        self.load_state_dict(checkpoint["state_dict"])
        self.best_metric_epoch = checkpoint["best_metric_epoch"]
        self.best_metric_value = checkpoint["best_metric_value"]
        return self

    def load_best_state(self, args):
        return self.load_state(self._checkpoint_path(args))
```

Before: 23610 plots/s.

## Fuse global-level backward (fp3 BN sums, fp3 bwd, pool bwd, sa3 bwd) into one kernel

Adds a single persistent kernel for the backward of the global level. It fuses fp3's BN-gradient sums, the fp3 backward, the global max-pool backward and the sa3 backward, using cross-workgroup exchange through tagged atomic slots (shared with the forward's gl_collect). It replaces four or five launches and the du3/dy_sa3 round trips through HBM. It applies only when B<=28, M2<=256, stats are not frozen and bf16 MMA is off, and falls back otherwise. It risks spin-wait stalls if the workgroups are not co-resident.

Measured after the change: 23910 plots/s, median of 6. 1.01x the previous value.

```diff
diff --git a/include/strata_hip.h b/include/strata_hip.h
--- a/include/strata_hip.h
+++ b/include/strata_hip.h
@@ -171,6 +171,10 @@
 #define SN2_GLOBAL_CTL_WORDS 8
 int sn2_global_level_forward(const sn2_fp *sa3, const sn2_fp *fp3, float *x3, int *arg3, unsigned long long *xchg,
                              unsigned *ctl, void *stream);
+#define SN2_GLOBAL_BWD_XCHG_WORDS ((size_t)2 * 28 * 128)
+#define SN2_GLOBAL_BWD_CTL_WORDS 64
+int sn2_global_level_backward(const sn2_fp *sa3, const sn2_fp *fp3, const int *arg3, unsigned long long *xchg, unsigned *ctl,
+                              void *stream);
 int sn2_debug_global_spin_limit(unsigned sweeps);
 
 typedef struct sn2_head {
@@ -326,6 +330,7 @@
     int defer_grad_reduce;
     int arena_is_zero;
     int frozen_stats;
+    unsigned long long *gl_xchg; unsigned *gl_ctl;
 } sn2_net_bwd;
 
 #define SN2_NET_FORK 1
diff --git a/stratanet2_vegetation_coverage_maps_amd/_build.py b/stratanet2_vegetation_coverage_maps_amd/_build.py
--- a/stratanet2_vegetation_coverage_maps_amd/_build.py
+++ b/stratanet2_vegetation_coverage_maps_amd/_build.py
@@ -7,9 +7,9 @@
 CSRC = os.path.join(HERE, "csrc")
 LIB = os.path.join(CSRC, "libstrata_hip.so")
 VARIANT_DIR = os.path.join(os.path.dirname(HERE), "build", "variants")
-SOURCES = ["geometry.hip", "sa.hip", "sa_mfma.hip", "fp.hip", "interp_index.hip", "global_level.hip", "head.hip", "project.hip",
+SOURCES = ["geometry.hip", "sa.hip", "sa_mfma.hip", "fp.hip", "interp_index.hip", "global_level.hip", "global_level_bwd.hip", "head.hip", "project.hip",
            "loss.hip", "misc.hip", "net.hip", "parcel.hip", "sample.hip", "kde.hip"]
-HEADERS = ["common.h", "mlp.h", "fp_rows.h", os.path.join("..", "..", "include", "strata_hip.h")]
+HEADERS = ["common.h", "mlp.h", "fp_rows.h", "global_level.h", os.path.join("..", "..", "include", "strata_hip.h")]
 FLAGS = ["--offload-arch=gfx950", "-O3", "-fPIC", "-std=c++17", "-Wno-unused-result"] + os.environ.get("SN2_EXTRA_HIPCC_FLAGS", "").split()
 
 
diff --git a/stratanet2_vegetation_coverage_maps_amd/_lib.py b/stratanet2_vegetation_coverage_maps_amd/_lib.py
--- a/stratanet2_vegetation_coverage_maps_amd/_lib.py
+++ b/stratanet2_vegetation_coverage_maps_amd/_lib.py
@@ -88,7 +88,8 @@
     _fields_ = [("dcov", c_void_p), ("dproba", c_void_p), ("arena", c_void_p), ("arena_words", c_long), ("images", c_int),
                 ("image_stride", c_int)] + [(n, c_void_p) for n in (
                     "dy2", "dy3", "dx1", "dx2", "dx3", "dy_sa3", "sa1_ws", "dy1", "du1", "du2", "du3", "bn_ok", "src_ws1", "src_ws2")] + [
-                        ("defer_grad_reduce", c_int), ("arena_is_zero", c_int), ("frozen_stats", c_int)]
+                        ("defer_grad_reduce", c_int), ("arena_is_zero", c_int), ("frozen_stats", c_int), ("gl_xchg", c_void_p),
+                        ("gl_ctl", c_void_p)]
 
 
 class NetIO(Structure):
@@ -149,6 +150,7 @@
     "sn2_global_pool_backward": [c_void_p, c_int, c_void_p, c_void_p, c_void_p, c_void_p, c_int, c_int, c_int, c_void_p, c_void_p,
                                  c_void_p, c_void_p, c_void_p],
     "sn2_global_level_forward": [POINTER(FP), POINTER(FP), c_void_p, c_void_p, c_void_p, c_void_p, c_void_p],
+    "sn2_global_level_backward": [POINTER(FP), POINTER(FP), c_void_p, c_void_p, c_void_p, c_void_p],
     "sn2_debug_global_spin_limit": [ctypes.c_uint],
     "sn2_head_forward": [POINTER(Head), c_void_p],
     "sn2_fp_head_eval": [POINTER(FP), POINTER(Head), c_void_p],
diff --git a/stratanet2_vegetation_coverage_maps_amd/csrc/common.h b/stratanet2_vegetation_coverage_maps_amd/csrc/common.h
--- a/stratanet2_vegetation_coverage_maps_amd/csrc/common.h
+++ b/stratanet2_vegetation_coverage_maps_amd/csrc/common.h
@@ -33,6 +33,7 @@
 static inline int sn2_cdiv(long a, long b) { return (int)((a + b - 1) / b); }
 
 constexpr int GL_MAX_PLOTS = 28;
+constexpr int GL_BWD_MAX_ROWS = 256;
 
 #ifdef __HIPCC__
 static __global__ __launch_bounds__(256) void sn2_fill_words_kernel(uint32_t* __restrict__ p, uint32_t v, size_t n) {
diff --git a/stratanet2_vegetation_coverage_maps_amd/csrc/global_level.h b/stratanet2_vegetation_coverage_maps_amd/csrc/global_level.h
--- /dev/null
+++ b/stratanet2_vegetation_coverage_maps_amd/csrc/global_level.h
@@ -0,0 +1,40 @@
+#pragma once
+#include "fp_rows.h"
+
+extern unsigned g_gl_spin_limit;
+
+namespace {
+
+typedef unsigned long long gl_u64;
+constexpr int GL_GROUPS = 4;
+
+constexpr unsigned GL_POISON = 0x80000000u;
+__device__ __forceinline__ bool gl_collect(const gl_u64* gx, int n, unsigned tag, float* s_x, unsigned spin_limit) {
+    bool ok = true;
+    for (int i0 = threadIdx.x; i0 < n; i0 += 8 * 1024) {
+        gl_u64 v[8];
+        unsigned spins = 0;
+        bool all, poisoned;
+        do {
+#pragma unroll
+            for (int u = 0; u < 8; ++u) {
+                const int i = i0 + u * 1024;
+                v[u] = __hip_atomic_load(gx + (i < n ? i : i0), __ATOMIC_RELAXED, __HIP_MEMORY_SCOPE_AGENT);
+            }
+            all = true, poisoned = false;
+#pragma unroll
+            for (int u = 0; u < 8; ++u) {
+                all = all && (unsigned)(v[u] >> 32) == tag;
+                poisoned = poisoned || (unsigned)(v[u] >> 32) == (tag ^ GL_POISON);
+            }
+            if (!all && !poisoned) __builtin_amdgcn_s_sleep(2);
+        } while (!all && !poisoned && ++spins < spin_limit);
+        if (!all) ok = false;
+#pragma unroll
+        for (int u = 0; u < 8; ++u)
+            if (i0 + u * 1024 < n) s_x[i0 + u * 1024] = __uint_as_float((unsigned)v[u]);
+    }
+    return ok;
+}
+
+}
diff --git a/stratanet2_vegetation_coverage_maps_amd/csrc/global_level.hip b/stratanet2_vegetation_coverage_maps_amd/csrc/global_level.hip
--- a/stratanet2_vegetation_coverage_maps_amd/csrc/global_level.hip
+++ b/stratanet2_vegetation_coverage_maps_amd/csrc/global_level.hip
@@ -1,4 +1,4 @@
-#include "fp_rows.h"
+#include "global_level.h"
 
 namespace {
 
@@ -16,8 +16,7 @@
 #else
 #define GSTAMP(i)
 #endif
-typedef unsigned long long gl_u64;
-constexpr int GL_GROUPS = 4, GL_QS = OuterAcc<16, 36>::QS;
+constexpr int GL_QS = OuterAcc<16, 36>::QS;
 constexpr int GL_W3 = 64 * 35 + 64, GL_WF = 64 * 96 + 64;
 constexpr int GL_FIXED_FLOATS = GL_GROUPS * 64 * GL_QS + GL_GROUPS * 128 + 128 + 64 + 2 * 1024 + 2 * 8 * 128 + GL_W3 + GL_WF;
 static_assert((GL_FIXED_FLOATS + GL_MAX_PLOTS * GL_GROUPS * 128) * 4 <= 160 * 1024, "LDS");
@@ -68,35 +67,6 @@
     unsigned spin_limit;
 };
 
-constexpr unsigned GL_POISON = 0x80000000u;
-__device__ __forceinline__ bool gl_collect(const gl_u64* gx, int n, unsigned tag, float* s_x, unsigned spin_limit) {
-    bool ok = true;
-    for (int i0 = threadIdx.x; i0 < n; i0 += 8 * 1024) {
-        gl_u64 v[8];
-        unsigned spins = 0;
-        bool all, poisoned;
-        do {
-#pragma unroll
-            for (int u = 0; u < 8; ++u) {
-                const int i = i0 + u * 1024;
-                v[u] = __hip_atomic_load(gx + (i < n ? i : i0), __ATOMIC_RELAXED, __HIP_MEMORY_SCOPE_AGENT);
-            }
-            all = true, poisoned = false;
-#pragma unroll
-            for (int u = 0; u < 8; ++u) {
-                all = all && (unsigned)(v[u] >> 32) == tag;
-                poisoned = poisoned || (unsigned)(v[u] >> 32) == (tag ^ GL_POISON);
-            }
-            if (!all && !poisoned) __builtin_amdgcn_s_sleep(2);
-        } while (!all && !poisoned && ++spins < spin_limit);
-        if (!all) ok = false;
-#pragma unroll
-        for (int u = 0; u < 8; ++u)
-            if (i0 + u * 1024 < n) s_x[i0 + u * 1024] = __uint_as_float((unsigned)v[u]);
-    }
-    return ok;
-}
-
 template <bool REPAIR>
 __device__ __forceinline__ void gl_level_body(const GlArgs& A, float* gl_smem) {
     const int tid = threadIdx.x, lane = tid & 63;
@@ -429,7 +399,7 @@
 
 }
 
-static unsigned g_gl_spin_limit = 1u << 18;
+unsigned g_gl_spin_limit = 1u << 18;
 extern "C" int sn2_debug_global_spin_limit(unsigned sweeps) {
     g_gl_spin_limit = sweeps ? sweeps : (1u << 18);
     return 0;
diff --git a/stratanet2_vegetation_coverage_maps_amd/csrc/global_level_bwd.hip b/stratanet2_vegetation_coverage_maps_amd/csrc/global_level_bwd.hip
--- /dev/null
+++ b/stratanet2_vegetation_coverage_maps_amd/csrc/global_level_bwd.hip
@@ -0,0 +1,499 @@
+#include <type_traits>
+#include "global_level.h"
+
+namespace {
+
+#ifdef SN2_GB_STAMPS
+__device__ unsigned long long g_gb_dbg[16];
+extern "C" int sn2_debug_gb_stamps(unsigned long long* out) {
+    return (int)hipMemcpyFromSymbol(out, HIP_SYMBOL(g_gb_dbg), sizeof(g_gb_dbg));
+}
+#define BSTAMP(i)                                                                                   \
+    if (blockIdx.x == 0 && threadIdx.x == 0) {                                                      \
+        unsigned long long t_;                                                                      \
+        asm volatile("s_memtime %0\n\ts_waitcnt lgkmcnt(0)" : "=s"(t_)::"memory");                   \
+        g_gb_dbg[i] = t_;                                                                           \
+    }
+#else
+#define BSTAMP(i)
+#endif
+constexpr int GB_QS = OuterAcc<16, 36>::QS;
+constexpr int GB_LD = 68;
+constexpr int GB_WC = 33;
+constexpr int GB_TILES = GL_GROUPS * 64 * (GB_QS + GB_LD);
+constexpr int GB_FIXED_FLOATS = GB_TILES + 128 * GB_WC + 8 * 64 + 16 * 128 + 2 * 128 + 4 * 64;
+static_assert(GB_QS >= 48, "three 16-column tiles of staged inputs");
+static_assert(GL_GROUPS * 128 * 37 <= GB_TILES, "the groups' dW | db partials go through the staging tiles");
+static_assert((GB_FIXED_FLOATS + GL_MAX_PLOTS * 128) * 4 <= 160 * 1024, "LDS");
+
+struct GbLayer {
+    const float *W, *gamma, *mean, *invstd, *h;
+    float *dW, *db, *dgamma, *dbeta;
+};
+struct GbArgs {
+    int B, M2;
+    const float* x2;
+    const float* pos2;
+    const float* x3;
+    const int* arg3;
+    const float* dy3;
+    float* dx2;
+    float* dx3;
+    GbLayer sa3, fp3;
+    int img_stride;
+    gl_u64* xchg;
+    unsigned* ctl;
+    unsigned spin_limit;
+};
+
+__device__ __forceinline__ void gb_wave_sums(float (&s)[4], float* s_red, int wv, int lane, int off) {
+#pragma unroll
+    for (int t = 0; t < 4; ++t) {
+        s[t] += __shfl_xor(s[t], 16);
+        s[t] += __shfl_xor(s[t], 32);
+    }
+    if (lane < 16) {
+#pragma unroll
+        for (int t = 0; t < 4; ++t) s_red[wv * 128 + off + 4 * lane + t] = s[t];
+    }
+}
+
+template <bool ONE_TRIP>
+__device__ __forceinline__ bool gb_plot(const GbArgs& A, float* smem, int b, unsigned epoch, bool publish_only, bool repair) {
+    const int tid = threadIdx.x, lane = tid & 63, t256 = tid & 255;
+    const int grp = __builtin_amdgcn_readfirstlane(tid >> 8), g = __builtin_amdgcn_readfirstlane((tid >> 6) & 3);
+    const int wv = __builtin_amdgcn_readfirstlane(tid >> 6);
+    float* s_q = smem + grp * 64 * GB_QS;
+    float* s_p = smem + GL_GROUPS * 64 * GB_QS + grp * 64 * GB_LD;
+    float* s_wc = smem + GB_TILES;
+    float* s_par = s_wc + 128 * GB_WC;
+    float* s_cf = s_par + 6 * 64;
+    float* s_red = s_cf + 2 * 64;
+    float* s_bnf = s_red + 16 * 128;
+    float* s_bn3 = s_bnf + 128;
+    float* s_sdp = s_bn3 + 128;
+    float* s_g = s_sdp + 64;
+    float* s_x3 = s_g + 64;
+    int* s_arg = reinterpret_cast<int*>(s_x3 + 64);
+    float* s_x = s_x3 + 128;
+    __shared__ int s_fail;
+    const int B = A.B, M2 = A.M2;
+    const long row_lo = (long)b * M2, R_lim = row_lo + M2;
+    const int nblk = (M2 + 63) >> 6, trips = ONE_TRIP ? 1 : (nblk + GL_GROUPS - 1) / GL_GROUPS;
+    const float invR = 1.0f / (float)(B * M2);
+    const int qd = t256 & 15, rw = t256 >> 4;
+    const int r4 = lane >> 4, c16 = lane & 15;
+    const int n_gran = B * 128;
+    gl_u64* xa = A.xchg;
+    gl_u64* xb = A.xchg + GL_MAX_PLOTS * 128;
+    const unsigned tag_a = epoch * 2u, tag_b = epoch * 2u + 1u;
+    __syncthreads();
+    BSTAMP(0)
+#pragma unroll
+    for (int j = 0; j < 4; ++j) {
+        const int i = tid + 1024 * j, k = i >> 5, c = i & 31;
+        s_wc[k * GB_WC + c] = k < 64 ? A.fp3.W[k * 96 + 64 + c] : A.sa3.W[(k - 64) * 35 + c];
+    }
+    float wa[4];
+#pragma unroll
+    for (int j = 0; j < 4; ++j) wa[j] = A.fp3.W[(4 * (tid >> 6) + j) * 96 + (tid & 63)];
+    float dx3_old = 0.f, xh_arg = 0.f;
+    bool arg_ok = false;
+    if (tid < 64) {
+        s_par[0 * 64 + tid] = A.fp3.mean[tid], s_par[1 * 64 + tid] = A.fp3.invstd[tid], s_par[2 * 64 + tid] = A.fp3.gamma[tid];
+        const float m3 = A.sa3.mean[tid], is3 = A.sa3.invstd[tid];
+        s_par[3 * 64 + tid] = m3, s_par[4 * 64 + tid] = is3, s_par[5 * 64 + tid] = A.sa3.gamma[tid];
+        s_x3[tid] = A.x3[(size_t)b * 64 + tid];
+        const int ra = A.arg3[(size_t)b * 64 + tid];
+        arg_ok = ra >= 0 && ra < M2;
+        s_arg[tid] = arg_ok ? ra : -1;
+        if (arg_ok) xh_arg = (A.sa3.h[(size_t)(row_lo + ra) * 64 + tid] - m3) * is3;
+        dx3_old = A.dx3[(size_t)b * 64 + tid];
+    }
+    if (tid == 0) s_fail = 0;
+    if constexpr (ONE_TRIP) {
+        if (grp < nblk)
+            stage_inputs<32, 3, false>(s_q, GB_QS, g, lane, row_lo + (long)grp * 64, (int)R_lim, M2, M2, A.x2, 32, nullptr, nullptr, nullptr,
+                                       nullptr, A.pos2, 4);
+    }
+    float4 hv[4], dv[4];
+    auto load_rows = [&](const float* __restrict__ p, long r0, float4 (&v)[4]) {
+#pragma unroll
+        for (int u = 0; u < 4; ++u) {
+            const long r = r0 + rw + 16 * u;
+            v[u] = reinterpret_cast<const float4*>(p + (size_t)(r < R_lim ? r : R_lim - 1) * 64)[qd];
+        }
+    };
+    __syncthreads();
+    BSTAMP(1)
+    auto quad = [&](const float* p, float (&v)[4]) {
+        const float4 q = *reinterpret_cast<const float4*>(p + 4 * qd);
+        v[0] = q.x, v[1] = q.y, v[2] = q.z, v[3] = q.w;
+    };
+    {
+        float s1[4] = {0.f, 0.f, 0.f, 0.f}, s2[4] = {0.f, 0.f, 0.f, 0.f}, mean_f[4], is_f[4];
+        quad(s_par, mean_f), quad(s_par + 64, is_f);
+        for (int it = 0; it < trips; ++it) {
+            const int blk = it * GL_GROUPS + grp;
+            const long r0 = row_lo + (long)blk * 64;
+            if (blk < nblk) {
+                load_rows(A.fp3.h, r0, hv);
+                load_rows(A.dy3, r0, dv);
+#pragma unroll
+                for (int u = 0; u < 4; ++u) {
+                    const bool live = r0 + rw + 16 * u < R_lim;
+                    const float hq[4] = {hv[u].x, hv[u].y, hv[u].z, hv[u].w}, dq[4] = {dv[u].x, dv[u].y, dv[u].z, dv[u].w};
+#pragma unroll
+                    for (int t = 0; t < 4; ++t) {
+                        const float dd = live ? dq[t] : 0.f;
+                        s1[t] += dd;
+                        s2[t] = fmaf(dd, (hq[t] - mean_f[t]) * is_f[t], s2[t]);
+                    }
+                }
+            }
+        }
+        gb_wave_sums(s1, s_red, wv, lane, 0);
+        gb_wave_sums(s2, s_red, wv, lane, 64);
+        __syncthreads();
+        if (tid < 128) {
+            float v = 0.f;
+#pragma unroll
+            for (int w = 0; w < 16; ++w) v += s_red[w * 128 + tid];
+            __hip_atomic_store(xa + (size_t)b * 128 + tid, ((gl_u64)tag_a << 32) | (gl_u64)__float_as_uint(v), __ATOMIC_RELAXED,
+                               __HIP_MEMORY_SCOPE_AGENT);
+        }
+    }
+    BSTAMP(2)
+    if (!gl_collect(xa, n_gran, tag_a, s_x, A.spin_limit)) s_fail = 1;
+    __syncthreads();
+    BSTAMP(3)
+    if (s_fail) {
+        if (!repair && tid < 128)
+            __hip_atomic_store(xb + (size_t)b * 128 + tid, (gl_u64)(tag_b ^ GL_POISON) << 32, __ATOMIC_RELAXED, __HIP_MEMORY_SCOPE_AGENT);
+        return false;
+    }
+    if (tid < 128) {
+        double acc = 0.0;
+        for (int w = 0; w < B; ++w) acc += (double)s_x[w * 128 + tid];
+        s_bnf[tid] = (float)acc;
+        s_cf[tid] = (float)acc * invR;
+    }
+    __syncthreads();
+    auto dp_of = [&](float hh, float dd, float mean, float is, float gam, float dbeta_r, float dgamma_r, bool live) {
+        const float xh = (hh - mean) * is;
+        const float dh = gam * is * (dd - dbeta_r - xh * dgamma_r);
+        return (live && hh > 0.f) ? dh : 0.f;
+    };
+    auto stage_dp_fp3 = [&](long r0, float (&sd)[4]) {
+        float mean_f[4], is_f[4], gam_f[4], dbt_f[4], dgm_f[4];
+        quad(s_par, mean_f), quad(s_par + 64, is_f), quad(s_par + 128, gam_f), quad(s_cf, dbt_f), quad(s_cf + 64, dgm_f);
+#pragma unroll
+        for (int u = 0; u < 4; ++u) {
+            const bool live = r0 + rw + 16 * u < R_lim;
+            const float hq[4] = {hv[u].x, hv[u].y, hv[u].z, hv[u].w}, dq[4] = {dv[u].x, dv[u].y, dv[u].z, dv[u].w};
+            float p[4];
+#pragma unroll
+            for (int t = 0; t < 4; ++t) {
+                p[t] = dp_of(hq[t], dq[t], mean_f[t], is_f[t], gam_f[t], dbt_f[t], dgm_f[t], live);
+                sd[t] += p[t];
+            }
+            *reinterpret_cast<float4*>(&s_p[(rw + 16 * u) * GB_LD + 4 * qd]) = make_float4(p[0], p[1], p[2], p[3]);
+        }
+    };
+    {
+        float sd[4] = {0.f, 0.f, 0.f, 0.f};
+        for (int it = 0; it < trips; ++it) {
+            const int blk = it * GL_GROUPS + grp;
+            const long r0 = row_lo + (long)blk * 64;
+            if (blk < nblk) {
+                if constexpr (!ONE_TRIP) {
+                    load_rows(A.fp3.h, r0, hv);
+                    load_rows(A.dy3, r0, dv);
+                }
+                stage_dp_fp3(r0, sd);
+            }
+        }
+        gb_wave_sums(sd, s_red, wv, lane, 0);
+        __syncthreads();
+        if (tid < 64) {
+            float v = 0.f;
+#pragma unroll
+            for (int w = 0; w < 16; ++w) v += s_red[w * 128 + tid];
+            s_sdp[tid] = v;
+        }
+        __syncthreads();
+        {
+            const int part = tid >> 6;
+            float acc = 0.f;
+#pragma unroll
+            for (int j = 0; j < 4; ++j) acc = fmaf(s_sdp[4 * part + j], wa[j], acc);
+            s_red[part * 128 + 64 + (tid & 63)] = acc;
+        }
+        __syncthreads();
+        if (tid < 64) {
+            float v = 0.f;
+#pragma unroll
+            for (int k = 0; k < 16; ++k) v += s_red[k * 128 + 64 + tid];
+            const float gg = dx3_old + v;
+            s_g[tid] = gg;
+            const float g1 = arg_ok ? gg : 0.f;
+            __hip_atomic_store(xb + (size_t)b * 128 + tid, ((gl_u64)tag_b << 32) | (gl_u64)__float_as_uint(g1), __ATOMIC_RELAXED,
+                               __HIP_MEMORY_SCOPE_AGENT);
+            __hip_atomic_store(xb + (size_t)b * 128 + 64 + tid, ((gl_u64)tag_b << 32) | (gl_u64)__float_as_uint(g1 * xh_arg),
+                               __ATOMIC_RELAXED, __HIP_MEMORY_SCOPE_AGENT);
+        }
+    }
+    BSTAMP(4)
+    if (publish_only) return true;
+    f32x4 acc_f[2], acc_3[3];
+    f32x4 D[2];
+    acc_f[0] = acc_f[1] = acc_3[0] = acc_3[1] = acc_3[2] = D[0] = D[1] = f32x4{0.f, 0.f, 0.f, 0.f};
+    float4 hs[4];
+    float dx2_old[2][4];
+    auto ask_block = [&](long r0) {
+#pragma unroll
+        for (int jt = 0; jt < 2; ++jt)
+#pragma unroll
+            for (int r = 0; r < 4; ++r) {
+                const long row = r0 + 16 * g + 4 * r4 + r;
+                dx2_old[jt][r] = A.dx2[(size_t)(row < R_lim ? row : R_lim - 1) * 32 + 16 * jt + c16];
+            }
+        load_rows(A.sa3.h, r0, hs);
+    };
+    auto contract_tile = [&](auto& acc, auto nt, int k0) {
+        constexpr int NT = decltype(nt)::value;
+#pragma unroll 4
+        for (int st = 0; st < 16; ++st) {
+            const float av = s_p[(4 * st + r4) * GB_LD + 16 * g + c16];
+#pragma unroll
+            for (int c = 0; c < NT; ++c)
+                acc[c] = __builtin_amdgcn_mfma_f32_16x16x4f32(av, s_q[(4 * st + r4) * GB_QS + 16 * c + c16], acc[c], 0, 0, 0);
+        }
+#pragma unroll 4
+        for (int kb = 0; kb < 16; ++kb) {
+            const float av = s_p[(16 * g + c16) * GB_LD + 4 * kb + r4];
+#pragma unroll
+            for (int jt = 0; jt < 2; ++jt)
+                D[jt] = __builtin_amdgcn_mfma_f32_16x16x4f32(av, s_wc[(k0 + 4 * kb + r4) * GB_WC + 16 * jt + c16], D[jt], 0, 0, 0);
+        }
+    };
+    if constexpr (ONE_TRIP) {
+        if (grp < nblk) {
+            ask_block(row_lo + (long)grp * 64);
+            contract_tile(acc_f, std::integral_constant<int, 2>{}, 0);
+        }
+    }
+    if (!gl_collect(xb, n_gran, tag_b, s_x, A.spin_limit)) s_fail = 1;
+    __syncthreads();
+    BSTAMP(5)
+    if (s_fail) return false;
+    if (tid < 128) {
+        double acc = 0.0;
+        for (int w = 0; w < B; ++w) acc += (double)s_x[w * 128 + tid];
+        s_bn3[tid] = (float)acc;
+    }
+    __syncthreads();
+    for (int it = 0; it < trips; ++it) {
+        const int blk = it * GL_GROUPS + grp;
+        const long r0 = row_lo + (long)blk * 64;
+        const bool act = blk < nblk;
+        if constexpr (!ONE_TRIP) {
+            if (act) {
+                ask_block(r0);
+                stage_inputs<32, 3, false>(s_q, GB_QS, g, lane, r0, (int)R_lim, M2, M2, A.x2, 32, nullptr, nullptr, nullptr, nullptr,
+                                           A.pos2, 4);
+                float sd[4] = {0.f, 0.f, 0.f, 0.f};
+                load_rows(A.fp3.h, r0, hv);
+                load_rows(A.dy3, r0, dv);
+                stage_dp_fp3(r0, sd);
+            }
+            __syncthreads();
+            D[0] = D[1] = f32x4{0.f, 0.f, 0.f, 0.f};
+            if (act) contract_tile(acc_f, std::integral_constant<int, 2>{}, 0);
+            __syncthreads();
+        }
+        if (act) {
+#pragma unroll
+            for (int u = 0; u < 4; ++u) {
+                const int rp = blk * 64 + rw + 16 * u;
+                const bool live = rp < M2;
+                const float hq[4] = {hs[u].x, hs[u].y, hs[u].z, hs[u].w};
+                float p[4];
+#pragma unroll
+                for (int t = 0; t < 4; ++t) {
+                    const int c = 4 * qd + t;
+                    const float dd = s_arg[c] == rp ? s_g[c] : 0.f;
+                    p[t] = dp_of(hq[t], dd, s_par[3 * 64 + c], s_par[4 * 64 + c], s_par[5 * 64 + c], s_bn3[c] * invR, s_bn3[64 + c] * invR, live);
+                }
+                *reinterpret_cast<float4*>(&s_p[(rw + 16 * u) * GB_LD + 4 * qd]) = make_float4(p[0], p[1], p[2], p[3]);
+            }
+        }
+        __syncthreads();
+        if (act) {
+            contract_tile(acc_3, std::integral_constant<int, 3>{}, 64);
+#pragma unroll
+            for (int jt = 0; jt < 2; ++jt)
+#pragma unroll
+                for (int r = 0; r < 4; ++r) {
+                    const long row = r0 + 16 * g + 4 * r4 + r;
+                    if (row < R_lim) A.dx2[(size_t)row * 32 + 16 * jt + c16] = dx2_old[jt][r] + D[jt][r];
+                }
+        }
+        __syncthreads();
+    }
+    BSTAMP(6)
+    {
+        float* s_acc = smem;
+        const int img = b * A.img_stride;
+        float* dst[5];
+        float old[5], old_o[4], old_bn[2] = {0.f, 0.f};
+#pragma unroll
+        for (int j = 0; j < 5; ++j) {
+            const int i = tid + 1024 * j, o = i / 36, k = i - o * 36;
+            dst[j] = nullptr;
+            if (i < 128 * 36) {
+                if (o < 64) {
+                    if (k < 32) dst[j] = A.fp3.dW + img + o * 96 + 64 + k;
+                    else if (k == 35) dst[j] = A.fp3.db + img + o;
+                } else {
+                    dst[j] = k < 35 ? A.sa3.dW + img + (o - 64) * 35 + k : A.sa3.db + img + (o - 64);
+                }
+            }
+            old[j] = dst[j] ? *dst[j] : 0.f;
+        }
+#pragma unroll
+        for (int j = 0; j < 4; ++j) {
+            const int i = tid + 1024 * j;
+            old_o[j] = A.fp3.dW[img + (i >> 6) * 96 + (i & 63)];
+        }
+        float* bn_dst[2] = {nullptr, nullptr};
+        if (b == 0 && tid < 128) {
+            bn_dst[0] = tid < 64 ? A.fp3.dbeta + tid : A.fp3.dgamma + (tid - 64);
+            bn_dst[1] = tid < 64 ? A.sa3.dbeta + tid : A.sa3.dgamma + (tid - 64);
+            old_bn[0] = *bn_dst[0], old_bn[1] = *bn_dst[1];
+        }
+#pragma unroll
+        for (int c = 0; c < 3; ++c)
+#pragma unroll
+            for (int q = 0; q < 4; ++q) {
+                const int o = 16 * g + 4 * r4 + q, k = 16 * c + c16;
+                if (k < 36) {
+                    if (c < 2) s_acc[(grp * 128 + o) * 37 + k] = acc_f[c][q];
+                    s_acc[(grp * 128 + 64 + o) * 37 + k] = acc_3[c][q];
+                }
+            }
+        __syncthreads();
+#pragma unroll
+        for (int j = 0; j < 5; ++j) {
+            const int i = tid + 1024 * j, o = i / 36, k = i - o * 36;
+            if (dst[j]) {
+                const float v = (o < 64 && k == 35) ? s_sdp[o]
+                                                    : (s_acc[(0 * 128 + o) * 37 + k] + s_acc[(1 * 128 + o) * 37 + k]) +
+                                                          (s_acc[(2 * 128 + o) * 37 + k] + s_acc[(3 * 128 + o) * 37 + k]);
+                *dst[j] = old[j] + v;
+            }
+        }
+#pragma unroll
+        for (int j = 0; j < 4; ++j) {
+            const int i = tid + 1024 * j, o = i >> 6, k = i & 63;
+            A.fp3.dW[img + o * 96 + k] = old_o[j] + s_sdp[o] * s_x3[k];
+        }
+        if (tid < 64) A.dx3[(size_t)b * 64 + tid] = s_g[tid];
+        if (bn_dst[0]) {
+            *bn_dst[0] = old_bn[0] + s_bnf[tid];
+            *bn_dst[1] = old_bn[1] + s_bn3[tid];
+        }
+    }
+    BSTAMP(7)
+    return true;
+}
+
+template <bool ONE_TRIP>
+__device__ __noinline__ void gb_repair(GbArgs A, float* smem, unsigned epoch) {
+    for (int pass = 0; pass < 2; ++pass)
+        for (int b = 0; b < A.B; ++b)
+            if (__hip_atomic_load(&A.ctl[8 + b], __ATOMIC_RELAXED, __HIP_MEMORY_SCOPE_AGENT)) gb_plot<ONE_TRIP>(A, smem, b, epoch, pass == 0, true);
+    __syncthreads();
+    if (threadIdx.x == 0) {
+        for (int b = 0; b < A.B; ++b) __hip_atomic_store(&A.ctl[8 + b], 0u, __ATOMIC_RELAXED, __HIP_MEMORY_SCOPE_AGENT);
+        __hip_atomic_store(&A.ctl[2], __hip_atomic_load(&A.ctl[1], __ATOMIC_RELAXED, __HIP_MEMORY_SCOPE_AGENT), __ATOMIC_RELAXED,
+                           __HIP_MEMORY_SCOPE_AGENT);
+    }
+}
+
+template <bool ONE_TRIP>
+__global__ __launch_bounds__(1024) void global_level_bwd_kernel(GbArgs A) {
+    extern __shared__ __attribute__((aligned(16))) float gb_smem[];
+    __shared__ unsigned s_epoch;
+    __shared__ int s_last;
+    const int tid = threadIdx.x;
+    if (tid == 0) s_epoch = __hip_atomic_load(&A.ctl[0], __ATOMIC_RELAXED, __HIP_MEMORY_SCOPE_AGENT) + 1u;
+    __syncthreads();
+    const unsigned epoch = s_epoch;
+    const bool ok = gb_plot<ONE_TRIP>(A, gb_smem, (int)blockIdx.x, epoch, false, false);
+    if (!ok && tid == 0) {
+        __hip_atomic_store(&A.ctl[8 + blockIdx.x], 1u, __ATOMIC_RELAXED, __HIP_MEMORY_SCOPE_AGENT);
+        atomicAdd(&A.ctl[1], 1u);
+    }
+    __syncthreads();
+    if (tid == 0) {
+        const unsigned t = atomicAdd(&A.ctl[4], 1u);
+        int last = 0;
+        if (t == gridDim.x - 1) {
+            __hip_atomic_store(&A.ctl[4], 0u, __ATOMIC_RELAXED, __HIP_MEMORY_SCOPE_AGENT);
+            last = __hip_atomic_load(&A.ctl[1], __ATOMIC_RELAXED, __HIP_MEMORY_SCOPE_AGENT) !=
+                           __hip_atomic_load(&A.ctl[2], __ATOMIC_RELAXED, __HIP_MEMORY_SCOPE_AGENT)
+                       ? 2
+                       : 1;
+        }
+        s_last = last;
+    }
+    __syncthreads();
+    if (!s_last) return;
+    if (s_last == 2) gb_repair<ONE_TRIP>(A, gb_smem, epoch);
+    if (tid == 0) __hip_atomic_store(&A.ctl[0], epoch, __ATOMIC_RELAXED, __HIP_MEMORY_SCOPE_AGENT);
+}
+
+}
+
+extern "C" int sn2_global_level_backward(const sn2_fp* sa3, const sn2_fp* fp3, const int* arg3, unsigned long long* xchg,
+                                         unsigned* ctl, void* stream) {
+    if (!sa3 || !fp3 || !arg3 || !xchg || !ctl) return SN2_EINVAL;
+    const int B = sa3->B, M2 = sa3->R_per_plot;
+    if (!(B > 0 && M2 > 0 && fp3->B == B && fp3->R_per_plot == M2 && sa3->S_per_plot == M2 && fp3->S_per_plot == 1)) return SN2_EINVAL;
+    if (!(sa3->ca == 32 && sa3->cb == 3 && sa3->blk.cin == 35 && sa3->blk.cout == 64 && fp3->ca == 64 && fp3->cb == 32 &&
+          fp3->blk.cin == 96 && fp3->blk.cout == 64))
+        return SN2_ELIMIT;
+    if (sa3->blk.mma_bf16 || fp3->blk.mma_bf16 || sa3->act_bf16 || fp3->act_bf16 || sa3->blk.frozen_stats || fp3->blk.frozen_stats)
+        return SN2_ELIMIT;
+    if (sa3->knn_idx || sa3->src_a || !fp3->knn_idx || fp3->src_a) return SN2_EINVAL;
+    if (!sa3->src || sa3->src_stride != 32 || !sa3->skip || sa3->skip_stride != 4 || !sa3->h || sa3->h_stride != 64) return SN2_EINVAL;
+    if (!fp3->src || fp3->src_stride != 64 || fp3->skip != sa3->src || fp3->skip_stride != 32 || !fp3->h || fp3->h_stride != 64)
+        return SN2_EINVAL;
+    if (!fp3->dy || !fp3->dsrc || fp3->dsrc_stride != 64 || !fp3->dskip || fp3->dskip_stride != 32 || sa3->dsrc != fp3->dskip ||
+        sa3->dsrc_stride != 32)
+        return SN2_EINVAL;
+    for (const sn2_block* k : {&sa3->blk, &fp3->blk})
+        if (!k->W || !k->gamma || !k->mean || !k->invstd || !k->dW || !k->db || !k->dgamma || !k->dbeta) return SN2_EINVAL;
+    if (B > GL_MAX_PLOTS || (long)B * M2 >= (1L << 31) / 64) return SN2_ELIMIT;
+    if (sa3->blk.grad_replicas < B || fp3->blk.grad_replicas < B || sa3->blk.grad_replica_stride != fp3->blk.grad_replica_stride)
+        return SN2_ELIMIT;
+    GbArgs A;
+    A.B = B, A.M2 = M2;
+    A.x2 = sa3->src, A.pos2 = sa3->skip, A.x3 = fp3->src, A.arg3 = arg3, A.dy3 = fp3->dy, A.dx2 = fp3->dskip, A.dx3 = fp3->dsrc;
+    auto layer = [](const sn2_fp* p) {
+        GbLayer l;
+        l.W = p->blk.W, l.gamma = p->blk.gamma, l.mean = p->blk.mean, l.invstd = p->blk.invstd, l.h = p->h;
+        l.dW = p->blk.dW, l.db = p->blk.db, l.dgamma = p->blk.dgamma, l.dbeta = p->blk.dbeta;
+        return l;
+    };
+    A.sa3 = layer(sa3), A.fp3 = layer(fp3);
+    A.img_stride = sa3->blk.grad_replica_stride;
+    A.xchg = xchg, A.ctl = ctl;
+    A.spin_limit = g_gl_spin_limit;
+    const size_t lds = ((size_t)GB_FIXED_FLOATS + (size_t)B * 128) * 4;
+    auto kern = M2 <= GL_GROUPS * 64 ? &global_level_bwd_kernel<true> : &global_level_bwd_kernel<false>;
+    (void)hipFuncSetAttribute(reinterpret_cast<const void*>(kern), hipFuncAttributeMaxDynamicSharedMemorySize, (int)lds);
+    hipLaunchKernelGGL(kern, dim3(B), dim3(1024), lds, (hipStream_t)stream, A);
+    SN2_RETURN_LAUNCH();
+}
diff --git a/stratanet2_vegetation_coverage_maps_amd/csrc/net.hip b/stratanet2_vegetation_coverage_maps_amd/csrc/net.hip
--- a/stratanet2_vegetation_coverage_maps_amd/csrc/net.hip
+++ b/stratanet2_vegetation_coverage_maps_amd/csrc/net.hip
@@ -553,19 +553,24 @@
     p2.dy = b->dy2, p2.dsrc = b->dy3, p2.dsrc_stride = 64, p2.dskip = b->dx1, p2.dskip_stride = 16;
     p2.du_scratch = b->du2, p2.scatter_ws = g->inv2, p2.scatter_ready = 1, p2.bn_sums_done = b->bn_ok + 1;
     SN2_TRY(sn2_fp_backward(&p2, cur));
-    SN2_TRY(sn2_fp_bn_sums(&p2, m->fp3.gamma, m->fp3.beta, aux_row(a, 4, 2), aux_row(a, 4, 3), b->arena + m->fp3.ggamma,
-                           b->arena + m->fp3.gbeta, b->bn_ok + 2, cur));
-    sn2_fp pf3;
+    sn2_fp pf3, p3;
     fp_desc(&pf3, d, a, fp3_in(m, d, g, a), gd);
     pf3.dy = b->dy3, pf3.dsrc = b->dx3, pf3.dsrc_stride = 64, pf3.dskip = b->dx2, pf3.dskip_stride = 32;
-    pf3.du_scratch = b->du3, pf3.scatter_ws = g->inv3, pf3.scatter_ready = -1, pf3.bn_sums_done = b->bn_ok + 2;
-    SN2_TRY(sn2_fp_backward(&pf3, cur));
-    SN2_TRY(sn2_global_pool_backward(b->du3, 64, a->arg3, a->h_sa3, aux_row(a, 3, 2), aux_row(a, 3, 3), B, M2, 64, b->dx3, b->dy_sa3,
-                                     b->arena + m->sa3.ggamma, b->arena + m->sa3.gbeta, cur));
-    sn2_fp p3;
     fp_desc(&p3, d, a, sa3_in(m, d, g, a), gd);
-    p3.dy = b->dy_sa3, p3.dsrc = b->dx2, p3.dsrc_stride = 32, p3.bn_sums_done = b->bn_ok + 3;
-    SN2_TRY(sn2_fp_backward(&p3, cur));
+    p3.dsrc = b->dx2, p3.dsrc_stride = 32;
+    if (m->fuse_global_level && !b->frozen_stats && b->gl_xchg && b->gl_ctl && B <= GL_MAX_PLOTS && M2 <= GL_BWD_MAX_ROWS &&
+        !m->sa3.mma_bf16 && !m->fp3.mma_bf16) {
+        SN2_TRY(sn2_global_level_backward(&p3, &pf3, a->arg3, b->gl_xchg, b->gl_ctl, cur));
+    } else {
+        SN2_TRY(sn2_fp_bn_sums(&p2, m->fp3.gamma, m->fp3.beta, aux_row(a, 4, 2), aux_row(a, 4, 3), b->arena + m->fp3.ggamma,
+                               b->arena + m->fp3.gbeta, b->bn_ok + 2, cur));
+        pf3.du_scratch = b->du3, pf3.scatter_ws = g->inv3, pf3.scatter_ready = -1, pf3.bn_sums_done = b->bn_ok + 2;
+        SN2_TRY(sn2_fp_backward(&pf3, cur));
+        SN2_TRY(sn2_global_pool_backward(b->du3, 64, a->arg3, a->h_sa3, aux_row(a, 3, 2), aux_row(a, 3, 3), B, M2, 64, b->dx3,
+                                         b->dy_sa3, b->arena + m->sa3.ggamma, b->arena + m->sa3.gbeta, cur));
+        p3.dy = b->dy_sa3, p3.bn_sums_done = b->bn_ok + 3;
+        SN2_TRY(sn2_fp_backward(&p3, cur));
+    }
     sn2_sa sa;
     sa2_desc(&sa, m, d, g, a, gd, b->dx2, b->dx1);
     SN2_TRY(sn2_sa_backward(&sa, cur));
diff --git a/stratanet2_vegetation_coverage_maps_amd/executor.py b/stratanet2_vegetation_coverage_maps_amd/executor.py
--- a/stratanet2_vegetation_coverage_maps_amd/executor.py
+++ b/stratanet2_vegetation_coverage_maps_amd/executor.py
@@ -420,6 +420,9 @@
     cb.defer_grad_reduce = int(defer)
     cb.arena_is_zero = int(pre_zeroed)
     cb.frozen_stats = int(bool(s.__dict__.get("frozen", False)))
+    if model.fuse_global_level and not cb.frozen_stats and plan.B <= ops.GL_MAX_PLOTS and plan.dims.M2 <= ops.GL_BWD_MAX_ROWS:
+        ws = ops.global_level_ws(dev, owner=model)
+        cb.gl_xchg, cb.gl_ctl = ws[3].data_ptr(), ws[4].data_ptr()
     _lib.check(lib.sn2_net_backward(byref(ms.c), byref(plan.dims), byref(geo_struct(s.geo)), byref(s.cact), byref(cb), ops._stream()),
                "sn2_net_backward")
     flat = arena[:ms.n_flat]
diff --git a/stratanet2_vegetation_coverage_maps_amd/hip_ops.py b/stratanet2_vegetation_coverage_maps_amd/hip_ops.py
--- a/stratanet2_vegetation_coverage_maps_amd/hip_ops.py
+++ b/stratanet2_vegetation_coverage_maps_amd/hip_ops.py
@@ -838,7 +838,8 @@
         if torch.cuda.is_current_stream_capturing():
             raise StrataHipError("global_level_forward: its exchange area must exist before a stream capture starts -- run one "
                                  "eager training forward first (TrainPipeline.capture does) or call hip_ops.global_level_ws(dev, owner=model)")
-        ws = _GlobalWs([torch.zeros(2 * GL_MAX_PLOTS * 4 * 128, dtype=I64, device=dev), torch.zeros(8, dtype=I32, device=dev), 0])
+        ws = _GlobalWs([torch.zeros(2 * GL_MAX_PLOTS * 4 * 128, dtype=I64, device=dev), torch.zeros(8, dtype=I32, device=dev), 0,
+                        torch.zeros(2 * GL_MAX_PLOTS * 128, dtype=I64, device=dev), torch.zeros(64, dtype=I32, device=dev)])
         store[key] = ws
         import weakref
         _GLOBAL_WS_ALL[:] = [r for r in _GLOBAL_WS_ALL if r() is not None]
@@ -852,6 +853,20 @@
     _chk(arg3, I32, (B, 64), "arg3")
     ws = global_level_ws(x3.device, B, owner=owner)
     _call("sn2_global_level_forward", d_sa3, d_fp3, _ptr(x3), _ptr(arg3), _ptr(ws[0]), _ptr(ws[1]), _stream())
+
+
+GL_BWD_MAX_ROWS = 256
+
+
+def global_level_backward_fused(B: int, M2: int, frozen: bool, *blocks) -> bool:
+    return B <= GL_MAX_PLOTS and M2 <= GL_BWD_MAX_ROWS and not frozen and not any(b.mma_bf16 for b in blocks)
+
+
+def global_level_backward(d_sa3: FP, d_fp3: FP, arg3: torch.Tensor, owner=None):
+    B = d_sa3.B
+    _chk(arg3, I32, (B, 64), "arg3")
+    ws = global_level_ws(arg3.device, B, owner=owner)
+    _call("sn2_global_level_backward", d_sa3, d_fp3, _ptr(arg3), _ptr(ws[3]), _ptr(ws[4]), _stream())
 
 
 def global_level_gave_up(dev, warn: bool = True) -> int:
@@ -862,14 +877,14 @@
         ws = r()
         if ws is None or ws[1].device.index != key:
             continue
-        n = int(ws[1][1].item())
+        n = int(ws[1][1].item()) + int(ws[4][1].item())
         total += n
         if n > ws[2]:
             seen, ws[2] = ws[2], n
             if warn:
                 import warnings
-                warnings.warn(f"global_level_forward: {n - seen} exchange wait(s) gave up on {dev}; those launches were repeated "
-                              "by the single-workgroup repair launch (results unaffected, the passes took longer); set "
+                warnings.warn(f"global_level_forward / backward: {n - seen} exchange wait(s) gave up on {dev}; those launches were finished "
+                              "by their last workgroup alone (results unaffected, the passes took longer); set "
                               "PointNet2.fuse_global_level = False where other kernels or processes share the device",
                               StrataHipWarning, stacklevel=2)
     return total
diff --git a/stratanet2_vegetation_coverage_maps_amd/point_net2.py b/stratanet2_vegetation_coverage_maps_amd/point_net2.py
--- a/stratanet2_vegetation_coverage_maps_amd/point_net2.py
+++ b/stratanet2_vegetation_coverage_maps_amd/point_net2.py
@@ -646,18 +646,22 @@
         d2 = self._fp2_desc(s, dy=dy2, dsrc=dy3, dskip=dx1, du_scratch=torch.empty(B * M1, 64, dtype=F32, device=dev),
                             with_grads=True, interp_index=s.inv2, bn_sums_done=bn_ok[1:2])
         ops.fp_backward(d2)
-        bn3 = self.fp3_module.nn[0][2]
-        ops.fp_bn_sums(d2, bn3.weight.detach(), bn3.bias.detach(), s.b_fp3.aux[2], s.b_fp3.aux[3], views[id(bn3.weight)],
-                       views[id(bn3.bias)], bn_ok[2:3])
         dx3, dx2 = buf["dx3"].view(B, 64), buf["dx2"].view(B * M2, 32)
-        du3 = torch.empty(B * M2, 64, dtype=F32, device=dev)
-        ops.fp_backward(self._fp3_desc(s, dy=dy3, dsrc=dx3, dskip=dx2, du_scratch=du3, with_grads=True,
-                                       interp_index=s.inv3, bn_sums_done=bn_ok[2:3], gather=False))
-        dy_sa3 = buf["dy_sa3"].view(B * M2, 64)
-        bn_sa3 = self.sa3_module.nn[0][2]
-        ops.global_pool_backward(du3, s.arg3, s.h_sa3, s.b_sa3.aux[2], s.b_sa3.aux[3], B, M2, dx3, dy_sa3,
-                                 views[id(bn_sa3.weight)], views[id(bn_sa3.bias)])
-        ops.fp_backward(self._sa3_desc(s, dy=dy_sa3, dsrc=dx2, with_grads=True, bn_sums_done=bn_ok[3:4]))
+        if self.fuse_global_level and ops.global_level_backward_fused(B, M2, getattr(s.b_fp3, "frozen", False), s.b_sa3, s.b_fp3):
+            ops.global_level_backward(self._sa3_desc(s, dsrc=dx2, with_grads=True),
+                                      self._fp3_desc(s, dy=dy3, dsrc=dx3, dskip=dx2, with_grads=True), s.arg3, owner=self)
+        else:
+            bn3 = self.fp3_module.nn[0][2]
+            ops.fp_bn_sums(d2, bn3.weight.detach(), bn3.bias.detach(), s.b_fp3.aux[2], s.b_fp3.aux[3], views[id(bn3.weight)],
+                           views[id(bn3.bias)], bn_ok[2:3])
+            du3 = torch.empty(B * M2, 64, dtype=F32, device=dev)
+            ops.fp_backward(self._fp3_desc(s, dy=dy3, dsrc=dx3, dskip=dx2, du_scratch=du3, with_grads=True,
+                                           interp_index=s.inv3, bn_sums_done=bn_ok[2:3], gather=False))
+            dy_sa3 = buf["dy_sa3"].view(B * M2, 64)
+            bn_sa3 = self.sa3_module.nn[0][2]
+            ops.global_pool_backward(du3, s.arg3, s.h_sa3, s.b_sa3.aux[2], s.b_sa3.aux[3], B, M2, dx3, dy_sa3,
+                                     views[id(bn_sa3.weight)], views[id(bn_sa3.bias)])
+            ops.fp_backward(self._sa3_desc(s, dy=dy_sa3, dsrc=dx2, with_grads=True, bn_sums_done=bn_ok[3:4]))
         ops.sa_backward(self._sa2_desc(s, dout=dx2, dfeat=dx1, g=True))
         ops.sa_backward(self._sa1_desc(s, dout=dx1, g=True, bwd_ws=buf["sa1_ws"]))
         if getattr(self, "defer_grad_reduce", False):
```
